# pathint/RankCompV3.jl

Measured on AMD Instinct MI355X. Metric: gene-pair·sample comparisons/sec at 20k genes × 1k samples, higher is better.
Workload: dtype u16

## Files before the change

rankcompv3.jl_amd/_ffi.py:

```python
from __future__ import annotations

import ctypes
import os
import subprocess
from typing import NamedTuple

import numpy as np

_HERE = os.path.dirname(os.path.abspath(__file__))
LIB_PATH = os.environ.get("REO_LIB_PATH") or os.path.join(_HERE, "libreo_hip.so")
CSRC = os.path.join(_HERE, "csrc")

REO_OK, REO_EINVAL, REO_EHIP, REO_ECOMM, REO_ENOMEM = 0, -1, -2, -3, -4
NTIMINGS = 12
CALL_BINS = 8192

SYMBOLS = [
    "reo_version", "reo_last_error", "reo_create", "reo_destroy", "reo_trim_memory", "reo_set_shard", "reo_set_allreduce", "reo_set_allgather",
    "reo_create_multi", "reo_comm_unique_id", "reo_comm_init_rank",
    "reo_set_matrix_f64", "reo_set_matrix_i64", "reo_set_matrix_dev_f64", "reo_set_matrix_dev_i64",
    "reo_set_matrix_f32", "reo_set_matrix_i32", "reo_set_matrix_dev_f32", "reo_set_matrix_dev_i32",
    "reo_set_matrix_rm_f64", "reo_set_matrix_rm_i64", "reo_set_matrix_rm_f32", "reo_set_matrix_rm_i32",
    "reo_set_matrix_csc_f64", "reo_set_matrix_csc_i64", "reo_set_matrix_csc_f32", "reo_set_matrix_csc_i32",
    "reo_set_groups", "reo_compute_thresholds", "reo_set_thresholds", "reo_get_thresholds", "reo_threshold",
# ... 1138 lines not shown
        counts, key = np.zeros((m, 4), dtype=np.int32), np.zeros((m, 2), dtype=np.int64)
        found, passes = ctypes.c_int64(0), ctypes.c_int32(0)
        check(self._L.reo_top_pairs(self._h, a, b, _opt(gm), n, _ptr(gi), _ptr(gj), _ptr(counts), _ptr(key), ctypes.addressof(found),
                                    ctypes.addressof(passes)))
        k = int(found.value)
        return TopPairs(gi[:k].copy(), gj[:k].copy(), counts[:k, 0::2].copy(), counts[:k, 1::2].copy(), key[:k, 0].copy(), key[:k, 1].copy(),
                        sizes, a, None if b < 0 else b, int(passes.value))

    def top_partners(self, genes=None, m: int = 1, a: int = 0, b=None, partner_mask=None) -> TopPartners:
        m = int(m)
        a, b, sizes = self._sides(a, b)
        g = np.arange(self.G, dtype=np.int32) if genes is None else np.ascontiguousarray(np.asarray(genes).reshape(-1), dtype=np.int32)
        pm = None
        if partner_mask is not None:
            pm = np.asarray(partner_mask)
            if pm.shape != (self.G,):
                raise DimensionMismatch(REO_EINVAL, f"top_partners: partner_mask has shape {tuple(pm.shape)}, the matrix has {self.G} genes")
            pm = np.ascontiguousarray(pm if pm.dtype == np.uint8 else pm != 0, dtype=np.uint8)
        Q = int(g.size)
        w = min(max(m, 1), 1024)
        rows = Q if 1 <= Q <= 1 << 20 and Q * w <= 1 << 26 else 1
        partner = np.full((rows, w), -1, dtype=np.int32)
        counts, key = np.zeros((rows, w, 4), dtype=np.int32), np.zeros((rows, w, 2), dtype=np.int64)
        found = np.zeros(rows, dtype=np.int32)
        check(self._L.reo_top_partners(self._h, a, b, _ptr(g) if Q else None, Q, _opt(pm), m, _ptr(partner), _ptr(counts), _ptr(key), _ptr(found)))
        return TopPartners(g, partner, counts[:, :, 0::2].copy(), counts[:, :, 1::2].copy(), key[:, :, 0].copy(), key[:, :, 1].copy(), found,
                           sizes, a, None if b < 0 else b)

    def top_pairs_null(self, sides, a: int = 0, b=None, gene_mask=None, cuts=None) -> TopPairsNull:
        a, b, sizes = self._sides(a, b)
        rows = np.asarray(sides)
        if rows.ndim == 1:
            rows = rows.reshape(1, -1)
        if rows.ndim != 2 or rows.shape[1] != self.S:
            raise DimensionMismatch(REO_EINVAL, f"top_pairs_null: sides has shape {tuple(np.shape(sides))}, label rows are B x S = B x {self.S}")
        if rows.size and (rows.min() < 0 or rows.max() > 255):
            raise DimensionMismatch(REO_EINVAL, "top_pairs_null: label rows hold 0 (side B), 1 (side A) and 2 (takes no part)")
        rows = np.ascontiguousarray(rows, dtype=np.uint8)
        gm = None
        if gene_mask is not None:
            gm = np.asarray(gene_mask)
            if gm.shape != (self.G,):
                raise DimensionMismatch(REO_EINVAL, f"top_pairs_null: gene_mask has shape {tuple(gm.shape)}, the matrix has {self.G} genes")
            gm = np.ascontiguousarray(gm if gm.dtype == np.uint8 else gm != 0, dtype=np.uint8)
        ct = np.zeros(0, dtype=np.int64) if cuts is None else np.ascontiguousarray(np.asarray(cuts, dtype=np.int64).reshape(-1))
        B = rows.shape[0]
        m = min(max(B, 1), 1 << 20)
        nc = min(ct.size, 8)
        max_n, gi, gj = np.zeros(m, dtype=np.int64), np.zeros(m, dtype=np.int32), np.zeros(m, dtype=np.int32)
        reach = np.zeros((m, nc), dtype=np.int64)
        check(self._L.reo_top_pairs_null(self._h, a, b, _ptr(rows) if rows.size else None, B, _opt(gm), _ptr(ct) if ct.size else None, ct.size,
                                         _ptr(max_n), _ptr(gi), _ptr(gj), _ptr(reach) if reach.size else None))
        return TopPairsNull(max_n[:B], gi[:B], gj[:B], reach[:B], ct, sizes, a, None if b < 0 else b)

    def top_pairs_loo(self, kmax: int, a: int = 0, b=None, gene_mask=None) -> TopPairsLoo:
        kmax = int(kmax)
        a, b, sizes = self._sides(a, b)
        gm = None
        if gene_mask is not None:
            gm = np.asarray(gene_mask)
            if gm.shape != (self.G,):
                raise DimensionMismatch(REO_EINVAL, f"top_pairs_loo: gene_mask has shape {tuple(gm.shape)}, the matrix has {self.G} genes")
            gm = np.ascontiguousarray(gm if gm.dtype == np.uint8 else gm != 0, dtype=np.uint8)
        m, S = min(max(kmax, 1), 64), max(self.S, 1)
        gi, gj = np.full((S, m), -1, dtype=np.int32), np.full((S, m), -1, dtype=np.int32)
        num, gam = np.zeros((S, m), dtype=np.int64), np.zeros((S, m), dtype=np.int64)
        out, side, stats = np.zeros((S, m), dtype=np.int8), np.full(S, 2, dtype=np.int8), np.zeros(4, dtype=np.int64)
        check(self._L.reo_top_pairs_loo(self._h, a, b, _opt(gm), kmax, _ptr(gi), _ptr(gj), _ptr(num), _ptr(gam), _ptr(out), _ptr(side), _ptr(stats)))
        n = self.S
        return TopPairsLoo(gi[:n], gj[:n], num[:n], gam[:n], out[:n], side[:n], sizes, a, None if b < 0 else b, int(stats[0]), int(stats[1]))

    def mccullagh(self, cont) -> np.ndarray:
        cont = np.ascontiguousarray(cont, dtype=np.int32).reshape(-1, 9)
        out = np.zeros((cont.shape[0], 5), dtype=np.float64)
        check(self._L.reo_mccullagh(self._h, _ptr(cont), cont.shape[0], _ptr(out)))
        return out

    @staticmethod
    def _pseudobulk_args(cells, order, chunk_ptr):
        order = np.ascontiguousarray(order, dtype=np.int32)
        chunk_ptr = np.ascontiguousarray(chunk_ptr, dtype=np.int32)
        n_out = chunk_ptr.size - 1
        if hasattr(cells, "tocsc"):
            m = cells.tocsc()
            m.sort_indices()
            G, C = m.shape
            isint = np.issubdtype(m.dtype, np.integer)
            val = np.ascontiguousarray(m.data, dtype=np.int64 if isint else np.float64)
            colptr = np.ascontiguousarray(m.indptr, dtype=np.int64)
            rowidx = np.ascontiguousarray(m.indices, dtype=np.int32)
            args = (G, C, _ptr(colptr), _ptr(rowidx), _ptr(val), _ptr(order), order.size, _ptr(chunk_ptr), n_out)
            return "csc", "i64" if isint else "f64", args, G, (m, val, colptr, rowidx, order, chunk_ptr)
        X = np.asarray(cells)
        isint = np.issubdtype(X.dtype, np.integer)
        Xf = np.asfortranarray(X, dtype=np.int64 if isint else np.float64)
        G, C = Xf.shape
        args = (_ptr(Xf), G, C, G, _ptr(order), order.size, _ptr(chunk_ptr), n_out)
        return "dense", "i64" if isint else "f64", args, G, (Xf, order, chunk_ptr)

    def pseudobulk(self, cells, order, chunk_ptr) -> np.ndarray:
        form, ty, args, G, keep = self._pseudobulk_args(cells, order, chunk_ptr)
        out = np.zeros((G, args[-1]), dtype=np.int64 if ty == "i64" else np.float64, order="F")
        check(getattr(self._L, f"reo_pseudobulk_{form}_{ty}")(self._h, *args, _ptr(out)))
        return out

    def set_matrix_pseudobulk(self, cells, order, chunk_ptr) -> None:
        if is_device_sparse(cells) or is_device_tensor(cells):
            order = np.ascontiguousarray(order, dtype=np.int32)
            chunk_ptr = np.ascontiguousarray(chunk_ptr, dtype=np.int32)
            n_out = chunk_ptr.size - 1
            tail = (_ptr(order) if order.size else None, order.size, _ptr(chunk_ptr), n_out)
            if is_device_sparse(cells):
                ty, G, C, nnz, colptr, rowidx, val, bits, keep = device_csc_entry(cells)
                check(getattr(self._L, "reo_set_matrix_pseudobulk_csc_dev_" + ty)(self._h, G, C, nnz, _dptr(colptr), _dptr(rowidx), bits, _dptr(val), *tail))
            else:
                ptr, G, C, ld, ty, keep = device_matrix(cells)
                check(getattr(self._L, "reo_set_matrix_pseudobulk_dense_dev_" + ty)(self._h, ctypes.c_void_p(ptr), G, C, ld, *tail))
            self.G, self.S = G, n_out
            return
        form, ty, args, G, keep = self._pseudobulk_args(cells, order, chunk_ptr)
        check(getattr(self._L, f"reo_set_matrix_pseudobulk_{form}_{ty}")(self._h, *args))
        self.G, self.S = G, args[-1]

    def filter_matrix(self, min_profiles: int = 0, min_features: int = 0):
        info = self.info()
        pk = np.zeros(info["S"], dtype=np.uint8)
        gk = np.zeros(info["G"], dtype=np.uint8)
        sk, gkn = ctypes.c_int64(0), ctypes.c_int64(0)
        check(self._L.reo_filter_matrix(self._h, int(min_profiles), int(min_features), _ptr(pk) if pk.size else None, _ptr(gk) if gk.size else None,
                                        ctypes.byref(sk), ctypes.byref(gkn)))
        self.G, self.S = int(gkn.value), int(sk.value)
        return pk.astype(bool), gk.astype(bool)

    def get_matrix(self) -> np.ndarray:
        info = self.info()
        dt = {1: np.float64, 2: np.int64, 3: np.float32}.get(info["resident_dtype"])
        if dt is None:
            raise DimensionMismatch(REO_EINVAL, "no expression matrix set")
        out = np.zeros((info["G"], info["S"]), dtype=dt, order="F")
        check(self._L.reo_get_matrix(self._h, _ptr(out), out.nbytes))
        return out

    def set_profiling(self, on: bool) -> None:
        check(self._L.reo_set_profiling(self._h, 1 if on else 0))

    def reset_timings(self) -> None:
        check(self._L.reo_reset_timings(self._h))

    def timings(self) -> dict:
        ms = np.zeros(NTIMINGS, dtype=np.float64)
        check(self._L.reo_get_timings(self._h, _ptr(ms), NTIMINGS))
        return {"transform_ms": ms[0], "k1_ms": ms[1], "k2_ms": ms[2], "iter_ms": ms[3], "k3_ms": max(ms[3] - ms[2], 0.0), "k2_launches": int(ms[4]),
                "k1_launches": int(ms[5]), "exchange_ms": ms[6], "pseudobulk_ms": ms[7], "k2_full_ms": ms[8],
                "k2_full_launches": int(ms[9]), "k2_delta_ms": ms[10], "set_matrix_host_wall_ms": ms[11]}

    def info(self) -> dict:
        w = np.zeros(44, dtype=np.int64)
        check(self._L.reo_get_info(self._h, _ptr(w), 44))
        v = np.zeros(28, dtype=np.int64)
        v[:] = w[:28]
        return {"G": int(v[0]), "S": int(v[1]), "Gp": int(v[2]), "table_bytes": int(v[3]), "has_ties": int(v[4]),
                "tiles_owned": int(v[5]), "tiles_total": int(v[6]), "tile_i": int(v[7]), "chunk_j": int(v[8]),
                "chunks_per_panel": int(v[9]), "unit_h": int(v[10]), "sample_slots": int(v[11]),
                "shared_group_counts": int(v[12]), "group_count_bytes": int(v[13]), "transform_in_lds": int(v[14]), "xcc_local_histograms": int(v[15]),
                "cycle_period": int(v[16]), "cycle_found_at_pass": int(v[17]), "cycle_passes_skipped": int(v[18]), "upload_link_bytes": int(v[19]),
                "eager_range_launches": int(v[20]), "rowmajor_upload": int(v[21]),
                "csc_upload": int(v[22]), "csc_nnz": int(v[23]), "resident_dtype": int(v[24]),
                "k1_slot_order": int(v[25]), "k1_half_tiles_separated": int(v[26]), "csc_device": int(v[27]),
                "k1_unslot_form": int(w[28]), "contrast_treat": int(w[29]), "k1_slot_sides": int(w[30]),
                "masked_build": int(w[31]), "k1_slot_slice": int(w[32]), "planes_on_demand": int(w[33]),
                "perm_batch": int(w[34]), "perm_kernel_us": int(w[35]),
                "top_pairs_hist_us": int(w[36]), "top_pairs_emit_us": int(w[37]),
                "top_pairs_null_batch": int(w[38]), "top_pairs_null_us": int(w[39]),
                "top_pairs_loo_words_us": int(w[40]), "top_pairs_loo_select_us": int(w[41]),
                "top_partners_count_us": int(w[42]), "top_partners_select_us": int(w[43])}
```

rankcompv3.jl_amd/csrc/api.hip:

```cpp
#include <execinfo.h>
#include <signal.h>
#include <unistd.h>

#include <ctime>
#include <algorithm>
#include <chrono>
#include <cmath>
#include <cstdarg>
#include <cstdio>
#include <cstdlib>
#include <cstring>

#include "reo_internal.h"
#include "contrast.h"
#include "masked_pairs.h"
#include "perm_null.h"
#include "sample_counts.h"
#include "upload_csc.h"

#include <mutex>
#include <unordered_map>

namespace reo {

// ... 34 lines not shown
        auto &v = H.streams[kind];
        for (size_t i = v.size(); i-- > 0;)
            if (v[i].first == dev) { *s = v[i].second; v.erase(v.begin() + static_cast<long>(i)); return hipSuccess; }
    }
    if (kind == 0) return hipStreamCreateWithFlags(s, hipStreamNonBlocking);
    int lo_pri = 0, hi_pri = 0;
    const hipError_t e = hipDeviceGetStreamPriorityRange(&lo_pri, &hi_pri);
    return e != hipSuccess ? e : hipStreamCreateWithPriority(s, hipStreamNonBlocking, hi_pri);
}

hipError_t handle_event(hipEvent_t *ev, int kind)
{
    int dev = 0;
    (void)hipGetDevice(&dev);
    {
        Handles &H = handles();
        std::lock_guard<std::mutex> lk(H.mu);
        auto &v = H.events[kind];
        for (size_t i = v.size(); i-- > 0;)
            if (v[i].first == dev) { *ev = v[i].second; v.erase(v.begin() + static_cast<long>(i)); return hipSuccess; }
    }
    return kind ? hipEventCreate(ev) : hipEventCreateWithFlags(ev, hipEventDisableTiming);
}

void release_stream(hipStream_t s, int kind)
{
    if (!s) return;
    int dev = 0;
    (void)hipGetDevice(&dev);
    Handles &H = handles();
    {
        std::lock_guard<std::mutex> lk(H.mu);
        if (H.streams[kind].size() < 64 && pool().cap > 0 && hipStreamQuery(s) == hipSuccess) { H.streams[kind].emplace_back(dev, s); return; }
    }
    (void)hipStreamDestroy(s);
}

void release_event(hipEvent_t ev, int kind)
{
    if (!ev) return;
    int dev = 0;
    (void)hipGetDevice(&dev);
    Handles &H = handles();
    {
        std::lock_guard<std::mutex> lk(H.mu);
        if (H.events[kind].size() < 1024 && pool().cap > 0) { H.events[kind].emplace_back(dev, ev); return; }
    }
    (void)hipEventDestroy(ev);
}

hipError_t pool_alloc(void **out, size_t bytes, bool pinned)
{
    Pool &P = pool();
    bytes = pool_round(bytes);
    int dev = 0;
    (void)hipGetDevice(&dev);
    {
        std::lock_guard<std::mutex> lk(P.mu);
        if (!P.read_env) {
            P.read_env = true;
            if (const char *e = getenv("REO_DEVICE_CACHE_MB")) P.cap = static_cast<size_t>(std::max(0L, atol(e))) << 20;
        }
        int best = -1;
        for (int i = 0; i < static_cast<int>(P.free_blocks.size()); ++i) {
            const Block &b = P.free_blocks[i];
            if (b.pinned != pinned || (!pinned && b.device != dev) || b.bytes < bytes || b.bytes > bytes + bytes / 4 + 4096) continue;
            if (best < 0 || b.bytes < P.free_blocks[best].bytes) best = i;
        }
        if (best >= 0) {
            *out = P.free_blocks[best].p;
            P.cached -= P.free_blocks[best].bytes;
            P.live[*out] = P.free_blocks[best].bytes;
            P.free_blocks.erase(P.free_blocks.begin() + best);
            return hipSuccess;
        }
    }
    hipError_t e = raw_alloc(out, bytes, pinned);
    if (e == hipErrorOutOfMemory) {
        (void)hipGetLastError();
        (void)reo_trim_memory();
        e = raw_alloc(out, bytes, pinned);
    }
    if (e == hipSuccess) { std::lock_guard<std::mutex> lk(P.mu); P.live[*out] = bytes; }
    return e;
}

void pool_free(void *p, size_t bytes, bool pinned)
{
    if (!p) return;
    Pool &P = pool();
    bytes = pool_round(bytes);
    int dev = 0;
    (void)hipGetDevice(&dev);
    std::vector<Block> evict;
    {
        std::lock_guard<std::mutex> lk(P.mu);
        const auto it = P.live.find(p);
        if (it != P.live.end()) { bytes = it->second; P.live.erase(it); }
        if (bytes > P.cap) { evict.push_back({p, bytes, dev, pinned}); }
        else {
            P.free_blocks.push_back({p, bytes, dev, pinned});
            P.cached += bytes;
            while (P.cached > P.cap && !P.free_blocks.empty()) {
                evict.push_back(P.free_blocks.front());
                P.cached -= P.free_blocks.front().bytes;
                P.free_blocks.erase(P.free_blocks.begin());
            }
        }
    }
    for (const Block &b : evict) {
        if (!b.pinned && b.device != dev) (void)hipSetDevice(b.device);
        raw_free(b.p, b.pinned);
        if (!b.pinned && b.device != dev) (void)hipSetDevice(dev);
    }
}

void set_error(const char *fmt, ...)
{
    char buf[1024];
    va_list ap;
    va_start(ap, fmt);
    vsnprintf(buf, sizeof buf, fmt, ap);
    va_end(ap);
    g_err = buf;
}

void tic(reo_ctx *c, int slot)
{
    if (!c->profiling) return;
    StageTimer t;
    if (!c->pool.empty()) { t = c->pool.back(); c->pool.pop_back(); }
    else { (void)handle_event(&t.a, 1); (void)handle_event(&t.b, 1); }
    (void)hipEventRecord(t.a, c->stream);
    c->pending.emplace_back(slot, t);
    c->open.push_back(c->pending.size() - 1);
}

void toc(reo_ctx *c)
{
    if (!c->profiling || c->open.empty()) return;
    (void)hipEventRecord(c->pending[c->open.back()].second.b, c->stream);
    c->open.pop_back();
}

void collect_timings(reo_ctx *c)
{
    for (auto &pr : c->pending) {
        float ms = 0.f;
        (void)hipEventSynchronize(pr.second.b);
        if (hipEventElapsedTime(&ms, pr.second.a, pr.second.b) == hipSuccess) {
            c->t_ms[pr.first] += ms;
            if (pr.first == 2 && !c->k2_modes.empty()) {
                if (c->k2_seen < c->k2_modes.size()) {
                    if (c->k2_modes[c->k2_seen]) { c->t_ms[8] += ms; c->t_ms[9] += 1.0; }
                    else c->t_ms[10] += ms;
                }
                ++c->k2_seen;
            }
        }
        c->pool.push_back(pr.second);
    }
    c->pending.clear();
    c->open.clear();
    c->k2_modes.clear();
    c->k2_seen = 0;
}

static int32_t major_reo_lower_count(int32_t n, double thr) { return reo_lower_count(n, thr); }

static hipError_t stream_wait(reo_ctx *c)
{
    if (!c->spin_wait) return hipStreamSynchronize(c->stream);
    for (unsigned spin = 0;; ++spin) {
        const hipError_t q = hipStreamQuery(c->stream);
        if (q != hipErrorNotReady) return q;
        if (spin > (1u << 22)) return hipStreamSynchronize(c->stream);
    }
}

static struct sigaction g_old_action[3];

static void segv_backtrace(int sig)
{
    static const char head[] = "libreo_hip: fatal signal, native backtrace of the faulting thread:\n";
    (void)!write(2, head, sizeof head - 1);
    void *frames[64];
    const int n = backtrace(frames, 64);
    backtrace_symbols_fd(frames, n, 2);
    sigaction(sig, &g_old_action[sig == SIGSEGV ? 0 : (sig == SIGBUS ? 1 : 2)], nullptr);
    raise(sig);
}

static void install_segv_backtrace()
{
    static bool done = false;
    if (done) return;
    done = true;
    void *warm[2];
    (void)backtrace(warm, 2);
    struct sigaction sa;
    memset(&sa, 0, sizeof sa);
    sa.sa_handler = segv_backtrace;
    sa.sa_flags = SA_NODEFER;
    sigaction(SIGSEGV, &sa, &g_old_action[0]);
    sigaction(SIGBUS, &sa, &g_old_action[1]);
    sigaction(SIGABRT, &sa, &g_old_action[2]);
}

static double wall_us()
{
    timespec ts;
    clock_gettime(CLOCK_MONOTONIC, &ts);
    return ts.tv_sec * 1e6 + ts.tv_nsec * 1e-3;
}

static void drop_ref_mask(reo_ctx *c, const char *why)
{
    c->ref_slot = -1;
    c->ref_gone = why;
}

int32_t wait_or_drop_table(reo_ctx *c)
{
    const hipError_t e = stream_wait(c);
    if (e == hipSuccess) return REO_OK;
    c->built_k = -1;
    c->table_complete = false;
    drop_ref_mask(c, "a kernel queued on this context failed and the class table was dropped");
    set_error("a kernel queued on this context failed: %s (the class table was dropped: call reo_build_pairs again)", hipGetErrorString(e));
    return REO_EHIP;
}

int32_t use(reo_ctx *c)
{
    if (!c) { set_error("null context"); return REO_EINVAL; }
    REO_HIP_CHECK(hipSetDevice(c->device));
    return REO_OK;
}

int32_t no_multi(reo_ctx *c, const char *what)
{
    if (!c) { set_error("null context"); return REO_EINVAL; }
    if (c->in_multi) {
        set_error("%s is not available on a reo_create_multi context (every device would need the matrix: use one process per GPU, each with its own context)", what);
        return REO_EINVAL;
    }
    return REO_OK;
}

bool mask_in_force(reo_ctx *c)
{
    if (c->vmask_set && (c->vmask_G != c->G || c->vmask_S != c->S)) { c->vmask_set = false; c->vwords_valid = false; }
    return c->vmask_set;
}

int32_t refuse_under_mask(reo_ctx *c, const char *what)
{
    if (!c || !mask_in_force(c)) return REO_OK;
    char msg[320];
    mp_query_refusal(what, msg, sizeof msg);
    set_error("%s", msg);
    return REO_EINVAL;
}

static void invalidate(reo_ctx *c)
{
    drop_ref_mask(c, "the matrix or the groups changed after the last reo_identify_degs (reo_set_matrix_*, reo_filter_matrix, reo_set_groups): "
                     "the class table it ran on is gone");
    c->transformed = false;
    c->planes_ready = false; c->planes_on_demand = 0; c->last_k1_slot_slice = 0;
    c->built_k = -1;
    c->built_treat = -1;
    c->built_masked = 0;
    c->gc_valid = false;
    c->eager_k1 = false;
    c->vwords_valid = false;
    (void)mask_in_force(c);
    c->last_k1_slots = 0; c->last_k1_slot_sides = 0; c->k1_slot_items = nullptr; c->k1_slot_items_n = 0; c->k1_slot_gp = 0;
}

static size_t elem_bytes(int dtype) { return dtype >= 3 ? 4 : 8; }

static int32_t check_shape(int64_t G, int64_t S)
{
    if (G < 2 || G > kMaxGenes || S < 2 || S > (1 << 20)) {
        set_error("matrix is %lld x %lld; G must be in [2, %d] and S in [2, 1048576]", (long long)G, (long long)S, kMaxGenes);
        return REO_EINVAL;
    }
    return REO_OK;
}

static int32_t set_matrix(reo_ctx *c, const void *X, int64_t G, int64_t S, int64_t ld, int dtype, bool on_device, int layout = kLayoutColMajor)
{
    const bool rowmajor = layout == kLayoutRowMajor;
    int32_t rc = use(c);
    if (rc) return rc;
    if (dtype >= 3 && getenv("REO_TRANSFORM") && getenv("REO_TRANSFORM")[0] == 's') {
        set_error("REO_TRANSFORM=segmented: the segmented sort of the A/B build takes Float64 and Int64 matrices only, not Float32 / Int32");
        return REO_EINVAL;
    }
    if (!X) { set_error("matrix pointer is null"); return REO_EINVAL; }
    if ((rc = check_shape(G, S))) return rc;
    if (rowmajor && ld < S) { set_error("row pitch %lld < S = %lld (row-major: ld counts the elements from one gene's row to the next)", (long long)ld, (long long)S); return REO_EINVAL; }
    if (layout == kLayoutColMajor && ld < G) { set_error("leading dimension %lld < G = %lld", (long long)ld, (long long)G); return REO_EINVAL; }
    invalidate(c);
    c->rowmajor_upload = 0;
    c->csc_upload = 0; c->csc_nnz = 0; c->csc_device = 0;
    const bool host_i32 = dtype == 4 && !on_device;
    const size_t resident = static_cast<size_t>(G) * S * (dtype == 3 ? 4 : 8);
    c->G = G; c->S = S; c->dtype = dtype == 4 ? 2 : dtype;
    if (on_device && dtype == 4) {
        if ((rc = c->dX_owned.ensure(resident))) return rc;
        c->dX = c->dX_owned.p; c->ld = G;
        if ((rc = widen_device_i32(c, X, ld, G, S, c->dX_owned.p))) { invalidate(c); c->dtype = 0; return rc; }
        if (hipStreamSynchronize(c->stream) != hipSuccess) { set_error("widening the Int32 matrix failed"); invalidate(c); c->dtype = 0; return REO_EHIP; }
    } else if (on_device) {
        c->dX = X; c->ld = ld;
        c->dX_owned.release();
    } else {
        if ((rc = c->dX_owned.ensure(resident))) return rc;
        c->dX = c->dX_owned.p; c->ld = G;
        const bool lds_ranking = G <= 65535 && !(getenv("REO_TRANSFORM") && getenv("REO_TRANSFORM")[0] == 's');
        if (c->eager_mode > 0 && lds_ranking && static_cast<int64_t>(c->group_id.size()) == S && !c->in_multi) {
            const bool k1 = c->eager_mode > 1 && c->ngroups == 2 && c->thr_set && c->world <= 1 && !c->comm && !c->ag && !c->ar && c->k1_wave &&
                            S <= 65535 && !c->k1_stamps;
            c->Gp = static_cast<int>((c->G + kGenePad - 1) / kGenePad) * kGenePad;
            c->Wp = c->Gp / 32;
            if ((rc = c->table.ensure(static_cast<size_t>(c->G) * kPlanes * c->Wp))) return rc;
            const double w0 = wall_us();
            struct DrainUp {
                reo_ctx *c;
                ~DrainUp() { if (c->up) (void)hipStreamSynchronize(c->up); if (c->rk) (void)hipStreamSynchronize(c->rk); }
            } drain_up{c};
            DrainOnExit drain(c);
            rc = eager_upload(c, X, ld, k1, host_i32, layout);
            if (rc) { invalidate(c); return rc; }
            c->rowmajor_upload = rowmajor ? 1 : 0;
            c->csc_upload = layout == kLayoutCsc ? 1 : 0;
            drain.dismiss();
            c->t_ms[11] += (wall_us() - w0) * 1e-3;
            if (c->eager_k1) { c->built_k = 0; c->table_complete = true; }
            return REO_OK;
        }
        struct DrainUp2 {
            reo_ctx *c;
            ~DrainUp2() { if (c->up) (void)hipStreamSynchronize(c->up); }
        } drain_up{c};
        DrainOnExit drain(c);
        const double w0 = wall_us();
        if ((rc = upload_columns(c, X, ld, G, S, c->dX_owned.p, dtype, layout))) { invalidate(c); return rc; }
        c->rowmajor_upload = rowmajor ? 1 : 0;
        c->csc_upload = layout == kLayoutCsc ? 1 : 0;
        drain.dismiss();
        c->t_ms[11] += (wall_us() - w0) * 1e-3;
    }
    return REO_OK;
}

int32_t ensure_transform(reo_ctx *c)
{
    if (c->dtype == 0) { set_error("no expression matrix set"); return REO_EINVAL; }
    if (c->group_id.empty()) { set_error("no groups set"); return REO_EINVAL; }
    if (static_cast<int64_t>(c->group_id.size()) != c->S) {
        set_error("'data' and 'group' do not have compatible sizes (%lld columns, %zu group labels)",
                  (long long)c->S, c->group_id.size());
        return REO_EINVAL;
    }
    if (c->transformed) return REO_OK;
    c->Gp = static_cast<int>((c->G + kGenePad - 1) / kGenePad) * kGenePad;
    c->Wp = c->Gp / 32;
    c->table_prezeroed = false;
    int32_t rc = c->table.ensure(static_cast<size_t>(c->G) * kPlanes * c->Wp);
    if (rc) return rc;
    return run_transform(c);
}

static int32_t ensure_iter_buffers(reo_ctx *c)
{
    int32_t rc;
    const size_t G = c->G;
    for (int t = 0; t < 2; ++t) {
        if ((rc = c->refbits[t].ensure(c->Wp))) return rc;
        if ((rc = c->refbytes[t].ensure(c->Gp))) return rc;
    }
    if ((rc = c->raw.ensure(G * kRaw)) ||
        (rc = c->delta_list.ensure(2 * static_cast<size_t>(c->Gp))) || (rc = c->cont.ensure(G * 9)) || (rc = c->result.ensure(G * 15)) ||
        (rc = c->sorted_d.ensure((G + 63) / 64 * 64 + (G + 63) / 64)) || (rc = c->sorted_p.ensure(G)) || (rc = c->rank_s.ensure(G)) ||
        (rc = c->rank_a.ensure(G)) || (rc = c->scal.ensure(8)) || (rc = c->blockmin.ensure(std::max<size_t>(64, (G + 1023) / 1024))) ||
        (rc = c->state.ensure(1)) ||
        (rc = c->chunk_v.ensure(((G + kSortChunk - 1) / kSortChunk) * (kSortChunk + kSortChunk / 32))) ||
        (rc = c->chunk_i.ensure(((G + kSortChunk - 1) / kSortChunk) * kSortChunk)) || (rc = c->part.ensure(3 * (std::max<size_t>(65536, (G + kSortChunk - 1) / kSortChunk * kSortChunk) / 16 + 8))) ||
        (rc = c->cand.ensure(2 * 1024)) || (rc = c->gridbar.ensure(4)) || (rc = c->hist.ensure(3 * kHistParts * ((G + 32767) / 32768 * 32768))) || (rc = c->olist.ensure(2 * kOneStride)) || (rc = c->mrank.ensure(c->Gp)) || (rc = c->lstate.ensure(1)) || (rc = c->clist.ensure(2 * kListStride)) || (rc = c->scal.ensure(64)))
        return rc;
    if (!c->host_state) REO_HIP_CHECK(pool_alloc(reinterpret_cast<void **>(&c->host_state), sizeof(IterState), true));
    return REO_OK;
}

static int32_t upload_ref(reo_ctx *c, const uint8_t *ref, int slot, int32_t *nref)
{
    int32_t n = 0;
    for (int64_t i = 0; i < c->G; ++i) n += ref[i] != 0;
    *nref = n;
    REO_HIP_CHECK(hipMemsetAsync(c->refbytes[slot].p, 0, c->Gp, c->stream));
    REO_HIP_CHECK(hipMemcpyAsync(c->refbytes[slot].p, ref, c->G, hipMemcpyHostToDevice, c->stream));
    return launch_pack_ref(c, c->refbytes[slot].p, c->refbits[slot].p);
}

static int32_t init_state(reo_ctx *c, int32_t nref)
{
    IterState st;
    memset(&st, 0, sizeof st);
    st.nref = nref;
    st.nref_prev = nref;
    st.delta_cnt[0] = st.delta_cnt[1] = 0x7FFFFFFF;
    st.need_full = 1;
    st.raw_pass = -1;
    st.kstar = -1;
    *c->host_state = st;
    REO_HIP_CHECK(hipMemcpyAsync(c->state.p, c->host_state, sizeof st, hipMemcpyHostToDevice, c->stream));
    return REO_OK;
}

static int32_t exchange_table(reo_ctx *c)
{
    if (c->x_pipelined) {
        c->table_complete = true;
        return REO_OK;
    }
    c->table_complete = c->world <= 1;
    if (c->world <= 1 && !c->comm) return REO_OK;
    int32_t rc;
    if (c->comm || c->ag) {
        const int64_t bytes = exchange_unit_words(c) * exchange_units_per_rank(c) * static_cast<int64_t>(sizeof(uint32_t));
        if ((rc = c->xsend.ensure(static_cast<size_t>(bytes / 4))) || (rc = c->xrecv.ensure(static_cast<size_t>(bytes / 4) * c->world))) return rc;
        tic(c, 6);
        if ((rc = launch_pack_units(c))) return rc;
        if (c->comm) {
            if ((rc = comm_allgather(c, c->xsend.p, c->xrecv.p, bytes)) < 0) return rc;
        } else {
            rc = c->ag(c->xsend.p, c->xrecv.p, bytes, c->stream, c->ag_user);
            if (rc) { set_error("all-gather hook failed with %d", rc); return REO_ECOMM; }
        }
        if ((rc = launch_expand_units(c))) return rc;
        toc(c);
    } else {
        if (!c->ar) return REO_OK;
        const int64_t count = static_cast<int64_t>(c->G) * kPlanes * c->Wp;
        tic(c, 6);
        rc = c->ar(c->table.p, count, c->stream, c->ar_user);
        toc(c);
        if (rc) { set_error("all-reduce hook failed with %d", rc); return REO_ECOMM; }
    }
    c->table_complete = true;
    return REO_OK;
}

static int32_t pass_fault(reo_ctx *c)
{
    const int32_t f = c->host_state ? c->host_state->fault : 0;
    if (!f) return REO_OK;
    if (f == kFaultTallies) {
        set_error("the iteration passes met tallies that no class table can produce (a gene pair in two states at once): the table in "
                  "this context is not what reo_build_pairs makes -- an exchange hook delivered wrong words and the scan of its "
                  "table was switched off (REO_CHECK_HOOK_TABLE=0)");
        c->built_k = -1;
        c->table_complete = false;
    } else {
        set_error("the persistent iteration kernel gave up at a grid barrier (a workgroup did not arrive within its bound); "
                  "REO_LIGHT=1 runs the same passes as separate launches");
    }
    return REO_EHIP;
}

int32_t upload_slot2col(reo_ctx *c, const std::vector<int32_t> &map)
{
    if (map == c->sc_slot2col_host && c->sc_slot2col.p == c->sc_slot2col_uploaded) return REO_OK;
    c->sc_slot2col_host = map;
    c->sc_slot2col_uploaded = nullptr;
    REO_HIP_CHECK(hipMemcpyAsync(c->sc_slot2col.p, c->sc_slot2col_host.data(), map.size() * sizeof(int32_t), hipMemcpyHostToDevice, c->stream));
    c->sc_slot2col_uploaded = c->sc_slot2col.p;
    return REO_OK;
}

int32_t need_complete_table(reo_ctx *c)
{
    if (c->built_k < 0) { set_error("no class table: call reo_build_pairs first"); return REO_EINVAL; }
    if (!c->table_complete) {
        set_error("shard %d of %d holds only its own part of the class table: attach a communicator (reo_comm_init_rank) or an "
                  "exchange hook (reo_set_allgather, reo_set_allreduce) before reo_build_pairs", c->rank, c->world);
        return REO_ECOMM;
    }
    return REO_OK;
}

}

using namespace reo;

extern "C" {

int32_t reo_version(void) { return 1600; }

int32_t reo_trim_memory(void)
{
    std::vector<Block> all;
    {
        Pool &P = pool();
        std::lock_guard<std::mutex> lk(P.mu);
        all.swap(P.free_blocks);
        P.cached = 0;
    }
    int dev = 0;
    const bool have_dev = hipGetDevice(&dev) == hipSuccess;
    for (const Block &b : all) {
        if (!b.pinned) (void)hipSetDevice(b.device);
        raw_free(b.p, b.pinned);
    }
    {
        Handles &H = handles();
        std::lock_guard<std::mutex> lk(H.mu);
        for (int k = 0; k < 2; ++k) {
            for (auto &st : H.streams[k]) { (void)hipSetDevice(st.first); (void)hipStreamDestroy(st.second); }
            for (auto &ev : H.events[k]) { (void)hipSetDevice(ev.first); (void)hipEventDestroy(ev.second); }
            H.streams[k].clear(); H.events[k].clear();
        }
    }
    if (have_dev) (void)hipSetDevice(dev);
    return REO_OK;
}

const char *reo_last_error(void) { return g_err.c_str(); }

int32_t reo_create(reo_ctx **out, int32_t device, uint64_t seed)
{
    if (!out) { set_error("out is null"); return REO_EINVAL; }
    *out = nullptr;
    if (getenv("REO_DEBUG_SEGV")) install_segv_backtrace();
    int ndev = 0;
    if (hipGetDeviceCount(&ndev) != hipSuccess || ndev == 0) {
        set_error("no HIP device visible: libreo_hip has no CPU fallback");
        return REO_EHIP;
    }
    if (device < 0) REO_HIP_CHECK(hipGetDevice(&device));
    if (device >= ndev) { set_error("device %d out of range (%d visible)", device, ndev); return REO_EINVAL; }
    hipDeviceProp_t prop;
    REO_HIP_CHECK(hipGetDeviceProperties(&prop, device));
    if (strncmp(prop.gcnArchName, "gfx950", 6) != 0) {
        set_error("device %d is %s; this library carries gfx950 (MI355X) code objects only", device, prop.gcnArchName);
        return REO_EHIP;
    }
    REO_HIP_CHECK(hipSetDevice(device));
    reo_ctx *c = new (std::nothrow) reo_ctx();
    if (!c) { set_error("out of host memory"); return REO_ENOMEM; }
    c->device = device;
    c->seed = seed;
    if (const char *e = getenv("REO_K1_WAVE")) c->k1_wave = (e[0] != '0');
    if (const char *e = getenv("REO_K1_HALF")) c->k1_half = (e[0] != '0');
    if (const char *e = getenv("REO_K1_SLOTS")) c->k1_slots = (e[0] != '0');
    if (const char *e = getenv("REO_K1_QUEUE")) c->k1_queue = (e[0] != '0');
    if (const char *e = getenv("REO_K1_UNSLOT")) { const int v = atoi(e); c->k1_unslot = (v == 8 || v == 4) ? v : (e[0] == '0' ? 0 : -1); }
    if (const char *e = getenv("REO_K1_SLOT_SIDES")) { const int v = atoi(e); c->k1_slot_sides = (v == 1 || v == 2) ? v : 0; }
    if (const char *e = getenv("REO_K1_SLOT_SLICE")) c->k1_slot_slice = atoi(e) != 0;
    if (const char *e = getenv("REO_K1_WORKERS")) c->k1_workers = std::max(1, atoi(e));
    if (const char *e = getenv("REO_K1_ORDER")) c->k1_order = std::max(0, std::min(2, atoi(e)));
    {
        int n = 0;
        if (hipDeviceGetAttribute(&n, hipDeviceAttributeMultiprocessorCount, c->device) == hipSuccess && n > 0) c->n_cus = n;
    }
    if (const char *e = getenv("REO_SPIN_WAIT")) c->spin_wait = (e[0] != '0');
    if (const char *e = getenv("REO_CHECK_HOOK_TABLE")) c->check_hook_table = (e[0] != '0');
    if (const char *e = getenv("REO_SHARE_GROUP_COUNTS")) c->share_counts = (e[0] != '0');
    if (const char *e = getenv("REO_LIGHT_BAND")) c->light_band = std::max(0, atoi(e));
    if (const char *e = getenv("REO_HIST_BELOW")) c->hist_below = std::max(0, atoi(e));
    if (const char *e = getenv("REO_CYCLE")) c->cycle_watch = atoi(e) != 0;
    if (const char *e = getenv("REO_LIGHT")) c->light_mode = e[0] == '0' ? 0 : (e[0] == '2' ? 2 : (e[0] == '3' ? 3 : 1));
    c->light_window = light_window(); c->light_min_g = light_min_genes();
    if (const char *e = getenv("REO_LIGHT_WINDOW")) c->light_window = std::max(1, std::min(31, atoi(e)));
    if (const char *e = getenv("REO_LIGHT_MIN_G")) c->light_min_g = std::max(64, atoi(e));
    if (const char *e = getenv("REO_STATE_MIRROR")) c->state_mirror_wanted = (e[0] != '0');
    if (const char *e = getenv("REO_EXCHANGE_WAVES")) c->x_waves = std::max(1, std::min(8, atoi(e)));
    if (const char *e = getenv("REO_EAGER_UPLOAD")) c->eager_mode = std::max(0, std::min(2, atoi(e)));
    if (const char *e = getenv("REO_EAGER_CHUNK")) c->eager_chunk = std::max(1, atoi(e));
    if (const char *e = getenv("REO_EAGER_GATE")) c->eager_gate = atoi(e) != 0;
    if (const char *e = getenv("REO_EAGER_RANGES")) c->eager_ranges = std::max(1, std::min(6, atoi(e)));
    if (const char *e = getenv("REO_UPLOAD_THREADS")) c->upload_threads = std::max(0, std::min(64, atoi(e)));
    c->debug_passes = getenv("REO_DEBUG_PASSES") != nullptr;
    c->debug_stamps = getenv("REO_DEBUG_STAMPS") != nullptr;
    c->k1_stamps = getenv("REO_K1_STAMPS") != nullptr;
    hipError_t e = handle_stream(&c->stream, 0);
    if (e != hipSuccess) { delete c; set_error("hipStreamCreate failed: %s", hipGetErrorString(e)); return REO_EHIP; }
    int ok = 0;
    const char *xe = getenv("REO_XCC_LOCAL");
    if (!(xe && xe[0] == '0')) {
        const int32_t rc = xcc_selftest(c, &ok);
        if (rc) { reo_destroy(c); return rc; }
    }
    c->xcc_local = ok;
    *out = c;
    return REO_OK;
}

void reo_destroy(reo_ctx *c)
{
    if (!c) return;
    for (reo_ctx *p : c->peers) reo_destroy(p);
    c->peers.clear();
    (void)hipSetDevice(c->device);
    for (int q = 0; q < 2; ++q) if (c->k1s[q]) (void)hipStreamSynchronize(c->k1s[q]);
    if (c->xs) (void)hipStreamSynchronize(c->xs);
    if (c->up) (void)hipStreamSynchronize(c->up);
    if (c->rk) (void)hipStreamSynchronize(c->rk);
    (void)hipStreamSynchronize(c->stream);
    comm_release(c);
    collect_timings(c);
    tl_release_synced = true;
    for (auto &t : c->pool) { release_event(t.a, 1); release_event(t.b, 1); }
    c->dX_owned.release(); c->pos.release(); c->lo.release(); c->hi.release(); c->goff_dev.release();
    c->table.release();
    c->t_kin.release(); c->t_kout.release(); c->t_vin.release(); c->t_vout.release(); c->t_temp.release();
    c->t_order.release(); c->t_flags.release(); c->t_slots.release(); c->unit_map.release();
    for (auto &il : c->k1_wave_items) il.buf.release();
    for (int q = 0; q < 2; ++q) { release_stream(c->k1s[q], 0); release_event(c->ev_k1_join[q], 0); }
    release_stream(c->xs, 0);
    release_stream(c->up, 0);
    release_stream(c->rk, 1);
    for (auto &e : c->ev_rk) release_event(e, 0);
    for (auto &e : c->ev_up) release_event(e, 0);
    c->e_lists.release();
    for (int q = 0; q < 3; ++q) {
        if (c->stage_h[q]) pool_free(c->stage_h[q], c->stage_cap, true);
        c->stage_d[q].release();
        release_event(c->ev_stage[q], 0);
        release_event(c->ev_widen[q], 0);
    }
    release_event(c->ev_fork, 0);
    release_event(c->ev_x, 0);
    for (auto &e : c->ev_k1) release_event(e, 0);
    c->t_pos16.release(); c->t_lo16.release(); c->t_hi16.release(); c->gcounts.release();
    c->k1_slot_part.release(); c->k1_slot_maps.release(); c->pos_s.release(); c->lo_s.release(); c->k1_queue_ctr.release();
    c->t_pos32.release(); c->t_lo32.release(); c->t_hi32.release(); c->t_vin32.release(); c->t_vout32.release();
    for (int t = 0; t < 2; ++t) { c->refbits[t].release(); c->refbytes[t].release(); }
    c->raw.release(); c->delta_list.release(); c->cont.release(); c->result.release(); c->sorted_d.release(); c->sorted_p.release();
    c->rank_s.release(); c->rank_a.release(); c->scal.release(); c->blockmin.release();
    c->state.release(); c->trace.release(); c->modes.release(); c->cand.release(); c->hist.release(); c->mrank.release(); c->lstate.release(); c->clist.release(); c->olist.release(); c->units_all.release(); c->xsend.release(); c->xrecv.release(); c->check_flag.release(); c->gridbar.release(); c->chunk_v.release(); c->chunk_i.release(); c->part.release();
    if (c->host_state) pool_free(c->host_state, sizeof(IterState), true);
    if (c->host_flags) pool_free(c->host_flags, 8 * sizeof(int32_t), true);
    release_event(c->ev_flags, 0);
    if (c->host_ref) pool_free(c->host_ref, c->host_ref_cap, true);
    release_stream(c->stream, 0);
    delete c;
    tl_release_synced = false;
}

int32_t reo_set_shard(reo_ctx *c, int32_t rank, int32_t world)
{
    if (!c) { set_error("null context"); return REO_EINVAL; }
    if (world < 1 || rank < 0 || rank >= world) { set_error("bad shard %d of %d", rank, world); return REO_EINVAL; }
    if (!c->peers.empty()) { set_error("a multi-GPU context (reo_create_multi) shards by itself"); return REO_EINVAL; }
    c->rank = rank; c->world = world;
    c->built_k = -1;
    drop_ref_mask(c, "reo_set_shard dropped the class table that the last reo_identify_degs ran on");
    c->eager_k1 = false;
    c->gc_valid = false;
    c->table_complete = false;
    return REO_OK;
}

int32_t reo_set_allreduce(reo_ctx *c, reo_allreduce_fn fn, void *user)
{
    if (!c) { set_error("null context"); return REO_EINVAL; }
    c->ar = fn; c->ar_user = user;
    return REO_OK;
}

int32_t reo_set_allgather(reo_ctx *c, reo_allgather_fn fn, void *user)
{
    if (!c) { set_error("null context"); return REO_EINVAL; }
    c->ag = fn; c->ag_user = user;
    return REO_OK;
}

static int32_t set_matrix_all(reo_ctx *c, const void *X, int64_t G, int64_t S, int64_t ld, int dtype, bool on_device, int layout = kLayoutColMajor)
{
    int32_t rc = set_matrix(c, X, G, S, ld, dtype, on_device, layout);
    for (size_t d = 0; d < (c ? c->peers.size() : 0) && !rc; ++d) {
        reo_ctx *p = c->peers[d];
        if (!on_device) { rc = set_matrix(p, X, G, S, ld, dtype, false, layout); continue; }
        const void *src = dtype == 4 ? c->dX : X;
        const int64_t sld = dtype == 4 ? G : ld;
        const size_t eb = dtype == 4 ? 8 : elem_bytes(dtype);
        if ((rc = use(p)) || (rc = p->dX_owned.ensure(static_cast<size_t>(G) * S * eb))) break;
        if (hipMemcpy2DAsync(p->dX_owned.p, static_cast<size_t>(G) * eb, src, static_cast<size_t>(sld) * eb, static_cast<size_t>(G) * eb, static_cast<size_t>(S),
                             hipMemcpyDefault, p->stream) != hipSuccess) {
            set_error("peer copy of the matrix to device %d failed", p->device); rc = REO_EHIP;
        }
        if (!rc && hipStreamSynchronize(p->stream) != hipSuccess) { set_error("peer copy failed"); rc = REO_EHIP; }
        if (!rc) { invalidate(p); p->G = G; p->S = S; p->dtype = dtype == 4 ? 2 : dtype; p->dX = p->dX_owned.p; p->ld = G; }
    }
    if (c && !c->peers.empty()) (void)hipSetDevice(c->device);
    return rc;
}

int32_t reo_set_matrix_f64(reo_ctx *c, const double *X, int64_t G, int64_t S, int64_t ld) { return set_matrix_all(c, X, G, S, ld, 1, false); }
int32_t reo_set_matrix_i64(reo_ctx *c, const int64_t *X, int64_t G, int64_t S, int64_t ld) { return set_matrix_all(c, X, G, S, ld, 2, false); }
int32_t reo_set_matrix_dev_f64(reo_ctx *c, const void *dX, int64_t G, int64_t S, int64_t ld) { return set_matrix_all(c, dX, G, S, ld, 1, true); }
int32_t reo_set_matrix_dev_i64(reo_ctx *c, const void *dX, int64_t G, int64_t S, int64_t ld) { return set_matrix_all(c, dX, G, S, ld, 2, true); }
int32_t reo_set_matrix_f32(reo_ctx *c, const float *X, int64_t G, int64_t S, int64_t ld) { return set_matrix_all(c, X, G, S, ld, 3, false); }
int32_t reo_set_matrix_i32(reo_ctx *c, const int32_t *X, int64_t G, int64_t S, int64_t ld) { return set_matrix_all(c, X, G, S, ld, 4, false); }
int32_t reo_set_matrix_dev_f32(reo_ctx *c, const void *dX, int64_t G, int64_t S, int64_t ld) { return set_matrix_all(c, dX, G, S, ld, 3, true); }
int32_t reo_set_matrix_dev_i32(reo_ctx *c, const void *dX, int64_t G, int64_t S, int64_t ld) { return set_matrix_all(c, dX, G, S, ld, 4, true); }
int32_t reo_set_matrix_rm_f64(reo_ctx *c, const double *X, int64_t G, int64_t S, int64_t ld) { return set_matrix_all(c, X, G, S, ld, 1, false, kLayoutRowMajor); }
int32_t reo_set_matrix_rm_i64(reo_ctx *c, const int64_t *X, int64_t G, int64_t S, int64_t ld) { return set_matrix_all(c, X, G, S, ld, 2, false, kLayoutRowMajor); }
int32_t reo_set_matrix_rm_f32(reo_ctx *c, const float *X, int64_t G, int64_t S, int64_t ld) { return set_matrix_all(c, X, G, S, ld, 3, false, kLayoutRowMajor); }
int32_t reo_set_matrix_rm_i32(reo_ctx *c, const int32_t *X, int64_t G, int64_t S, int64_t ld) { return set_matrix_all(c, X, G, S, ld, 4, false, kLayoutRowMajor); }

extern "C++" template <class V>
static int32_t set_matrix_csc(reo_ctx *c, int64_t G, int64_t S, const int64_t *colptr, const int32_t *rowidx, const V *val, int dtype)
{
    if (!c) { set_error("null context"); return REO_EINVAL; }
    int32_t rc = check_shape(G, S);
    if (rc) return rc;
    if (!colptr) { set_error("colptr is null"); return REO_EINVAL; }
    if (colptr[0] != 0) { set_error("colptr must start at 0 (colptr[0] = %lld)", (long long)colptr[0]); return REO_EINVAL; }
    const int64_t nnz = colptr[S];
    if (nnz < 0 || nnz > G * S) { set_error("colptr[S] = %lld is not a number of entries of a %lld x %lld matrix", (long long)nnz, (long long)G, (long long)S); return REO_EINVAL; }
    if (nnz > 0 && (!rowidx || !val)) { set_error("%s is null with nnz = %lld entries", !rowidx ? "rowidx" : "val", (long long)nnz); return REO_EINVAL; }
    const CscSrc<V> src{colptr, rowidx, val, nnz};
    rc = set_matrix_all(c, &src, G, S, 0, dtype, false, kLayoutCsc);
    if (!rc) {
        c->csc_nnz = nnz;
        for (reo_ctx *p : c->peers) p->csc_nnz = nnz;
    }
    return rc;
}
int32_t reo_set_matrix_csc_f64(reo_ctx *c, int64_t G, int64_t S, const int64_t *colptr, const int32_t *rowidx, const double *val) { return set_matrix_csc(c, G, S, colptr, rowidx, val, 1); }
int32_t reo_set_matrix_csc_i64(reo_ctx *c, int64_t G, int64_t S, const int64_t *colptr, const int32_t *rowidx, const int64_t *val) { return set_matrix_csc(c, G, S, colptr, rowidx, val, 2); }
int32_t reo_set_matrix_csc_f32(reo_ctx *c, int64_t G, int64_t S, const int64_t *colptr, const int32_t *rowidx, const float *val) { return set_matrix_csc(c, G, S, colptr, rowidx, val, 3); }
int32_t reo_set_matrix_csc_i32(reo_ctx *c, int64_t G, int64_t S, const int64_t *colptr, const int32_t *rowidx, const int32_t *val) { return set_matrix_csc(c, G, S, colptr, rowidx, val, 4); }

static int32_t set_matrix_pseudobulk(reo_ctx *c, bool csc, bool is_int, const void *X, int64_t G, int64_t C, int64_t ld, const int64_t *colptr,
                                     const int32_t *rowidx, const void *val, const int32_t *order, int64_t n_order, const int32_t *chunk_ptr,
                                     int32_t n_out)
{
    int32_t rc = no_multi(c, "reo_set_matrix_pseudobulk");
    if (rc) return rc;
    invalidate(c);
    c->dtype = 0; c->dX = nullptr;
    c->narrowed_bytes = 0; c->rowmajor_upload = 0; c->csc_upload = 0; c->csc_nnz = 0; c->csc_device = 0;
    if ((rc = use(c)) || (rc = check_shape(G, n_out))) return rc;
    rc = csc ? pseudobulk_resident_csc(c, is_int, G, C, colptr, rowidx, val, order, n_order, chunk_ptr, n_out)
             : pseudobulk_resident_dense(c, X, is_int, G, C, ld, order, n_order, chunk_ptr, n_out);
    if (rc) return rc;
    c->narrowed_bytes = 0;
    c->G = G; c->S = n_out; c->ld = G; c->dX = c->dX_owned.p; c->dtype = is_int ? 2 : 1;
    return REO_OK;
}

int32_t reo_set_matrix_pseudobulk_dense_f64(reo_ctx *c, const double *X, int64_t G, int64_t C, int64_t ld, const int32_t *order, int64_t n_order,
                                            const int32_t *chunk_ptr, int32_t n_out)
{ return set_matrix_pseudobulk(c, false, false, X, G, C, ld, nullptr, nullptr, nullptr, order, n_order, chunk_ptr, n_out); }
int32_t reo_set_matrix_pseudobulk_dense_i64(reo_ctx *c, const int64_t *X, int64_t G, int64_t C, int64_t ld, const int32_t *order, int64_t n_order,
                                            const int32_t *chunk_ptr, int32_t n_out)
{ return set_matrix_pseudobulk(c, false, true, X, G, C, ld, nullptr, nullptr, nullptr, order, n_order, chunk_ptr, n_out); }
int32_t reo_set_matrix_pseudobulk_csc_f64(reo_ctx *c, int64_t G, int64_t C, const int64_t *colptr, const int32_t *rowidx, const double *val,
                                          const int32_t *order, int64_t n_order, const int32_t *chunk_ptr, int32_t n_out)
{ return set_matrix_pseudobulk(c, true, false, nullptr, G, C, 0, colptr, rowidx, val, order, n_order, chunk_ptr, n_out); }
int32_t reo_set_matrix_pseudobulk_csc_i64(reo_ctx *c, int64_t G, int64_t C, const int64_t *colptr, const int32_t *rowidx, const int64_t *val,
                                          const int32_t *order, int64_t n_order, const int32_t *chunk_ptr, int32_t n_out)
{ return set_matrix_pseudobulk(c, true, true, nullptr, G, C, 0, colptr, rowidx, val, order, n_order, chunk_ptr, n_out); }

static int32_t begin_device_entry(reo_ctx *c, const char *what, int64_t G, int64_t S)
{
    int32_t rc = no_multi(c, what);
    if (rc) return rc;
    invalidate(c);
    c->dtype = 0; c->dX = nullptr;
    c->narrowed_bytes = 0; c->rowmajor_upload = 0; c->csc_upload = 0; c->csc_nnz = 0; c->csc_device = 0;
    if ((rc = use(c)) || (rc = check_shape(G, S))) return rc;
    return REO_OK;
}

static int32_t set_matrix_csc_dev(reo_ctx *c, int64_t G, int64_t S, int64_t nnz, const void *d_colptr, const void *d_rowidx, int32_t index_bits,
                                  const void *d_val, int dtype)
{
    int32_t rc = begin_device_entry(c, "reo_set_matrix_csc_dev", G, S);
    if (rc) return rc;
    if (dtype >= 3 && getenv("REO_TRANSFORM") && getenv("REO_TRANSFORM")[0] == 's') {
        set_error("REO_TRANSFORM=segmented: the segmented sort of the A/B build takes Float64 and Int64 matrices only, not Float32 / Int32");
        return REO_EINVAL;
    }
    DrainOnExit drain(c);
    const int64_t *colptr = nullptr;
    if ((rc = csc_device_check(c, G, S, nnz, d_colptr, d_rowidx, index_bits, d_val, &colptr))) return rc;
    if ((rc = c->dX_owned.ensure(static_cast<size_t>(G) * S * (dtype == 3 ? 4 : 8)))) return rc;
    if ((rc = densify_device_csc(c, G, S, colptr, d_rowidx, index_bits, d_val, dtype, c->dX_owned.p))) return rc;
// ... 282 lines not shown
    int32_t rc;
    if ((rc = c->sc_slot2col.ensure(map.size())) || (rc = c->vwords.ensure(map.size() / 32 * static_cast<size_t>(c->Gp)))) return rc;
    if ((rc = upload_slot2col(c, map)) || (rc = launch_valid_words(c, c->sc_slot2col.p))) return rc;
    c->vwords_valid = true;
    return REO_OK;
}

int32_t reo_set_valid_mask(reo_ctx *c, const uint8_t *valid, int64_t G, int64_t S, int64_t ld)
{
    int32_t rc = use(c);
    if (rc) return rc;
    if (!valid) { c->vmask_set = false; c->vwords_valid = false; return REO_OK; }
    char msg[320];
    if (mp_check_mask_args(mp_state(c), G, S, ld, msg, sizeof msg)) { set_error("%s", msg); return REO_EINVAL; }
    REO_HIP_CHECK(stream_wait(c));
    if ((rc = c->vmask.ensure(static_cast<size_t>(G) * S))) { c->vmask_set = false; c->vwords_valid = false; return rc; }
    c->vmask_set = false; c->vwords_valid = false;
    DrainOnExit drain(c);
    REO_HIP_CHECK(hipMemcpy2DAsync(c->vmask.p, static_cast<size_t>(G), valid, static_cast<size_t>(ld), static_cast<size_t>(G), static_cast<size_t>(S),
                                   hipMemcpyHostToDevice, c->stream));
    REO_HIP_CHECK(hipStreamSynchronize(c->stream));
    drain.dismiss();
    c->vmask_set = true; c->vmask_G = G; c->vmask_S = S;
    return REO_OK;
}

int32_t reo_build_pairs_masked(reo_ctx *c, int32_t k, double pval_reo, const int32_t *min_complete)
{
    int32_t rc = use(c);
    if (rc) return rc;
    const MpState st = mp_state(c);
    if (!st.multi && st.world <= 1 && (c->dtype == 0 || c->group_id.empty() || static_cast<int64_t>(c->group_id.size()) != c->S))
        return ensure_transform(c);
    char msg[320];
    if (mp_check_build_args(st, k, pval_reo, min_complete, msg, sizeof msg)) { set_error("%s", msg); return REO_EINVAL; }
    int32_t n1 = 0;
    for (int32_t g : c->group_id) n1 += g == k;
    const int32_t n2 = static_cast<int32_t>(c->S) - n1;
    if (c->mp_thr_n[0] != n1 || c->mp_thr_n[1] != n2 || c->mp_thr_pval != pval_reo || c->mp_thr_host.size() != static_cast<size_t>(n1) + n2 + 2) {
        std::vector<int32_t> m1, m2;
        if (!mp_threshold_table(n1, pval_reo, m1) || !mp_threshold_table(n2, pval_reo, m2)) {
            set_error("reo_build_pairs_masked: no count in 0..n/2 has a two-sided binomial p above %g (the reference's findfirst returns nothing)", pval_reo);
            return REO_EINVAL;
        }
        c->mp_thr_host = m1;
        c->mp_thr_host.insert(c->mp_thr_host.end(), m2.begin(), m2.end());
        c->mp_thr_n[0] = n1; c->mp_thr_n[1] = n2; c->mp_thr_pval = pval_reo;
        c->mp_thr_uploaded = nullptr;
    }
    if ((rc = ensure_transform(c))) return rc;
    if ((rc = c->table.ensure(static_cast<size_t>(c->G) * kPlanes * c->Wp)) || (rc = c->mp_thr.ensure(c->mp_thr_host.size()))) return rc;
    if (c->mp_thr_uploaded != c->mp_thr.p) {
        REO_HIP_CHECK(hipMemcpyAsync(c->mp_thr.p, c->mp_thr_host.data(), c->mp_thr_host.size() * sizeof(int32_t), hipMemcpyHostToDevice, c->stream));
        REO_HIP_CHECK(hipStreamSynchronize(c->stream));
        c->mp_thr_uploaded = c->mp_thr.p;
    }
    if ((rc = ensure_valid_words(c, "reo_build_pairs_masked"))) return rc;
    drop_ref_mask(c, "reo_build_pairs_masked has replaced the class table that the last reo_identify_degs ran on: no reo_identify_degs has run on the current one");
    c->built_k = -1; c->built_treat = -1; c->built_masked = 0; c->eager_k1 = false; c->table_complete = false;
    c->last_k1_slots = 0; c->last_k1_slot_sides = 0; c->k1_slot_items = nullptr; c->k1_slot_items_n = 0; c->k1_slot_gp = 0; c->last_k1_shared = 0;
    REO_HIP_CHECK(hipMemsetAsync(c->table.p, 0, static_cast<size_t>(c->G) * kPlanes * c->Wp * sizeof(uint32_t), c->stream));
    c->table_prezeroed = false;
    if ((rc = launch_pairs_masked(c, k, c->mp_thr.p, n1, c->mp_thr.p + n1 + 1, n2, min_complete[0], min_complete[1]))) return rc;
    c->built_k = k; c->built_masked = 1; c->table_complete = true;
    return REO_OK;
}

int32_t reo_pair_counts_masked(reo_ctx *c, int64_t i0, int64_t i1, int64_t j0, int64_t j1, int32_t *n_gt, int32_t *n_eq, int32_t *n_avail)
{
    int32_t rc = use(c);
    if (rc) return rc;
    const MpState st = mp_state(c);
    if (!st.multi && st.world <= 1 && (c->dtype == 0 || c->group_id.empty() || static_cast<int64_t>(c->group_id.size()) != c->S))
        return ensure_transform(c);
    char msg[320];
    if (mp_check_counts_args(st, i0, i1, j0, j1, n_gt, n_eq, n_avail, msg, sizeof msg)) { set_error("%s", msg); return REO_EINVAL; }
    if ((rc = ensure_transform(c)) || (rc = ensure_valid_words(c, "reo_pair_counts_masked"))) return rc;
    const size_t n = static_cast<size_t>(i1 - i0) * (j1 - j0) * c->ngroups;
    DevBuf<int32_t> dg, de, da;
    if ((rc = dg.ensure(n)) || (rc = de.ensure(n)) || (rc = da.ensure(n))) return rc;
    DrainOnExit drain(c);
    if ((rc = launch_counts_masked(c, i0, i1, j0, j1, dg.p, de.p, da.p))) return rc;
    REO_HIP_CHECK(hipMemcpyAsync(n_gt, dg.p, n * sizeof(int32_t), hipMemcpyDeviceToHost, c->stream));
    REO_HIP_CHECK(hipMemcpyAsync(n_eq, de.p, n * sizeof(int32_t), hipMemcpyDeviceToHost, c->stream));
    REO_HIP_CHECK(hipMemcpyAsync(n_avail, da.p, n * sizeof(int32_t), hipMemcpyDeviceToHost, c->stream));
    if ((rc = wait_or_drop_table(c))) return rc;
    drain.dismiss();
    return REO_OK;
}

int32_t reo_get_codes(reo_ctx *c, int64_t i0, int64_t i1, int64_t j0, int64_t j1, uint8_t *code)
{
    int32_t rc = use(c);
    if (rc) return rc;
    if (c->built_k < 0) { set_error("no class table: call reo_build_pairs first"); return REO_EINVAL; }
    if (!code || i0 < 0 || j0 < 0 || i1 > c->G || j1 > c->G || i0 >= i1 || j0 >= j1) {
        set_error("bad pair block"); return REO_EINVAL;
    }
    const size_t n = static_cast<size_t>(i1 - i0) * (j1 - j0);
    DevBuf<uint8_t> d;
    if ((rc = d.ensure(n))) return rc;
    DrainOnExit drain(c);
    rc = launch_decode(c, i0, i1, j0, j1, d.p);
    if (!rc) {
        hipError_t e = hipMemcpyAsync(code, d.p, n, hipMemcpyDeviceToHost, c->stream);
        if (e == hipSuccess) e = hipStreamSynchronize(c->stream);
        if (e != hipSuccess) { set_error("copy-back failed: %s", hipGetErrorString(e)); rc = REO_EHIP; }
    }
    d.release();
    return rc;
}

int32_t reo_tally(reo_ctx *c, const uint8_t *ref_mask, int32_t *cont)
{
    int32_t rc = use(c);
    if (rc) return rc;
    if ((rc = need_complete_table(c))) return rc;
    if (!ref_mask || !cont) { set_error("null argument"); return REO_EINVAL; }
    if ((rc = ensure_iter_buffers(c))) return rc;
    drop_ref_mask(c, "reo_tally has run since the last reo_identify_degs: it uploads its own mask into the iteration's buffers");
    DrainOnExit drain(c);
    int32_t nref = 0;
    if ((rc = upload_ref(c, ref_mask, 0, &nref))) return rc;
    if ((rc = init_state(c, nref))) return rc;
    if ((rc = launch_tally(c, nref))) return rc;
    REO_HIP_CHECK(hipMemcpyAsync(cont, c->cont.p, sizeof(int32_t) * 9 * c->G, hipMemcpyDeviceToHost, c->stream));
    REO_HIP_CHECK(hipStreamSynchronize(c->stream));
    drain.dismiss();
    collect_timings(c);
    return REO_OK;
}

int32_t reo_identify_degs(reo_ctx *c, const uint8_t *ref0, double pval_deg, double padj_deg, int32_t n_iter,
                          int32_t n_conv, double *result, int32_t *iters_run, int32_t *trace)
{
    int32_t rc = use(c);
    if (rc) return rc;
    drop_ref_mask(c, "the last reo_identify_degs on this context failed");
    if ((rc = need_complete_table(c))) return rc;
    if (!ref0 || !result) { set_error("null argument"); return REO_EINVAL; }
    if ((rc = ensure_iter_buffers(c))) return rc;
    const int64_t G = c->G;
    const int64_t a = static_cast<int64_t>(std::nearbyint(static_cast<double>(G) * 0.05));
    const int64_t b = static_cast<int64_t>(std::nearbyint(static_cast<double>(G) * 0.95));
    if (n_iter > 0 && (a < 1 || b > G || b - a + 1 < 2)) {
        set_error("G = %lld: the slice %lld:%lld of the sorted delta1 vector is out of bounds or too short "
                  "(the reference throws at src/RankCompV3.jl:411-413)", (long long)G, (long long)a, (long long)b);
        return REO_EINVAL;
    }
    if ((rc = c->trace.ensure(2 * static_cast<size_t>(n_iter > 0 ? n_iter : 1)))) return rc;
    if ((rc = c->modes.ensure(static_cast<size_t>(n_iter > 0 ? n_iter : 1) + 64))) return rc;
    for (const auto &pr : c->pending)
        if (pr.first == 2) { collect_timings(c); break; }
    if (c->host_ref_cap < static_cast<size_t>(G)) {
        if (c->host_ref) pool_free(c->host_ref, c->host_ref_cap, true);
        c->host_ref = nullptr; c->host_ref_cap = 0;
        REO_HIP_CHECK(pool_alloc(reinterpret_cast<void **>(&c->host_ref), static_cast<size_t>(c->Gp), true));
        c->host_ref_cap = static_cast<size_t>(c->Gp);
    }
    int32_t nref = 0;
    for (int64_t i = 0; i < G; ++i) { c->host_ref[i] = ref0[i]; nref += ref0[i] != 0; }
    {
        IterState st;
        memset(&st, 0, sizeof st);
        st.nref = nref;
        st.nref_prev = nref;
        st.delta_cnt[0] = st.delta_cnt[1] = 0x7FFFFFFF;
        st.need_full = 1;
        st.raw_pass = -1;
        st.kstar = -1;
        st.cyc_period = -1;
        *c->host_state = st;
    }
    const bool watch = c->cycle_watch && c->light_mode != 0 && (c->light_mode == 1 || G > 65535) && G >= c->light_min_g && n_iter > 0;
    if (watch) {
        if ((rc = c->snap.ensure(2 * static_cast<size_t>(c->Gp)))) return rc;
        c->host_state->cyc_period = 0;
    }
    c->it_cycle_period = 0; c->it_cycle_at = 0; c->it_cycle_skipped = 0;
    DrainOnExit drain(c);
    if ((rc = launch_iter_init(c, c->host_ref, c->host_state))) return rc;
    c->it_pval_deg = pval_deg; c->it_padj_deg = padj_deg; c->it_n_iter = n_iter; c->it_n_conv = n_conv;
    c->it_a0 = static_cast<int>(a - 1); c->it_b0 = static_cast<int>(b - 1);
    c->k2_idx = 0;
    const int light_form = (G > 65535 && c->light_mode != 0) ? 1 : c->light_mode;
    c->it_light_form = light_form;
    c->state_mirror = light_form != 2 && c->state_mirror_wanted;
    bool small = G < c->light_min_g || c->light_mode == 0;
    c->it_no_light = false;
    int passes = 0, seen_need_full = 1, light_batches = 0, idle_light = 0, idle_any = 0;
    while (n_iter > 0) {
        const int remaining = n_iter - passes;
        const double w_loop = c->debug_passes ? wall_us() : 0.0;
        const int nfull = small ? std::min(8, remaining) : (seen_need_full ? std::min(passes == 0 ? 4 : 2, remaining) : 0);
        const int nlight = (small || seen_need_full) ? 0 : std::min(light_batches == 0 ? 32 : kLightBatch, remaining);
        if (nlight > 0) ++light_batches;
        tic(c, 3);
        for (int t = 0; t < nfull; ++t)
            if ((rc = launch_full_pass(c, false))) return rc;
        if (nlight > 0 && light_form == 2) {
            if ((rc = launch_light_persistent(c))) return rc;
        } else if (nlight > 0) {
            if ((rc = launch_light_batch(c, nlight))) return rc;
        }
        toc(c);
        if (!c->state_mirror) REO_HIP_CHECK(hipMemcpyAsync(c->host_state, c->state.p, sizeof(IterState), hipMemcpyDeviceToHost, c->stream));
        const double w0 = c->debug_passes ? wall_us() : 0.0;
        if ((rc = wait_or_drop_table(c))) return rc;
        if (c->debug_passes) fprintf(stderr, "  waited %.0f us for the batch (enqueueing it took %.0f us)\n", wall_us() - w0, w0 - w_loop);
        if (c->debug_passes && nlight > 0 && light_form == 3) {
            static LightState hs;
            if (hipMemcpy(&hs, c->lstate.p, sizeof hs, hipMemcpyDeviceToHost) == hipSuccess)
                for (int q = 1; q <= nlight; ++q)
                    if (hs.slot[q].pad0[0] || q <= 3)
                        fprintf(stderr, "  launch %d: why %d (1 window, 2 se left the bracket, 4 the histogram's cut left the band, 8 a list overflowed, 16 too many listed, 32 cut below the band), "
                                "cut of the m_lo histogram %d, listed %d, surely inside %d, cut %d (band around %d), eta %.3g, se %.10g\n", q, hs.slot[q].pad0[0], hs.slot[q].pad0[1],
                                hs.slot[q].pad0[2], hs.slot[q].pad0[3], hs.slot[q].pad0[4], hs.slot[q - 1].rec.kstar, hs.slot[q - 1].eta, hs.slot[q].se_base);
        }
        if (c->debug_passes)
            fprintf(stderr, "batch: %d sorting + %d light launches, passes %d -> %d, need_full %d, done %d, last_full %d, changed genes in front of the next pass %d\n", nfull, nlight,
                    passes, c->host_state->passes, c->host_state->need_full, c->host_state->done, c->host_state->last_full,
                    c->host_state->delta_cnt[c->host_state->passes & 1]);
        if ((rc = pass_fault(c))) return rc;
        idle_any = c->host_state->passes == passes ? idle_any + 1 : 0;
        if (idle_any >= 4) {
            set_error("the iteration made no progress in four batches of launches (passes %d, need_full %d): loop control fault", passes, c->host_state->need_full);
            return REO_EHIP;
        }
        if (nlight > 0) idle_light = c->host_state->passes == passes ? idle_light + 1 : 0;
        if (idle_light >= 2 && !small) {
            small = true;
            c->it_no_light = true;
        }
        if (c->host_state->passes < passes || c->host_state->passes > n_iter) {
            set_error("the iteration's pass counter reads %d after %d of %d passes: loop control fault", c->host_state->passes, passes, n_iter);
            return REO_EHIP;
        }
        passes = c->host_state->passes;
        seen_need_full = c->host_state->need_full;
        if (c->host_state->done || passes >= n_iter) break;
        if (c->host_state->cyc_period > 0) {
            const int p = c->host_state->cyc_period, P = (p & 1) ? 2 * p : p;
            const int skip = (n_iter - passes - 1) / P * P;
            if ((rc = launch_cycle_skip(c, skip, p))) return rc;
            c->it_cycle_period = p; c->it_cycle_at = passes; c->it_cycle_skipped = skip;
            if (c->debug_passes) fprintf(stderr, "cycle: the reference set in front of pass %d equals that of pass %d; %d passes skipped\n", passes, passes - p, skip);
            passes += skip;
        }
    }
    if (passes > 0 && !c->host_state->last_full) {
        tic(c, 3);
        if ((rc = launch_full_pass(c, true))) return rc;
        toc(c);
    }
    if (trace && passes > 0)
        REO_HIP_CHECK(hipMemcpyAsync(trace, c->trace.p, sizeof(int32_t) * 2 * passes, hipMemcpyDeviceToHost, c->stream));
    const int nk2 = std::min<int>(c->k2_idx, static_cast<int>(c->modes.n));
    if (c->profiling && nk2 > 0) {
        c->k2_modes.assign(c->k2_idx, 0);
        REO_HIP_CHECK(hipMemcpyAsync(c->k2_modes.data(), c->modes.p, sizeof(int32_t) * nk2, hipMemcpyDeviceToHost, c->stream));
    }
    if (c->debug_stamps) {
        unsigned long long st[24];
        REO_HIP_CHECK(hipMemcpy(st, c->scal.p + 32, sizeof st, hipMemcpyDeviceToHost));
        if (light_form == 3) {
            fprintf(stderr, "stamps kl_one (inputs back, se, cut, lists + mask step, changed rows, delta1, sums + windows, end):");
            for (int k = 0; k <= 7; ++k) fprintf(stderr, " %lld", (long long)(st[k] - st[8]));
        } else if (light_form == 2) {
            fprintf(stderr, "stamps kl_persist, one pass (phase 1, barrier, phase 2, barrier, loads asked, cut, mask step):");
            for (int k = 1; k <= 7; ++k) fprintf(stderr, " %lld", (long long)(st[k] - st[0]));
        } else {
            fprintf(stderr, "stamps kl_head (inputs back, cut, mask step, changed rows, delta1, window flags, block sums, end):");
            for (int k = 0; k <= 7; ++k) fprintf(stderr, " %lld", (long long)(st[k] - st[8]));
            fprintf(stderr, "\nstamps kl_rank (inputs back, selection + se, p + BH rank, end):");
            for (int k = 20; k <= 23; ++k) fprintf(stderr, " %lld", (long long)(st[k] - st[19]));
        }
        fprintf(stderr, "  (x 10 ns)\n");
    }
    if (iters_run) *iters_run = passes;
    const double w_copy = c->debug_passes ? wall_us() : 0.0;
    REO_HIP_CHECK(hipMemcpyAsync(result, c->result.p, sizeof(double) * 15 * G, hipMemcpyDeviceToHost, c->stream));
    const double w_copied = c->debug_passes ? wall_us() : 0.0;
    if ((rc = wait_or_drop_table(c))) return rc;
    drain.dismiss();
    if (c->debug_passes) fprintf(stderr, "  result copy: enqueued in %.0f us, waited %.0f us\n", w_copied - w_copy, wall_us() - w_copied);
    collect_timings(c);
    if ((rc = pass_fault(c))) return rc;
    if (passes > 0) c->ref_slot = (passes - 1) & 1;
    else drop_ref_mask(c, "the last reo_identify_degs was called with n_iter <= 0: no pass ran, no tallies were counted");
    return REO_OK;
}

int32_t reo_get_ref_mask(reo_ctx *c, uint8_t *ref_mask, int32_t *nref)
{
    int32_t rc = use(c);
    if (rc) return rc;
    if (!ref_mask) { set_error("reo_get_ref_mask: ref_mask must not be null"); return REO_EINVAL; }
    if (c->ref_slot < 0 || c->built_k < 0) {
        set_error("reo_get_ref_mask: no reference set to deliver: %s", c->ref_slot < 0 ? c->ref_gone : "the class table was dropped");
        return REO_EINVAL;
    }
    DrainOnExit drain(c);
    REO_HIP_CHECK(hipMemcpyAsync(ref_mask, c->refbytes[c->ref_slot].p, static_cast<size_t>(c->G), hipMemcpyDeviceToHost, c->stream));
    REO_HIP_CHECK(hipStreamSynchronize(c->stream));
    drain.dismiss();
    int32_t n = 0;
    for (int64_t i = 0; i < c->G; ++i) { ref_mask[i] = ref_mask[i] != 0; n += ref_mask[i]; }
    if (nref) *nref = n;
    return REO_OK;
}


namespace {

PnState pn_state(reo_ctx *c)
{
    PnState st{};
    st.multi = c->in_multi || !c->peers.empty();
    st.world = c->world;
    st.G = c->dtype ? c->G : 0; st.S = c->dtype ? c->S : 0;
    st.ngroups = c->ngroups;
    st.n_labels = static_cast<int64_t>(c->group_id.size());
    st.has_mask = mask_in_force(c);
    st.thr_set = c->thr_set && c->thr.size() == 2 * static_cast<size_t>(c->ngroups);
    st.built_k = c->built_k;
    st.plain_table = c->built_k >= 0 && c->built_treat < 0 && !c->built_masked && c->table_complete;
    return st;
}

struct TableLoan {
    reo_ctx *c;
    uint32_t *resident;
    explicit TableLoan(reo_ctx *ctx) : c(ctx), resident(ctx->table.p) {}
    TableLoan(const TableLoan &) = delete;
    TableLoan &operator=(const TableLoan &) = delete;
    void lend(uint32_t *t) { c->table.p = t; }
    void back() { c->table.p = resident; }
    ~TableLoan() { back(); }
};

int32_t pn_slot_map(reo_ctx *c, const char *what)
{
    std::vector<int32_t> map;
    if (!sc_slot_map(c->group_id.data(), c->S, c->ngroups, map) || c->goff32.empty() || static_cast<int64_t>(map.size()) != c->goff32.back()) {
        set_error("%s: the sample slots of the bit planes do not match the group labels", what);
        return REO_EHIP;
    }
    int32_t rc = c->sc_slot2col.ensure(map.size());
    return rc ? rc : upload_slot2col(c, map);
}

int32_t pn_side_size(const reo_ctx *c, int32_t k)
{
    int32_t n1 = 0;
    for (int32_t g : c->group_id) n1 += g == k;
    return n1;
}

}

int32_t reo_perm_codes(reo_ctx *c, int32_t k, const uint8_t *side_a, int64_t i0, int64_t i1, int64_t j0, int64_t j1, uint8_t *code)
{
    int32_t rc = use(c);
    if (rc) return rc;
    const PnState st = pn_state(c);
    char msg[320];
    const int32_t n1 = (k >= 0 && k < c->ngroups) ? pn_side_size(c, k) : 0;
    if (pn_check_codes_args(st, k, side_a, n1, i0, i1, j0, j1, code, msg, sizeof msg)) { set_error("%s", msg); return REO_EINVAL; }
    if ((rc = ensure_transform(c)) || (rc = pn_slot_map(c, "reo_perm_codes"))) return rc;
    const int nblk = c->goff32.back() / 32;
    const size_t table_words = static_cast<size_t>(c->G) * kPlanes * c->Wp, n = static_cast<size_t>(i1 - i0) * (j1 - j0);
    const char *env = getenv("REO_PERM_CODES_SLOT");
    int slot = env ? atoi(env) : 0;
    if (slot < 0 || slot >= kPermBatchCap) slot = 0;
    const int np = slot + 1;
    const size_t S = static_cast<size_t>(c->S);
    std::vector<uint8_t> rep(static_cast<size_t>(np) * S);
    for (int t = 0; t < np; ++t)
        for (size_t s = 0; s < S; ++s) rep[static_cast<size_t>(t) * S + s] = side_a[t == slot ? s : (s + static_cast<size_t>(t) + 1) % S];
    DevBuf<uint32_t> d_table, d_aw, d_live;
    DevBuf<uint8_t> d_side, d_code;
    if ((rc = d_table.ensure(static_cast<size_t>(np) * table_words)) || (rc = d_aw.ensure(pn_word_count(np, nblk))) || (rc = d_live.ensure(nblk)) ||
        (rc = d_side.ensure(rep.size())) || (rc = d_code.ensure(n)))
        return rc;
    TableLoan loan(c);
    DrainOnExit drain(c);
    REO_HIP_CHECK(hipMemcpyAsync(d_side.p, rep.data(), rep.size(), hipMemcpyHostToDevice, c->stream));
    REO_HIP_CHECK(hipMemsetAsync(d_table.p, 0, static_cast<size_t>(np) * table_words * sizeof(uint32_t), c->stream));
    if ((rc = launch_perm_words(c, d_side.p, np, c->sc_slot2col.p, d_aw.p, d_live.p)) ||
        (rc = launch_pairs_permuted(c, d_aw.p, d_live.p, np, n1, static_cast<int>(c->S) - n1, c->thr[2 * k], c->thr[2 * k + 1], d_table.p)))
        return rc;
    loan.lend(d_table.p + static_cast<size_t>(slot) * table_words);
    rc = launch_decode(c, i0, i1, j0, j1, d_code.p);
    loan.back();
    if (rc) return rc;
    REO_HIP_CHECK(hipMemcpyAsync(code, d_code.p, n, hipMemcpyDeviceToHost, c->stream));
    REO_HIP_CHECK(hipStreamSynchronize(c->stream));
    drain.dismiss();
    return REO_OK;
}

int32_t reo_perm_null(reo_ctx *c, int32_t k, const uint8_t *side_a, int64_t n_perm, const uint8_t *ref_mask, double pval_deg, double padj_deg,
                      double *delta1_obs, int32_t *n_ge, int32_t *n_up, int32_t *n_down, double *se_null, double *delta1_null)
{
    int32_t rc = use(c);
    if (rc) return rc;
    const PnState st = pn_state(c);
    char msg[320];
    const int32_t n1 = (k >= 0 && k < c->ngroups) ? pn_side_size(c, k) : 0;
    if (pn_check_null_args(st, k, side_a, n_perm, n1, ref_mask, pval_deg, padj_deg, delta1_obs, n_ge, n_up, n_down, se_null, msg, sizeof msg)) {
        set_error("%s", msg);
        return REO_EINVAL;
    }
    if ((rc = need_complete_table(c)) || (rc = ensure_transform(c))) return rc;
    if ((rc = wait_or_drop_table(c))) return rc;
    const int64_t G = c->G, S = c->S;
    const int nblk = c->goff32.back() / 32;
    const size_t table_words = static_cast<size_t>(G) * kPlanes * c->Wp;
    size_t free_b = 0, total_b = 0;
    REO_HIP_CHECK(hipMemGetInfo(&free_b, &total_b));
    const char *env = getenv("REO_PERM_BATCH");
    const int64_t P = pn_batch_tables(free_b, table_words * sizeof(uint32_t), n_perm, env ? atoll(env) : 0);
    if (P < 1) {
        set_error("reo_perm_null: one permuted class table needs %zu bytes of device memory beside the resident one, %zu are free", table_words * sizeof(uint32_t),
                  free_b);
        return REO_ENOMEM;
    }
    c->perm_batch = P; c->perm_kernel_us = 0;
    DevBuf<uint32_t> d_tables, d_aw, d_live;
    DevBuf<uint8_t> d_side;
    DevBuf<double> d_obs, d_se;
    DevBuf<int32_t> d_nge, d_cnt;
    if ((rc = d_tables.ensure(static_cast<size_t>(P) * table_words)) || (rc = d_aw.ensure(pn_word_count(P, nblk))) || (rc = d_live.ensure(nblk)) ||
        (rc = d_side.ensure(static_cast<size_t>(P) * S)) || (rc = d_obs.ensure(G)) || (rc = d_se.ensure(n_perm)) || (rc = d_nge.ensure(G)) ||
        (rc = d_cnt.ensure(2 * static_cast<size_t>(n_perm))) || (rc = pn_slot_map(c, "reo_perm_null")))
        return rc;
    std::vector<double> host_res(static_cast<size_t>(15) * G);
    hipEvent_t ev[2] = {nullptr, nullptr};
    REO_HIP_CHECK(hipEventCreate(&ev[0]));
    if (hipEventCreate(&ev[1]) != hipSuccess) { (void)hipEventDestroy(ev[0]); set_error("reo_perm_null: no event"); return REO_EHIP; }
    struct EventPair { hipEvent_t *e; ~EventPair() { (void)hipEventDestroy(e[0]); (void)hipEventDestroy(e[1]); } } ev_guard{ev};
    TableLoan loan(c);
    DrainOnExit drain(c);
    int32_t iters = 0;
    if ((rc = reo_identify_degs(c, ref_mask, pval_deg, padj_deg, 1, 0, host_res.data(), &iters, nullptr))) return rc;
    memcpy(delta1_obs, host_res.data() + 11 * G, sizeof(double) * G);
    REO_HIP_CHECK(hipMemcpyAsync(d_obs.p, c->result.p + 11 * G, sizeof(double) * G, hipMemcpyDeviceToDevice, c->stream));
    REO_HIP_CHECK(hipMemsetAsync(d_nge.p, 0, sizeof(int32_t) * G, c->stream));
    REO_HIP_CHECK(hipMemsetAsync(d_cnt.p, 0, sizeof(int32_t) * 2 * n_perm, c->stream));
    REO_HIP_CHECK(hipMemsetAsync(d_tables.p, 0, static_cast<size_t>(P) * table_words * sizeof(uint32_t), c->stream));
    for (int64_t p0 = 0; p0 < n_perm; p0 += P) {
        const int np = static_cast<int>(std::min<int64_t>(P, n_perm - p0));
        REO_HIP_CHECK(hipMemcpyAsync(d_side.p, side_a + p0 * S, static_cast<size_t>(np) * S, hipMemcpyHostToDevice, c->stream));
        if ((rc = launch_perm_words(c, d_side.p, np, c->sc_slot2col.p, d_aw.p, d_live.p))) return rc;
        REO_HIP_CHECK(hipEventRecord(ev[0], c->stream));
        if ((rc = launch_pairs_permuted(c, d_aw.p, d_live.p, np, n1, static_cast<int>(S) - n1, c->thr[2 * k], c->thr[2 * k + 1], d_tables.p))) return rc;
        REO_HIP_CHECK(hipEventRecord(ev[1], c->stream));
        for (int q = 0; q < np; ++q) {
            const int64_t p = p0 + q;
            loan.lend(d_tables.p + static_cast<size_t>(q) * table_words);
            rc = reo_identify_degs(c, ref_mask, pval_deg, padj_deg, 1, 0, host_res.data(), &iters, nullptr);
            loan.back();
            if (rc) return rc;
            if (q == 0) {
                float ms = 0.f;
                REO_HIP_CHECK(hipEventElapsedTime(&ms, ev[0], ev[1]));
                c->perm_kernel_us += static_cast<int64_t>(ms * 1000.0f + 0.5f);
            }
            if ((rc = launch_perm_accumulate(c, d_obs.p, pval_deg, padj_deg, d_nge.p, d_cnt.p + p, d_cnt.p + n_perm + p, d_se.p + p))) return rc;
            if (delta1_null) memcpy(delta1_null + p * G, host_res.data() + 11 * G, sizeof(double) * G);
        }
    }
    REO_HIP_CHECK(hipMemcpyAsync(n_ge, d_nge.p, sizeof(int32_t) * G, hipMemcpyDeviceToHost, c->stream));
    REO_HIP_CHECK(hipMemcpyAsync(n_up, d_cnt.p, sizeof(int32_t) * n_perm, hipMemcpyDeviceToHost, c->stream));
    REO_HIP_CHECK(hipMemcpyAsync(n_down, d_cnt.p + n_perm, sizeof(int32_t) * n_perm, hipMemcpyDeviceToHost, c->stream));
    REO_HIP_CHECK(hipMemcpyAsync(se_null, d_se.p, sizeof(double) * n_perm, hipMemcpyDeviceToHost, c->stream));
    if ((rc = wait_or_drop_table(c))) return rc;
    drain.dismiss();
    drop_ref_mask(c, "reo_perm_null has run since the last reo_identify_degs: its passes use the iteration's buffers");
    return REO_OK;
}

int32_t reo_mccullagh(reo_ctx *c, const int32_t *cont, int64_t n, double *out)
{
    int32_t rc = use(c);
    if (rc) return rc;
    if (!cont || !out || n < 1) { set_error("bad argument"); return REO_EINVAL; }
    DevBuf<int32_t> dc;
    DevBuf<double> dout;
    if ((rc = dc.ensure(n * 9)) || (rc = dout.ensure(n * 5))) return rc;
    DrainOnExit drain(c);
    hipError_t e = hipMemcpyAsync(dc.p, cont, sizeof(int32_t) * 9 * n, hipMemcpyHostToDevice, c->stream);
    if (e == hipSuccess) {
        rc = launch_mccullagh(c, dc.p, n, dout.p);
        if (!rc) {
            e = hipMemcpyAsync(out, dout.p, sizeof(double) * 5 * n, hipMemcpyDeviceToHost, c->stream);
            if (e == hipSuccess) e = hipStreamSynchronize(c->stream);
        }
    }
    if (e != hipSuccess) { set_error("HIP failure: %s", hipGetErrorString(e)); rc = REO_EHIP; }
    dc.release(); dout.release();
    return rc;
}

int32_t reo_set_profiling(reo_ctx *c, int32_t on)
{
    if (!c) { set_error("null context"); return REO_EINVAL; }
    c->profiling = on != 0;
    for (reo_ctx *p : c->peers) p->profiling = c->profiling;
    return REO_OK;
}

int32_t reo_reset_timings(reo_ctx *c)
{
    if (!c) { set_error("null context"); return REO_EINVAL; }
    collect_timings(c);
    for (double &v : c->t_ms) v = 0.0;
    return REO_OK;
}

int32_t reo_get_timings(reo_ctx *c, double *ms, int32_t n)
{
    if (!c || !ms) { set_error("null argument"); return REO_EINVAL; }
    collect_timings(c);
    for (int i = 0; i < n && i < REO_NTIMINGS; ++i) ms[i] = c->t_ms[i];
    return REO_OK;
}

int32_t reo_get_info(reo_ctx *c, int64_t *info, int32_t n)
{
    if (!c || !info) { set_error("null argument"); return REO_EINVAL; }
    int64_t separated = 0;
    if (n > 26 && c->last_k1_slots) {
        int32_t rc = use(c);
        if (rc || (rc = launch_slot_separated(c, &separated))) return rc;
    }
    const int64_t v[44] = {c->G, c->S, c->Gp, static_cast<int64_t>(c->table.n * sizeof(uint32_t)), c->has_ties,
                           c->tiles_owned, c->tiles_total, kTileI, c->k1_cj, c->k1_q, kUnitH,
                           c->goff32.empty() ? 0 : c->goff32.back(), c->last_k1_shared,
                           static_cast<int64_t>(c->gcounts.n * sizeof(uint16_t)), c->transform_in_lds, c->xcc_local,
                           c->it_cycle_period, c->it_cycle_at, c->it_cycle_skipped, c->narrowed_bytes, c->eager_range_launches, c->rowmajor_upload,
                           c->csc_upload, c->csc_nnz, c->dtype, c->last_k1_slots, separated, c->csc_device,
                           c->last_k1_slots ? c->last_k1_unslot : 0, c->built_k >= 0 ? c->built_treat : -1,
                           c->last_k1_slots ? c->last_k1_slot_sides : 0, (c->built_k >= 0 && c->built_masked) ? 1 : 0,
                           c->last_k1_slots ? c->last_k1_slot_slice : 0, c->transformed ? c->planes_on_demand : 0, c->perm_batch, c->perm_kernel_us,
                           c->top_hist_us, c->top_emit_us, c->top_null_batch, c->top_null_us, c->top_loo_words_us, c->top_loo_select_us,
                           c->top_partners_count_us, c->top_partners_select_us};
    for (int i = 0; i < n && i < 44; ++i) info[i] = v[i];
    return REO_OK;
}

}
```

rankcompv3.jl_amd/csrc/kernels.hip:

```cpp
#include <algorithm>
#include <chrono>
#include <cstddef>
#include <cstdio>
#include <cstdlib>
#include <cstring>
#include <mutex>
#include <type_traits>

#include "reo_internal.h"
#include "k1_items.h"
#include "k1_slots.h"
#include "k1_queue.h"
#include "contrast.h"
#include "tie_coin.h"
#include "band_chain.h"

namespace reo {

namespace {

template <bool COH, class T>
__device__ __forceinline__ T ldc(const T *p)
{
    if (COH) return __hip_atomic_load(p, __ATOMIC_RELAXED, __HIP_MEMORY_SCOPE_AGENT);
// ... 1197 lines not shown
__global__ __launch_bounds__(64, NB > 16 ? 2 : 3) void k1w_pairs_multi(K1Args a)
{
    constexpr int RI = kTileI, RJ = kRJ, NE = TIES ? 2 : 1;
    constexpr bool BIG = NB > 16;
    constexpr int LQ = BIG ? 5 : 4, ROWB = BIG ? 128 : 64;
    __shared__ uint4 ring[2 * RI * ROWB / 16];
    const uint32_t item = a.items[blockIdx.x];
    const int i0 = __builtin_amdgcn_readfirstlane(static_cast<int>(item & 0xFFFFu) * RI);
    const int jw = __builtin_amdgcn_readfirstlane(static_cast<int>((item >> 16) & 0x7FFFu) * (64 * RJ));
    const int lane = threadIdx.x, jl = jw + lane, bi = i0 >> 6;
    const uint32_t lds = static_cast<uint32_t>(reinterpret_cast<uintptr_t>(&ring[0]));
    uint32_t nk[RJ * (RI / 2)], tot[RJ * (RI / 2)];
    uint32_t park[TIES ? RJ * (RI / 2) : 1];
#pragma unroll
    for (int h = 0; h < RJ * (RI / 2); ++h) { nk[h] = 0; tot[h] = 0; }
#pragma clang loop unroll(disable)
    for (int g = 0; g < a.ngroups; ++g) {
        const int bb = __builtin_amdgcn_readfirstlane(a.goff[g]), be = __builtin_amdgcn_readfirstlane(a.goff[g + 1]);
        if (be <= bb) continue;
        u32x16 gt0, gt1, gt2, gt3;
        const char *pb = reinterpret_cast<const char *>(a.P) + static_cast<size_t>(bb) * LQ * a.Gp * 16;
        const size_t aoff = (static_cast<size_t>(bb) * a.Gp + i0) * ROWB;
#pragma clang loop unroll(disable)
        for (int e = 0; e < NE; ++e) {
            const char *ab = reinterpret_cast<const char *>(e ? a.AL : (TIES ? a.AH : a.AL)) + aoff;
            k1_loop<NB>(gt0, gt1, gt2, gt3, pb, static_cast<uint32_t>(a.Gp) * 16u, ab, static_cast<uint32_t>(a.Gp) * static_cast<uint32_t>(ROWB),
                        static_cast<uint32_t>(be - bb), static_cast<uint32_t>(jl) * 16u, static_cast<uint32_t>(lane) * 16u, lds);
            if (TIES && e == 0) {
#pragma unroll
                for (int h = 0; h < RI / 2; ++h) {
                    park[h] = gt0[h]; park[(TIES ? 1 : 0) * (RI / 2) + h] = gt1[h];
                    park[(TIES ? 2 : 0) * (RI / 2) + h] = gt2[h]; park[(TIES ? 3 : 0) * (RI / 2) + h] = gt3[h];
                }
            }
        }
#pragma clang loop unroll(disable)
        for (int r = 0; r < RJ; ++r) {
            const int j = jl + 64 * r;
#pragma unroll
            for (int h = 0; h < RI / 2; ++h) {
                uint32_t w = gt0[h];
                if (TIES) {
                    const uint32_t w2 = park[r * (RI / 2) + h];
                    uint32_t n0 = w & 0xFFFFu, n1 = w >> 16;
                    const uint32_t e0 = (w2 & 0xFFFFu) - n0, e1 = (w2 >> 16) - n1;
                    if (e0) n0 += tie_wins(a.seed, i0 + 2 * h, j, g, e0);
                    if (e1) n1 += tie_wins(a.seed, i0 + 2 * h + 1, j, g, e1);
                    w = n0 | (n1 << 16);
                }
                if (g == a.gc) nk[r * (RI / 2) + h] = w; else tot[r * (RI / 2) + h] += w;
            }
            gt0 = gt1; gt1 = gt2; gt2 = gt3;
        }
    }
#pragma clang loop unroll(disable)
    for (int r = 0; r < RJ; ++r) {
        uint32_t ck[RI / 2], ct[RI / 2];
#pragma unroll
        for (int h = 0; h < RI / 2; ++h) { ck[h] = nk[r * (RI / 2) + h]; ct[h] = tot[r * (RI / 2) + h]; }
        emit_gene<RI, true>(a, i0, jl + 64 * r, bi, lane, 0, a.m1, a.nc - a.m1, [&](int ii) { return static_cast<int>((ii & 1) ? (ck[ii >> 1] >> 16) : (ck[ii >> 1] & 0xFFFFu)); });
        emit_gene<RI, true>(a, i0, jl + 64 * r, bi, lane, 2, a.m2, a.nt - a.m2, [&](int ii) { return static_cast<int>((ii & 1) ? (ct[ii >> 1] >> 16) : (ct[ii >> 1] & 0xFFFFu)); });
    }
}

template <bool BIG>
__global__ __launch_bounds__(256) void k1_counts(const uint4 *__restrict__ P, const uint4 *__restrict__ AL,
                                                 const uint4 *__restrict__ AH, int Gp, int nbits,
                                                 const int32_t *__restrict__ goff, int ngroups, int ci0, int ci1, int cj0, int cj1,
                                                 uint16_t *__restrict__ out_gt, uint16_t *__restrict__ out_eq)
{
    constexpr int NW = BandLayout<BIG>::NW;
    const int j = cj0 + blockIdx.x * 256 + threadIdx.x, i = ci0 + blockIdx.y;
    if (j >= cj1 || i >= ci1) return;
    const int nj = cj1 - cj0;
    for (int g = 0; g < ngroups; ++g) {
        uint32_t n_gt = 0, n_ge = 0;
        for (int b = goff[g]; b < goff[g + 1]; ++b) {
            uint32_t p[NW], lo[NW], hi[NW];
#pragma unroll
            for (int q = 0; q < BandLayout<BIG>::NQ; ++q) {
                band_unpack(P[(static_cast<size_t>(b) * BandLayout<BIG>::NQ + q) * Gp + j], p, q);
                band_unpack(AL[band_edge_row<BIG>(Gp, b, i) + q], lo, q);
                band_unpack(AH[band_edge_row<BIG>(Gp, b, i) + q], hi, q);
            }
            uint32_t lt = 0, le = 0;
#pragma unroll
            for (int k = 0; k < NW; ++k) {
                if (k >= nbits) break;
                const int ew = BandLayout<BIG>::edge_word(k);
                lt = band_borrow(p[k], lo[ew], lt);
                le = band_borrow(p[k], hi[ew], le);
            }
            n_gt += __builtin_popcount(lt);
            n_ge += __builtin_popcount(le);
        }
        const size_t o = (static_cast<size_t>(i - ci0) * nj + (j - cj0)) * ngroups + g;
        out_gt[o] = static_cast<uint16_t>(n_gt);
        out_eq[o] = static_cast<uint16_t>(n_ge - n_gt);
    }
}

__global__ void k_decode(const uint32_t *__restrict__ table, int Wp, int i0, int i1, int j0, int j1,
                         uint8_t *__restrict__ code)
{
    const int j = j0 + blockIdx.x * blockDim.x + threadIdx.x;
    const int i = i0 + blockIdx.y;
    if (j >= j1 || i >= i1) return;
    const uint32_t *row = table + static_cast<size_t>(i) * kPlanes * Wp + (j >> 5);
    const uint32_t sh = j & 31;
    const int l = (row[0] >> sh) & 1, h = (row[Wp] >> sh) & 1;
    const int tl = (row[2 * Wp] >> sh) & 1, th = (row[3 * Wp] >> sh) & 1;
    const int ic = l ? 0 : (h ? 2 : 1), it = tl ? 0 : (th ? 2 : 1);
    code[static_cast<size_t>(i - i0) * (j1 - j0) + (j - j0)] = (i == j) ? 255 : static_cast<uint8_t>(3 * ic + it);
}

__global__ void k_time_mark(unsigned long long *out) { if (threadIdx.x == 0) *out = __builtin_amdgcn_s_memrealtime(); }

__global__ __launch_bounds__(256) void k_check_table(const uint32_t *__restrict__ table, int G, int Wp, int32_t *__restrict__ flag)
{
    const int row = blockIdx.x * 4 + (threadIdx.x >> 6), lane = threadIdx.x & 63;
    if (row >= G) return;
    const uint32_t *r = table + static_cast<size_t>(row) * kPlanes * Wp;
    uint32_t bad = 0;
    for (int w = lane; w < Wp; w += 64) {
        const uint32_t cl = r[w], ch = r[Wp + w], tl = r[2 * Wp + w], th = r[3 * Wp + w];
        uint32_t valid = 0xFFFFFFFFu;
        const int c0 = w * 32;
        if (c0 + 32 > G) valid = c0 >= G ? 0u : (0xFFFFFFFFu >> (c0 + 32 - G));
        if ((row >> 5) == w) valid &= ~(1u << (row & 31));
        bad |= (cl & ch) | (tl & th) | ((cl | ch | tl | th) & ~valid);
    }
    if (__ballot(bad != 0) && lane == 0) atomicOr(flag, 1);
}

__global__ __launch_bounds__(256) void k_pack_ref(const uint8_t *__restrict__ bytes, int Gp,
                                                  uint32_t *__restrict__ bits)
{
    const int g = blockIdx.x * 256 + threadIdx.x;
    const unsigned long long m = __ballot(g < Gp && bytes[g] != 0);
    if ((threadIdx.x & 63) == 0) {
        bits[g >> 5] = static_cast<uint32_t>(m);
        bits[(g >> 5) + 1] = static_cast<uint32_t>(m >> 32);
    }
}

struct IterInitArgs {
    const uint8_t *host_ref;
    const uint32_t *host_state;
    uint8_t *refbytes;
    uint32_t *refbits, *state;
    uint32_t *zero[3];
    size_t zero_n[3];
    int G, Gp, state_words;
};
__global__ __launch_bounds__(256) void k_iter_init(IterInitArgs a)
{
    const int g = blockIdx.x * 256 + threadIdx.x;
    const uint8_t b = g < a.G ? a.host_ref[g] : 0;
    a.refbytes[g] = b;
    const unsigned long long m = __ballot(b != 0);
    if ((threadIdx.x & 63) == 0) {
        a.refbits[g >> 5] = static_cast<uint32_t>(m);
        a.refbits[(g >> 5) + 1] = static_cast<uint32_t>(m >> 32);
    }
    if (blockIdx.x == 0 && static_cast<int>(threadIdx.x) < a.state_words) a.state[threadIdx.x] = a.host_state[threadIdx.x];
    const size_t nthreads = static_cast<size_t>(gridDim.x) * 256;
#pragma unroll
    for (int k = 0; k < 3; ++k)
        for (size_t i = static_cast<size_t>(g); i < a.zero_n[k]; i += nthreads) a.zero[k][i] = 0;
}

__device__ __forceinline__ void tally_word(uint32_t cl, uint32_t ch, uint32_t tl, uint32_t th, uint32_t m,
                                           uint32_t (&c)[kRaw])
{
    cl &= m; ch &= m; tl &= m; th &= m;
    c[0] += __popc(cl); c[1] += __popc(ch); c[2] += __popc(tl); c[3] += __popc(th);
    c[4] += __popc(cl & tl); c[5] += __popc(cl & th); c[6] += __popc(ch & tl); c[7] += __popc(ch & th);
}

__device__ __forceinline__ void tally_rows(const uint4 *__restrict__ table, const uint4 *__restrict__ refbits, int G, int Wq,
                                           int32_t *__restrict__ raw)
{
    const int lane = threadIdx.x & 63;
    const int row = blockIdx.x * 4 + (threadIdx.x >> 6);
    if (row >= G) return;
    const uint4 *r = table + static_cast<size_t>(row) * kPlanes * Wq;
    uint32_t c[kRaw] = {0, 0, 0, 0, 0, 0, 0, 0};
    for (int q = lane; q < Wq; q += 64) {
        const uint4 m = refbits[q];
        const uint4 cl = r[q], ch = r[Wq + q], tl = r[2 * Wq + q], th = r[3 * Wq + q];
        tally_word(cl.x, ch.x, tl.x, th.x, m.x, c);
        tally_word(cl.y, ch.y, tl.y, th.y, m.y, c);
        tally_word(cl.z, ch.z, tl.z, th.z, m.z, c);
        tally_word(cl.w, ch.w, tl.w, th.w, m.w, c);
    }
#pragma unroll
    for (int t = 0; t < kRaw; ++t) {
        uint32_t v = c[t];
#pragma unroll
        for (int o = 32; o > 0; o >>= 1) v += __shfl_xor(v, o, 64);
        c[t] = v;
    }
    if (lane == 0) {
        int4 *o = reinterpret_cast<int4 *>(raw + static_cast<size_t>(row) * kRaw);
        o[0] = make_int4(c[0], c[1], c[2], c[3]);
        o[1] = make_int4(c[4], c[5], c[6], c[7]);
    }
}

template <bool COH, int U = 4>
__device__ __forceinline__ void delta_counts(const uint32_t *__restrict__ table, int Wp, const uint32_t *list, int n, int i, int (&d)[kRaw])
{
    const int w = i >> 5, sh = i & 31;
#pragma unroll
    for (int q = 0; q < kRaw; ++q) d[q] = 0;
    for (int e0 = 0; e0 < n; e0 += U) {
        uint32_t ent[U], w0[U], w1[U], w2[U], w3[U];
#pragma unroll
        for (int u = 0; u < U; ++u) ent[u] = ldc<COH>(list + min(e0 + u, n - 1));
#pragma unroll
        for (int u = 0; u < U; ++u) {
            if (U > 4 && e0 + u >= n) { w0[u] = w1[u] = w2[u] = w3[u] = 0; continue; }
            const uint32_t *row = table + static_cast<size_t>(ent[u] >> 1) * kPlanes * Wp + w;
            w0[u] = row[0]; w1[u] = row[Wp]; w2[u] = row[2 * Wp]; w3[u] = row[3 * Wp];
        }
#pragma unroll
        for (int u = 0; u < U; ++u) {
            if (e0 + u >= n) continue;
            const int sgn = (ent[u] & 1u) ? 1 : -1;
            const int cl = (w1[u] >> sh) & 1, ch = (w0[u] >> sh) & 1;
            const int tl = (w3[u] >> sh) & 1, th = (w2[u] >> sh) & 1;
            d[0] += sgn * cl; d[1] += sgn * ch; d[2] += sgn * tl; d[3] += sgn * th;
            d[4] += sgn * (cl & tl); d[5] += sgn * (cl & th); d[6] += sgn * (ch & tl); d[7] += sgn * (ch & th);
        }
    }
}

__device__ __forceinline__ void delta_counts_block(const uint32_t *__restrict__ table, int Wp, const uint32_t *list, int n, int (&d)[kRaw], uint4 *buf)
{
    static_assert(kDeltaMax <= 255 && kDeltaMax * 32 <= 256 * 16, "8-bit fields; at most 16 fetches per thread");
    const int items = n * 32;
    uint32_t v[16];
#pragma unroll
    for (int k = 0; k < 16; ++k) {
        const int id = threadIdx.x + 256 * k;
        v[k] = 0;
        if (id < items) {
            const uint32_t ent = list[id >> 5];
            v[k] = table[(static_cast<size_t>(ent >> 1) * kPlanes + ((id >> 3) & 3)) * Wp + blockIdx.x * 8 + (id & 7)];
        }
    }
#pragma unroll
    for (int k = 0; k < 16; ++k) {
        const int id = threadIdx.x + 256 * k;
        if (id < items) reinterpret_cast<uint32_t *>(buf)[((id >> 5) * 8 + (id & 7)) * 4 + ((id >> 3) & 3)] = v[k];
    }
    lds_barrier();
    const int wi = threadIdx.x >> 5, sh = threadIdx.x & 31;
    uint32_t accA[2] = {0, 0}, accB[2] = {0, 0}, accX[2] = {0, 0};
#pragma unroll 4
    for (int e = 0; e < n; ++e) {
        const uint4 w = buf[e * 8 + wi];
        const uint32_t A = ((w.y >> sh) & 1u) | (((w.x >> sh) & 1u) << 16);
        const uint32_t B = ((w.w >> sh) & 1u) | (((w.z >> sh) & 1u) << 8);
        const int s = list[e] & 1u;
        accA[s] += A; accB[s] += B; accX[s] += A * B;
    }
    auto f = [](uint32_t x, int at) { return static_cast<int>((x >> at) & 0xFFu); };
    d[0] = f(accA[1], 0) - f(accA[0], 0);  d[1] = f(accA[1], 16) - f(accA[0], 16);
    d[2] = f(accB[1], 0) - f(accB[0], 0);  d[3] = f(accB[1], 8) - f(accB[0], 8);
    d[4] = f(accX[1], 0) - f(accX[0], 0);  d[5] = f(accX[1], 8) - f(accX[0], 8);
    d[6] = f(accX[1], 16) - f(accX[0], 16); d[7] = f(accX[1], 24) - f(accX[0], 24);
}

__device__ __forceinline__ void delta_gene(const uint32_t *__restrict__ table, int Wp, const uint32_t *__restrict__ list,
                                           int n, int32_t *__restrict__ raw, int i)
{
    int d[kRaw];
    delta_counts<false>(table, Wp, list, n, i, d);
    int4 *o = reinterpret_cast<int4 *>(raw + static_cast<size_t>(i) * kRaw);
    int4 a = o[0], b = o[1];
    a.x += d[0]; a.y += d[1]; a.z += d[2]; a.w += d[3];
    b.x += d[4]; b.y += d[5]; b.z += d[6]; b.w += d[7];
    o[0] = a; o[1] = b;
}

__device__ __forceinline__ void delta_genes(const uint32_t *__restrict__ table, int G, int Wp, const uint32_t *__restrict__ list,
                                            int n, int32_t *__restrict__ raw)
{
    const int i = blockIdx.x * 256 + threadIdx.x;
    if (i < G) delta_gene(table, Wp, list, n, raw, i);
}

struct IterArgs {
    IterState *st;
    const uint32_t *table;
    int G, Gp, Wp;
    int n_iter, n_conv;
    int a0, b0;
    double pval_deg, padj_deg;
    uint32_t *refbits[2];
    uint8_t *refbytes[2];
    int32_t *raw;
    uint32_t *delta_list;
    double *result;
    double *chunk_v; uint16_t *chunk_i; double *chunk_spl;
    double *sorted_d; double *sorted_spl; double *sorted_p;
    uint32_t *rank_s; uint32_t *rank_a;
    double *part; double *blockmin; double *scal;
    int32_t *trace; int32_t *modes;
    double *cand;
    int32_t *hist;
    int hist_stride;
    int32_t *mrank;
    int replay;
    int k2_idx;
    int xcc_local;
    int32_t *olist;
    int hist_below;
    uint8_t *snap;
    int32_t *clist; int band;
    int window, light_min_g;
    unsigned long long *stamps;
    IterState *host_st;
};

#ifdef REO_STAMPS
#define STAMP(a, k) do { if (blockIdx.x == 0 && threadIdx.x == 0) (a).stamps[k] = __builtin_amdgcn_s_memrealtime(); } while (0)
#else
#define STAMP(a, k) do { } while (0)
#endif

__device__ __forceinline__ void raise_fault(const IterArgs &a, int code)
{
    a.st->fault = code;
    if (a.host_st) a.host_st->fault = code;
}

constexpr int kCandMax = 64;
constexpr int kWindow = 24;
constexpr int kLightMinG = 4096;

__device__ __forceinline__ bool full_pass_active(const IterArgs &a, int &t, int &nref)
{
    const IterState *st = a.st;
    if (a.replay) { t = st->passes - 1; nref = st->nref_prev; return t >= 0; }
    t = st->passes; nref = st->nref;
    return !st->done && st->passes < a.n_iter && st->need_full;
}

__global__ __launch_bounds__(256) void k2_tally(IterArgs a)
{
    int t, nref;
    if (!full_pass_active(a, t, nref) || a.st->raw_pass == t) return;
    const int cur = t & 1;
    const int n = a.st->delta_cnt[cur];
    const bool full = n > kDeltaMax;
    if (a.modes && blockIdx.x == 0 && threadIdx.x == 0) a.modes[a.k2_idx] = full ? 1 : 0;
    if (full) tally_rows(reinterpret_cast<const uint4 *>(a.table), reinterpret_cast<const uint4 *>(a.refbits[cur]), a.G, a.Wp / 4, a.raw);
    else if (static_cast<int>(blockIdx.x) * 256 < a.G) delta_genes(a.table, a.G, a.Wp, a.delta_list + static_cast<size_t>(cur) * a.Gp, n, a.raw);
}

__global__ __launch_bounds__(256) void k2_scan(const uint32_t *__restrict__ table, const uint4 *__restrict__ refbits, int G, int Wp,
                                               int32_t *__restrict__ raw)
{
    tally_rows(reinterpret_cast<const uint4 *>(table), refbits, G, Wp / 4, raw);
}

template <bool FULL>
__device__ __forceinline__ void mccullagh3(const int32_t *n, double *out)
{
    const long long n12 = n[1], n13 = n[2], n21 = n[3], n23 = n[5], n31 = n[6], n32 = n[7];
    const long long a = n12 + n13 + n21 + n31;
    const long long b = n13 + n31;
    const long long d = n13 + n23 + n31 + n32;
    const long long R1 = n12 + n13, R2 = n13 + n23;
    const long long det = a * d - b * b;
    const double fa = static_cast<double>(a), fd = static_cast<double>(d);
    double w1 = 0.0, w2 = 0.0;
    if (det != 0) {
        const double fdet = static_cast<double>(det);
        w1 = static_cast<double>(d * (a - b)) / fdet;
        w2 = static_cast<double>(a * (d - b)) / fdet;
    } else {
        bool singular = b == 0;
        if (!singular) {
            const double B = fa, inv = 1.0 / B, l = B * inv;
            const double u = B - B * l;
            singular = u == 0.0 || fabs(B * u) <= 2.220446049250313e-16;
            if (!singular) {
                const double inv2 = 1.0 / u;
                const double i10 = (0.0 - l) * inv2, i11 = inv2;
                const double i00 = inv - l * i10, i01 = 0.0 - l * i11;
                w1 = i00 * B + i01 * B;
                w2 = i10 * B + i11 * B;
            }
        }
        if (singular) { out[0] = 1.0; out[1] = out[2] = out[3] = out[4] = 0.0; return; }
    }
    const double nu = 1.0 / (fa * w1 + fd * w2);
    const double r1 = static_cast<double>(R1), r2 = static_cast<double>(R2);
    const double d1 = (fa * w1 * nu) * log((r1 + 0.5) / (fa - r1 + 0.5)) +
                      (fd * w2 * nu) * log((r2 + 0.5) / (fd - r2 + 0.5));
    out[1] = d1;
    if (!FULL) return;
    const double A = w1 * r1 + w2 * r2, B = w1 * (fa - r1) + w2 * (fd - r2);
    const double d2 = log((0.5 + A) / (0.5 + B));
    const double v1 = 4.0 * (1.0 + 0.25 * d1 * d1) * nu;
    const double v2 = 4.0 * (1.0 + 0.25 * d2 * d2) * nu;
    const double se = sqrt((v1 + v2) * 0.5);
    const double z1 = d1 / se;
    double p = erfc(fabs(z1) * 0.70710678118654752440);
    out[0] = p > 1.0 ? 1.0 : p;
    out[2] = d2; out[3] = se; out[4] = z1;
}

__global__ void k_mccullagh(const int32_t *__restrict__ cont, int64_t n, double *__restrict__ out)
{
    const int64_t i = static_cast<int64_t>(blockIdx.x) * blockDim.x + threadIdx.x;
    if (i >= n) return;
    int32_t c[9];
    for (int t = 0; t < 9; ++t) c[t] = cont[i * 9 + t];
    double o[5];
    mccullagh3<true>(c, o);
    for (int t = 0; t < 5; ++t) out[i * 5 + t] = o[t];
}

__device__ __forceinline__ bool tallies_from(const int4 &r0, const int4 &r1, int total, int32_t (&c)[9])
{
    const int cLt = r0.x, cHt = r0.y, tLt = r0.z, tHt = r0.w, LL = r1.x, LH = r1.y, HL = r1.z, HH = r1.w;
    c[0] = LL; c[2] = LH; c[6] = HL; c[8] = HH;
    c[1] = cLt - LL - LH;
    c[7] = cHt - HL - HH;
    c[3] = tLt - LL - HL;
    c[5] = tHt - LH - HH;
    c[4] = total - (cLt + cHt + c[3] + c[5]);
    return (c[0] | c[1] | c[2] | c[3] | c[4] | c[5] | c[6] | c[7] | c[8]) >= 0;
}

__device__ __forceinline__ bool tallies_of(const int32_t *__restrict__ raw, bool in_ref, int nref, int i, int32_t (&c)[9])
{
    const int4 r0 = reinterpret_cast<const int4 *>(raw)[2 * i], r1 = reinterpret_cast<const int4 *>(raw)[2 * i + 1];
    return tallies_from(r0, r1, nref - (in_ref ? 1 : 0), c);
}


__global__ __launch_bounds__(256) void k3_tallies(const int32_t *__restrict__ raw, const uint8_t *__restrict__ refbytes, int nref, int G,
                                                  int32_t *__restrict__ cont)
{
    const int i = blockIdx.x * 256 + threadIdx.x;
    if (i >= G) return;
    int32_t c[9];
    tallies_of(raw, refbytes[i] != 0, nref, i, c);
#pragma unroll
    for (int t = 0; t < 9; ++t) cont[static_cast<size_t>(i) * 9 + t] = c[t];
}

__global__ __launch_bounds__(256) void k3_derive(IterArgs a)
{
    int t, nref;
    if (!full_pass_active(a, t, nref)) return;
    const int cur = t & 1;
    const int i = blockIdx.x * 256 + threadIdx.x;
    if (i == 0 && !a.replay) {
        a.st->delta_cnt[1 - cur] = 0;
        a.st->raw_pass = t;
    }
    if (i >= a.G) return;
    int32_t c[9];
    const bool ok = tallies_of(a.raw, a.refbytes[cur][i] != 0, nref, i, c);
    double o[5] = {1.0, 0.0, 0.0, 0.0, 0.0};
    if (ok) mccullagh3<true>(c, o);
    if (!ok || !(fabs(o[1]) < INFINITY)) {
        o[0] = 1.0; o[1] = o[2] = o[3] = o[4] = 0.0;
        raise_fault(a, kFaultTallies);
    }
    const size_t Gs = a.G;
    double *result = a.result;
    result[i] = o[0];
    result[Gs + i] = 1.0;
#pragma unroll
    for (int q = 0; q < 9; ++q) result[(2 + q) * Gs + i] = static_cast<double>(c[q]);
    result[11 * Gs + i] = o[1]; result[12 * Gs + i] = o[2];
    result[13 * Gs + i] = o[3]; result[14 * Gs + i] = o[4];
}

__device__ __forceinline__ double block_sum_256(double v, double *red)
{
#pragma unroll
    for (int o = 32; o > 0; o >>= 1) v += __shfl_xor(v, o, 64);
    if ((threadIdx.x & 63) == 0) red[threadIdx.x >> 6] = v;
    lds_barrier();
    const double r = (red[0] + red[1]) + (red[2] + red[3]);
    lds_barrier();
    return r;
}

__device__ __forceinline__ void block_sum2_256(double v, double w, double *red, double &rv, double &rw)
{
#pragma unroll
    for (int o = 32; o > 0; o >>= 1) { const double pv = __shfl_xor(v, o, 64), pw = __shfl_xor(w, o, 64); v += pv; w += pw; }
    if ((threadIdx.x & 63) == 0) { red[threadIdx.x >> 6] = v; red[4 + (threadIdx.x >> 6)] = w; }
    lds_barrier();
    rv = (red[0] + red[1]) + (red[2] + red[3]);
    rw = (red[4] + red[5]) + (red[6] + red[7]);
    lds_barrier();
}


template <int J>
__device__ __forceinline__ int lane_xor_b32(int v)
{
    if constexpr (J == 1) return __builtin_amdgcn_update_dpp(0, v, 0xB1, 0xF, 0xF, true);
    else if constexpr (J == 2) return __builtin_amdgcn_update_dpp(0, v, 0x4E, 0xF, 0xF, true);
    else if constexpr (J < 32) return __builtin_amdgcn_ds_swizzle(v, (J << 10) | 0x1F);
    else return __shfl_xor(v, J, 64);
}
template <int J>
__device__ __forceinline__ double lane_xor(double x)
{
    const long long b = __double_as_longlong(x);
    const int lo = lane_xor_b32<J>(static_cast<int>(b)), hi = lane_xor_b32<J>(static_cast<int>(b >> 32));
    return __longlong_as_double((static_cast<long long>(hi) << 32) | static_cast<unsigned int>(lo));
}

__device__ __forceinline__ void cmpx(double &v, uint32_t &i, double pv, uint32_t pi, bool keep_min)
{
    const bool take = ((pv < v) & keep_min) | ((pv > v) & !keep_min);
    v = take ? pv : v;
    i = take ? pi : i;
}

__global__ __launch_bounds__(kSortChunk) void k3_sort_chunks(IterArgs a)
{
    int tp, nref;
    if (!full_pass_active(a, tp, nref)) return;
    __shared__ double sv[kSortChunk];
    __shared__ uint16_t si[kSortChunk];
    const double *d1 = a.result + 11 * static_cast<size_t>(a.G);
    const int t = threadIdx.x, base = blockIdx.x * kSortChunk;
    double v = base + t < a.G ? d1[base + t] : INFINITY;
    uint32_t id = t;
    for (int k = 2; k <= kSortChunk; k <<= 1) {
        const bool up = (t & k) == 0;
        for (int j = k >> 1; j >= 64; j >>= 1) {
            lds_barrier();
            sv[t] = v; si[t] = static_cast<uint16_t>(id);
            lds_barrier();
            cmpx(v, id, sv[t ^ j], si[t ^ j], ((t & j) == 0) == up);
        }
        const int j0 = (k >> 1) < 32 ? (k >> 1) : 32;
        auto stage = [&](auto J) {
            constexpr int jj = decltype(J)::value;
            const double pv = lane_xor<jj>(v);
            const uint32_t pi = static_cast<uint32_t>(lane_xor_b32<jj>(static_cast<int>(id)));
            cmpx(v, id, pv, pi, ((t & jj) == 0) == up);
        };
        if (j0 >= 32) stage(std::integral_constant<int, 32>{});
        if (j0 >= 16) stage(std::integral_constant<int, 16>{});
        if (j0 >= 8) stage(std::integral_constant<int, 8>{});
        if (j0 >= 4) stage(std::integral_constant<int, 4>{});
        if (j0 >= 2) stage(std::integral_constant<int, 2>{});
        stage(std::integral_constant<int, 1>{});
    }
    a.chunk_v[base + t] = v; a.chunk_i[base + t] = static_cast<uint16_t>(id);
    if ((t & 31) == 0) a.chunk_spl[blockIdx.x * (kSortChunk / 32) + (t >> 5)] = v;
}

struct Range { int l, h; };

template <int LOG>
__device__ __forceinline__ Range coarse_range(const double *spl, int nspl, int n, double v, bool strict)
{
    int lo = 0, hi = nspl;
    while (lo < hi) { const int m = (lo + hi) >> 1; const double w = spl[m]; if (strict ? (w < v) : (w <= v)) lo = m + 1; else hi = m; }
    if (lo == 0) return Range{0, 0};
    return Range{((lo - 1) << LOG) + 1, min(n, lo << LOG)};
}

__device__ __forceinline__ void halve(Range &r, double w, double v, bool strict)
{
    if (r.l < r.h) { const int m = (r.l + r.h) >> 1; if (strict ? (w < v) : (w <= v)) r.l = m + 1; else r.h = m; }
}

constexpr int kMergeLanes = 16;
constexpr int kMergeThreads = 256;
constexpr int kSplit = kSortChunk / 32;

__global__ __launch_bounds__(kMergeThreads) void k3_merge_rank(IterArgs a, int nchunk)
{
    int tp, nref;
    if (!full_pass_active(a, tp, nref)) return;
    const int G = a.G;
    const double *cv = a.chunk_v;
    __shared__ double slice[kMergeThreads / kMergeLanes];
    extern __shared__ double spl[];
    for (int t = threadIdx.x; t < nchunk * kSplit; t += kMergeThreads) spl[t] = a.chunk_spl[t];
    __syncthreads();
    const int e = blockIdx.x * (kMergeThreads / kMergeLanes) + threadIdx.x / kMergeLanes;
    const int sub = threadIdx.x % kMergeLanes;
    const int c = e / kSortChunk, p = e % kSortChunk;
    const bool live = e < nchunk * kSortChunk;
    const int gene = live ? c * kSortChunk + a.chunk_i[e] : G;
    const double v = live ? cv[e] : 0.0;
    int count = 0;
    if (gene < G) {
        for (int cc = sub; cc < nchunk; cc += 2 * kMergeLanes) {
            const int c2 = cc + kMergeLanes;
            const bool on1 = cc != c, on2 = c2 < nchunk && c2 != c;
            const int n1 = min(kSortChunk, G - cc * kSortChunk), n2 = on2 ? min(kSortChunk, G - c2 * kSortChunk) : 0;
            const bool s1 = cc > c, s2 = c2 > c;
            Range r1 = on1 ? coarse_range<5>(spl + cc * kSplit, (n1 + 31) >> 5, n1, v, s1) : Range{0, 0};
            Range r2 = on2 ? coarse_range<5>(spl + c2 * kSplit, (n2 + 31) >> 5, n2, v, s2) : Range{0, 0};
            const double *ch1 = cv + cc * kSortChunk, *ch2 = cv + (on2 ? c2 : cc) * kSortChunk;
#pragma unroll
            for (int step = 0; step < 5; ++step) {
                const double w1 = ch1[min((r1.l + r1.h) >> 1, kSortChunk - 1)], w2 = ch2[min((r2.l + r2.h) >> 1, kSortChunk - 1)];
                halve(r1, w1, v, s1); halve(r2, w2, v, s2);
            }
            count += r1.l + r2.l;
        }
    }
#pragma unroll
    for (int o = kMergeLanes >> 1; o > 0; o >>= 1) count += __shfl_xor(count, o, 64);
    bool in = false;
    if (sub == 0 && gene < G) {
        const int rank = min(p + count, G - 1);
        a.rank_s[gene] = rank;
        a.sorted_d[rank] = v;
        if ((rank & 63) == 0) a.sorted_spl[rank >> 6] = v;
        in = rank >= a.a0 && rank <= a.b0;
    }
    if (sub == 0) slice[threadIdx.x / kMergeLanes] = in ? v : NAN;
    __syncthreads();
    if (threadIdx.x < 64) {
        constexpr int kElems = kMergeThreads / kMergeLanes;
        static_assert(kElems <= 64, "one wave reduces the workgroup's slice values");
        const double x = static_cast<int>(threadIdx.x) < kElems ? slice[threadIdx.x] : NAN;
        const bool has = x == x;
        double n = has ? 1.0 : 0.0, sum = has ? x : 0.0;
#pragma unroll
        for (int o = 32; o > 0; o >>= 1) { n += __shfl_xor(n, o, 64); sum += __shfl_xor(sum, o, 64); }
        const double mean = n > 0.0 ? sum / n : 0.0;
        double m2 = has ? (x - mean) * (x - mean) : 0.0;
#pragma unroll
        for (int o = 32; o > 0; o >>= 1) m2 += __shfl_xor(m2, o, 64);
        if (threadIdx.x == 0) { a.part[3 * blockIdx.x] = n; a.part[3 * blockIdx.x + 1] = mean; a.part[3 * blockIdx.x + 2] = m2; }
    }
}

__device__ __forceinline__ void combine_moments(const double *__restrict__ part, int npart, double *red, double &n, double &mean, double &m2)
{
    double nb = 0.0, sb = 0.0;
    for (int t = threadIdx.x; t < npart; t += 256) { const double n_ = part[3 * t]; nb += n_; sb += n_ * part[3 * t + 1]; }
    n = block_sum_256(nb, red);
    mean = block_sum_256(sb, red) / n;
    double qb = 0.0;
    for (int t = threadIdx.x; t < npart; t += 256) {
        const double n_ = part[3 * t], d_ = part[3 * t + 1] - mean;
        qb += part[3 * t + 2] + n_ * d_ * d_;
    }
    m2 = block_sum_256(qb, red);
}

__device__ __forceinline__ double normal_p(double v, double se)
{
    if (se == 0.0) return 0.0;
    const double p = erfc(fabs(v) / se * 0.70710678118654752440);
    return p > 1.0 ? 1.0 : p;
}

__global__ __launch_bounds__(256) void k3_abs_rank(IterArgs a, int npart)
{
    int tp, nref;
    if (!full_pass_active(a, tp, nref)) return;
    const int G = a.G;
    const double *sorted_d = a.sorted_d;
    __shared__ double red[256];
    extern __shared__ double spl[];
    const int nspl = (G + 63) >> 6;
    for (int t = threadIdx.x; t < nspl; t += 256) spl[t] = a.sorted_spl[t];
    double n, mean, m2;
    combine_moments(a.part, npart, red, n, mean, m2);
    const double se = sqrt(m2 / (n - 1.0));
    if (blockIdx.x == 0 && threadIdx.x == 0) a.scal[0] = se;
    const int i = blockIdx.x * 256 + threadIdx.x;
    if (i >= G) return;
    const double v = a.result[11 * static_cast<size_t>(G) + i];
    const int r = a.rank_s[i];
    Range r1 = coarse_range<6>(spl, nspl, G, v, true), r2 = coarse_range<6>(spl, nspl, G, -v, false),
          r3 = coarse_range<6>(spl, nspl, G, v, false);
#pragma unroll
    for (int step = 0; step < 6; ++step) {
        const double w1 = sorted_d[min((r1.l + r1.h) >> 1, G - 1)], w2 = sorted_d[min((r2.l + r2.h) >> 1, G - 1)],
                     w3 = sorted_d[min((r3.l + r3.h) >> 1, G - 1)];
        halve(r1, w1, v, true); halve(r2, w2, -v, false); halve(r3, w3, v, false);
    }
    const int lbv = r1.l, ubn = r2.l, ubv = r3.l;
    int rank;
    if (v > 0.0) {
        rank = (G - ubv) + ubn + (r - lbv);
    } else {
        rank = lbv + (G - ubn) + (r - lbv);
    }
    rank = min(max(rank, 0), G - 1);
    a.rank_a[i] = rank;
    const double p = normal_p(v, se);
    a.result[i] = p;
    a.sorted_p[rank] = p;
}

__global__ __launch_bounds__(1024) void k3_bh_local(IterArgs a)
{
    int tp, nref;
    if (!full_pass_active(a, tp, nref)) return;
    const int G = a.G;
    __shared__ double wmin[16];
    const int r = blockIdx.x * 1024 + threadIdx.x;
    const int lane = threadIdx.x & 63, wave = threadIdx.x >> 6;
    double v = r < G ? a.sorted_p[r] * (static_cast<double>(G) / static_cast<double>(r + 1)) : INFINITY;
#pragma unroll
    for (int o = 1; o < 64; o <<= 1) {
        const double w = __shfl_down(v, o, 64);
        if (lane + o < 64) v = w < v ? w : v;
    }
    if (lane == 0) wmin[wave] = v;
    __syncthreads();
    double t = INFINITY;
    for (int k = wave + 1; k < 16; ++k) { const double w = wmin[k]; t = w < t ? w : t; }
    v = t < v ? t : v;
    if (r < G) a.sorted_p[r] = v;
    if (threadIdx.x == 0) a.blockmin[blockIdx.x] = v;
}

__device__ __forceinline__ int publish_mask(const IterArgs &a, int t, int i, bool ind, bool in_cut)
{
    IterState *st = a.st;
    const int cur = t & 1, nxt = 1 - cur;
    if (i < a.Gp) a.refbytes[nxt][i] = ind ? 1 : 0;
    const bool changed = i < a.G && ind != (a.refbytes[cur][i] != 0);
    const unsigned long long cm = __ballot(changed);
    if (cm) {
        int basepos = 0;
        if ((threadIdx.x & 63) == 0) basepos = atomicAdd(&st->delta_cnt[nxt], __popcll(cm));
        basepos = __shfl(basepos, 0, 64);
        const int at = basepos + __popcll(cm & ((1ULL << (threadIdx.x & 63)) - 1ULL));
        if (changed && at < kDeltaMax) a.delta_list[static_cast<size_t>(nxt) * a.Gp + at] = (static_cast<uint32_t>(i) << 1) | (ind ? 1u : 0u);
    }
    const unsigned long long m = __ballot(ind), mc = __ballot(in_cut);
    __shared__ int wave_nn[4], wave_kc[4];
    if ((threadIdx.x & 63) == 0) {
        if (i < a.Gp) {
            a.refbits[nxt][i >> 5] = static_cast<uint32_t>(m);
            a.refbits[nxt][(i >> 5) + 1] = static_cast<uint32_t>(m >> 32);
        }
        wave_nn[threadIdx.x >> 6] = __popcll(m);
        wave_kc[threadIdx.x >> 6] = __popcll(mc);
    }
    __syncthreads();
    if (threadIdx.x != 0) return -1;
    const int nn_blk = wave_nn[0] + wave_nn[1] + wave_nn[2] + wave_nn[3];
    if (nn_blk) atomicAdd(&st->nn_acc, nn_blk);
    const int kc_blk = wave_kc[0] + wave_kc[1] + wave_kc[2] + wave_kc[3];
    if (kc_blk) atomicAdd(&st->kcut_acc, kc_blk);
    __threadfence();
    const int tk = atomicAdd(&st->ticket, 1);
    if (tk != static_cast<int>(gridDim.x) - 1) return -1;
    __threadfence();
    const int nn = atomicAdd(&st->nn_acc, 0);
    a.trace[2 * t] = a.G - nn;
    a.trace[2 * t + 1] = nn;
    st->passes = t + 1;
    st->cyc_pow = 0;
    st->nref_prev = st->nref;
    const int diff = st->nref - nn;
    if ((diff < 0 ? -diff : diff) < a.n_conv) {
        st->done = 1;
    } else {
        st->i_iter += 1;
        st->nref = nn;
    }
    st->last_full = 1;
    st->kstar = atomicAdd(&st->kcut_acc, 0);
    st->kcut_acc = 0;
    st->nn_acc = 0;
    st->ticket = 0;
    return atomicAdd(&st->delta_cnt[nxt], 0) > kDeltaMax ? 1 : 0;
}

__global__ __launch_bounds__(256) void k3_finalize(IterArgs a)
{
    int t, nref;
    if (!full_pass_active(a, t, nref)) return;
    const int G = a.G;
    constexpr int kMaxBlocks = (kMaxGenes + 1023) / 1024;
    __shared__ double tail[kMaxBlocks + 1];
    const int nb = (G + 1023) / 1024;
    __shared__ double bm[kMaxBlocks];
    for (int b = threadIdx.x; b < nb; b += 256) bm[b] = a.blockmin[b];
    __syncthreads();
    for (int b = threadIdx.x; b <= nb; b += 256) {
        double run = INFINITY;
        for (int k = b + 1; k < nb; ++k) { const double m = bm[k]; run = m < run ? m : run; }
        tail[b] = run;
    }
    __syncthreads();
    const int i = blockIdx.x * 256 + threadIdx.x;
    bool ind = false, in_cut = false;
    if (i < G) {
        const uint32_t r = a.rank_a[i];
        double q = a.sorted_p[r];
        const double tl = tail[r >> 10];
        q = tl < q ? tl : q;
        q = q < 1.0 ? q : 1.0;
        a.result[static_cast<size_t>(G) + i] = q;
        in_cut = q <= a.padj_deg;
        ind = !(a.result[i] <= a.pval_deg && in_cut);
    }
    if (a.replay) return;
    const int over = publish_mask(a, t, i, ind, in_cut);
    if (over < 0) return;
    const int W = a.window;
    bool ok = G >= a.light_min_g && a.a0 - W >= 0 && a.b0 + W < G && a.a0 + W < a.b0 - W;
    if (ok) {
        const double va = a.sorted_d[a.a0], vb = a.sorted_d[a.b0];
        const double wa_lo = a.sorted_d[a.a0 - W], wa_hi = a.sorted_d[a.a0 + W];
        const double wb_lo = a.sorted_d[a.b0 - W], wb_hi = a.sorted_d[a.b0 + W];
        ok = wa_hi < wb_lo;
        a.scal[1] = wa_lo; a.scal[2] = wa_hi; a.scal[3] = wb_lo; a.scal[4] = wb_hi;
        a.scal[5] = va - wa_lo; a.scal[6] = wa_hi - va; a.scal[7] = vb - wb_lo; a.scal[8] = wb_hi - vb;
    }
    a.st->need_full = (over || !ok) ? 1 : 0;
    if (a.host_st) {
        IterState *h = a.host_st;
        h->passes = t + 1; h->done = a.st->done; h->need_full = (over || !ok) ? 1 : 0; h->last_full = 1;
        h->delta_cnt[(t + 1) & 1] = a.st->delta_cnt[(t + 1) & 1];
    }
}


template <int K, int J>
__device__ __forceinline__ void sort_stage(double &x, int t)
{
    const bool up = (t & K) == 0 || K == 64;
    const bool keep_min = ((t & J) == 0) == up;
    const double px = lane_xor<J>(x);
    const bool take = ((px < x) & keep_min) | ((px > x) & !keep_min);
    x = take ? px : x;
}
__device__ __forceinline__ double sort64(double x)
{
    const int t = threadIdx.x & 63;
    sort_stage<2, 1>(x, t);
    sort_stage<4, 2>(x, t); sort_stage<4, 1>(x, t);
    sort_stage<8, 4>(x, t); sort_stage<8, 2>(x, t); sort_stage<8, 1>(x, t);
    sort_stage<16, 8>(x, t); sort_stage<16, 4>(x, t); sort_stage<16, 2>(x, t); sort_stage<16, 1>(x, t);
    sort_stage<32, 16>(x, t); sort_stage<32, 8>(x, t); sort_stage<32, 4>(x, t); sort_stage<32, 2>(x, t); sort_stage<32, 1>(x, t);
    sort_stage<64, 32>(x, t); sort_stage<64, 16>(x, t); sort_stage<64, 8>(x, t); sort_stage<64, 4>(x, t); sort_stage<64, 2>(x, t); sort_stage<64, 1>(x, t);
    return x;
}

__device__ __forceinline__ double wave_sum(double v)
{
    v += lane_xor<32>(v); v += lane_xor<16>(v); v += lane_xor<8>(v); v += lane_xor<4>(v); v += lane_xor<2>(v); v += lane_xor<1>(v);
    return v;
}

template <bool COH>
__device__ __forceinline__ int bh_cut(const int32_t *hist, int G, int rmax)
{
    __shared__ __attribute__((aligned(16))) int wsum[16][4];
    __shared__ int wbest[4];
    const int lane = threadIdx.x & 63, wave = threadIdx.x >> 6;
    const int ntile = (min(G, max(rmax, 1)) + 2047) / 2048;
    int best = 0, carry = 0;
    for (int q0 = 0; q0 < ntile; q0 += 16) {
        int hv[16][8];
        int s[16], inc[16];
#pragma unroll
        for (int e = 0; e < 16; ++e) {
            const size_t o = (static_cast<size_t>(q0 + e) * 256 + threadIdx.x) * 8;
            if (q0 + e >= ntile) {
#pragma unroll
                for (int u = 0; u < 8; ++u) hv[e][u] = 0;
            } else if (COH) {
#pragma unroll
                for (int u = 0; u < 4; ++u) {
                    const unsigned long long w = __hip_atomic_load(reinterpret_cast<const unsigned long long *>(hist + o) + u, __ATOMIC_RELAXED, __HIP_MEMORY_SCOPE_AGENT);
                    hv[e][2 * u] = static_cast<int>(w & 0xFFFFFFFFull); hv[e][2 * u + 1] = static_cast<int>(w >> 32);
                }
            } else {
                const int4 h0 = reinterpret_cast<const int4 *>(hist + o)[0], h1 = reinterpret_cast<const int4 *>(hist + o)[1];
                hv[e][0] = h0.x; hv[e][1] = h0.y; hv[e][2] = h0.z; hv[e][3] = h0.w; hv[e][4] = h1.x; hv[e][5] = h1.y; hv[e][6] = h1.z; hv[e][7] = h1.w;
            }
        }
#pragma unroll
        for (int e = 0; e < 16; ++e) {
            s[e] = ((hv[e][0] + hv[e][1]) + (hv[e][2] + hv[e][3])) + ((hv[e][4] + hv[e][5]) + (hv[e][6] + hv[e][7]));
            inc[e] = s[e];
        }
        const int nt = min(16, ntile - q0);
#pragma unroll
        for (int o = 1; o < 64; o <<= 1)
#pragma unroll
            for (int e = 0; e < 16; ++e)
                if (e < nt) { const int u = __shfl_up(inc[e], o, 64); if (lane >= o) inc[e] += u; }
        if (lane == 63)
#pragma unroll
            for (int e = 0; e < 16; ++e) wsum[e][wave] = inc[e];
        __syncthreads();
        int4 ws[16];
#pragma unroll
        for (int e = 0; e < 16; ++e) ws[e] = *reinterpret_cast<const int4 *>(wsum[e]);
#pragma unroll
        for (int e = 0; e < 16; ++e) {
            int run = carry + inc[e] - s[e] + (wave > 0 ? ws[e].x : 0) + (wave > 1 ? ws[e].y : 0) + (wave > 2 ? ws[e].z : 0);
            const int r0 = ((q0 + e) * 256 + threadIdx.x) * 8 + 1;
#pragma unroll
            for (int u = 0; u < 8; ++u) { run += hv[e][u]; if (r0 + u <= G && run >= r0 + u) best = max(best, r0 + u); }
            carry += ws[e].x + ws[e].y + ws[e].z + ws[e].w;
        }
        __syncthreads();
    }
#pragma unroll
    for (int o = 32; o > 0; o >>= 1) { const int u = __shfl_xor(best, o, 64); best = u > best ? u : best; }
    if (lane == 0) wbest[wave] = best;
    __syncthreads();
    const int k = max(max(wbest[0], wbest[1]), max(wbest[2], wbest[3]));
    __syncthreads();
    return k;
}

__device__ __forceinline__ int bh_rank(double p, int G, double al)
{
    const double Gd = static_cast<double>(G);
    auto within = [&](int r) { return p * (Gd / static_cast<double>(r)) <= al; };
    if (!within(G)) return G + 1;
    const double est = ceil(p * Gd / al);
    int m = est < 1.0 ? 1 : (est > Gd ? G : static_cast<int>(est));
    while (m > 1 && within(m - 1)) --m;
    while (!within(m)) ++m;
    return m;
}

__device__ __forceinline__ bool slice_std_vals(const IterArgs &a, double x, const double (&pn)[kPartPer], const double (&pm)[kPartPer], const double (&pq)[kPartPer],
                                               int below_a, int below_b, int cnt_a, int cnt_b, double (*sel)[4], double *red, double &se, double &va, double &vb)
{
    const int ia = a.a0 - below_a, ib = a.b0 - below_b;
    if (!(cnt_a <= kCandMax && cnt_b <= kCandMax && ia >= 0 && ia < cnt_a && ib >= 0 && ib < cnt_b)) return false;
    const int lane = threadIdx.x & 63, wave = threadIdx.x >> 6;
    if (wave < 2) {
        const int cnt = wave ? cnt_b : cnt_a, pos = wave ? ib : ia;
        x = sort64(lane < cnt ? x : INFINITY);
        const bool in = wave ? lane <= pos : (lane >= pos && lane < cnt);
        const double n = static_cast<double>(wave ? pos + 1 : cnt - pos);
        const double mean = wave_sum(in ? x : 0.0) / n;
        const double q = wave_sum(in ? (x - mean) * (x - mean) : 0.0);
        const double stat = __shfl(x, pos, 64);
        if (lane == 0) { sel[wave][0] = stat; sel[wave][1] = n; sel[wave][2] = mean; sel[wave][3] = q; }
    }
    double n0, mean0, sn = 0.0, sm = 0.0;
#pragma unroll
    for (int u = 0; u < kPartPer; ++u) { sn += pn[u]; sm += pn[u] * pm[u]; }
    block_sum2_256(sn, sm, red, n0, mean0);
    mean0 /= n0;
    double sq = 0.0;
#pragma unroll
    for (int u = 0; u < kPartPer; ++u) sq += pq[u] + pn[u] * (pm[u] - mean0) * (pm[u] - mean0);
    double q0 = block_sum_256(sq, red);
    va = sel[0][0]; vb = sel[1][0];
    const double n1 = sel[0][1], mean1 = sel[0][2], q1 = sel[0][3], n2 = sel[1][1], mean2 = sel[1][2], q2 = sel[1][3];
    lds_barrier();
    if (!(n0 > 0.0)) { mean0 = 0.0; q0 = 0.0; }
    const double n = n0 + n1 + n2;
    const double mean = (n0 * mean0 + n1 * mean1 + n2 * mean2) / n;
    const double m2 = (q0 + n0 * (mean0 - mean) * (mean0 - mean)) + (q1 + n1 * (mean1 - mean) * (mean1 - mean)) +
                      (q2 + n2 * (mean2 - mean) * (mean2 - mean));
    se = sqrt(m2 / (n - 1.0));
    return static_cast<int>(n) == a.b0 - a.a0 + 1;
}

constexpr int kPartLane = kListWgs / 64;
__device__ __forceinline__ bool slice_std_split(const IterArgs &a, double x, const double (&pn)[kPartLane], const double (&pm)[kPartLane], const double (&pq)[kPartLane],
                                                int below_a, int below_b, int cnt_a, int cnt_b, double (*sel)[4], double &se, double &va, double &vb)
{
    const int ia = a.a0 - below_a, ib = a.b0 - below_b;
    if (!(cnt_a <= kCandMax && cnt_b <= kCandMax && ia >= 0 && ia < cnt_a && ib >= 0 && ib < cnt_b)) return false;
    const int lane = threadIdx.x & 63, wave = threadIdx.x >> 6;
    if (wave < 2) {
// ... 1787 lines not shown
        if (!c->table_prezeroed) REO_HIP_CHECK(hipMemsetAsync(c->table.p, 0, static_cast<size_t>(c->G) * kPlanes * c->Wp * sizeof(uint32_t), c->stream));
        c->table_prezeroed = false;
    }
    if (units.empty()) return REO_OK;
    c->last_k1_shared = pl.shared ? 1 : 0;
    if (k1_slots_wanted(c, pl, sides, keep_table, gate, range, prepare) && c->k1_items_n) {
        if (k1_slots_alloc(c) == REO_OK) pl.slots = true;
        else (void)hipGetLastError();
    }
    if (!(pl.slots && c->k1_slot_slice) && (rc = ensure_planes(c))) return rc;
    if (a.stamps) k_time_mark<<<1, 64, 0, c->stream>>>(a.stamps + c->k1_items_n * 4);
    tic(c, 1);
    const int slot_sides = !pl.slots ? 0 : (c->k1_unslot == 0 ? 1 : slot_sides_wanted(a.ce - a.cb, a.te - a.tb, c->k1_slot_sides));
    if (pl.slots && (rc = k1_slots_front(c, a, slot_sides))) { toc(c); return rc; }
    dispatch_pairs(c, a, pl);
    if (pl.slots && (rc = k1_slots_back(c, a, slot_sides))) { toc(c); return rc; }
    toc(c);
    if (pl.slots) {
        c->last_k1_slots = 1; c->last_k1_slot_sides = slot_sides;
        c->k1_slot_items = a.items; c->k1_slot_items_n = c->k1_items_n; c->k1_slot_gp = a.Gp;
    }
    if (a.stamps) k_time_mark<<<1, 64, 0, c->stream>>>(a.stamps + c->k1_items_n * 4 + 1);
    REO_HIP_CHECK(hipGetLastError());
    if (a.stamps) return report_k1_stamps(c, a.stamps);
    return REO_OK;
}


int64_t exchange_unit_words(const reo_ctx *c) { return static_cast<int64_t>(kUnitRows) * kPlanes * (c->k1_q * c->k1_cj / 32); }
int32_t exchange_units_per_rank(const reo_ctx *c)
{
    const int total = static_cast<int>(c->units_all_host.size()), world = std::max(c->world, 1);
    return std::max(1, (total + world - 1) / world);
}

static int32_t upload_units_all(reo_ctx *c)
{
    int32_t rc;
    const size_t total = c->units_all_host.size();
    if ((rc = c->units_all.ensure(std::max<size_t>(total, 1)))) return rc;
    if (total && (c->units_all.p != c->units_all_uploaded || c->units_all_host != c->units_all_dev)) {
        REO_HIP_CHECK(hipMemcpyAsync(c->units_all.p, c->units_all_host.data(), total * sizeof(uint32_t), hipMemcpyHostToDevice, c->stream));
        REO_HIP_CHECK(hipStreamSynchronize(c->stream));
        c->units_all_dev = c->units_all_host;
        c->units_all_uploaded = c->units_all.p;
    }
    return REO_OK;
}

static int32_t exchange_args(reo_ctx *c, XArgs &a, int m0, int mcnt)
{
    const int32_t rc = upload_units_all(c);
    if (rc) return rc;
    a.table = c->table.p; a.units = c->units_all.p;
    a.G = static_cast<int>(c->G); a.Wp = c->Wp; a.Wc = c->k1_q * c->k1_cj / 32;
    a.total = static_cast<int>(c->units_all_host.size()); a.world = std::max(c->world, 1); a.rank = c->rank; a.maxu = exchange_units_per_rank(c);
    a.m0 = m0; a.mcnt = mcnt < 0 ? a.maxu : mcnt;
    return REO_OK;
}

int32_t launch_pack_units(reo_ctx *c, int m0, int mcnt, uint32_t *send, hipStream_t st)
{
    XArgs a;
    int32_t rc = exchange_args(c, a, m0, mcnt);
    if (rc) return rc;
    const size_t uw = static_cast<size_t>(exchange_unit_words(c));
    x_pack<<<dim3(static_cast<unsigned>((uw + 255) / 256), a.mcnt), 256, 0, st ? st : c->stream>>>(a, send ? send : c->xsend.p);
    REO_HIP_CHECK(hipGetLastError());
    return REO_OK;
}

int32_t launch_expand_units(reo_ctx *c, int m0, int mcnt, const uint32_t *recv, hipStream_t st)
{
    XArgs a;
    int32_t rc = exchange_args(c, a, m0, mcnt);
    if (rc) return rc;
    if (a.world < 2) return REO_OK;
    const size_t uw = static_cast<size_t>(exchange_unit_words(c));
    if (!st) st = c->stream;
    if (!recv) recv = c->xrecv.p;
    x_expand_fwd<<<dim3(static_cast<unsigned>((uw + 255) / 256), a.mcnt * a.world), 256, 0, st>>>(a, recv);
    x_expand_mirror<<<dim3(a.Wc, kPlanes, a.mcnt * a.world), 256, 0, st>>>(a, recv);
    REO_HIP_CHECK(hipGetLastError());
    return REO_OK;
}

int32_t launch_counts(reo_ctx *c, int64_t i0, int64_t i1, int64_t j0, int64_t j1, uint16_t *d_gt, uint16_t *d_eq)
{
    const int32_t rc = ensure_planes(c);
    if (rc) return rc;
    dim3 grid(static_cast<unsigned>((j1 - j0 + 255) / 256), static_cast<unsigned>(i1 - i0));
    const auto kernel = c->G > 65535 ? k1_counts<true> : k1_counts<false>;
    kernel<<<grid, 256, 0, c->stream>>>(c->pos.p, c->lo.p, c->hi.p, c->Gp, plane_bits(c->G), c->goff_dev.p, c->ngroups, static_cast<int>(i0),
                                        static_cast<int>(i1), static_cast<int>(j0), static_cast<int>(j1), d_gt, d_eq);
    REO_HIP_CHECK(hipGetLastError());
    return REO_OK;
}

int32_t launch_check_table(reo_ctx *c, int *bad)
{
    *bad = 0;
    int32_t rc = c->check_flag.ensure(1);
    if (rc) return rc;
    REO_HIP_CHECK(hipMemsetAsync(c->check_flag.p, 0, sizeof(int32_t), c->stream));
    const int G = static_cast<int>(c->G);
    k_check_table<<<(G + 3) / 4, 256, 0, c->stream>>>(c->table.p, G, c->Wp, c->check_flag.p);
    int32_t h = 0;
    REO_HIP_CHECK(hipMemcpyAsync(&h, c->check_flag.p, sizeof h, hipMemcpyDeviceToHost, c->stream));
    REO_HIP_CHECK(hipStreamSynchronize(c->stream));
    *bad = h;
    return REO_OK;
}

int32_t launch_decode(reo_ctx *c, int64_t i0, int64_t i1, int64_t j0, int64_t j1, uint8_t *d_code)
{
    dim3 grid(static_cast<unsigned>((j1 - j0 + 255) / 256), static_cast<unsigned>(i1 - i0));
    k_decode<<<grid, 256, 0, c->stream>>>(c->table.p, c->Wp, static_cast<int>(i0), static_cast<int>(i1),
                                          static_cast<int>(j0), static_cast<int>(j1), d_code);
    REO_HIP_CHECK(hipGetLastError());
    return REO_OK;
}

int32_t launch_pack_ref(reo_ctx *c, const uint8_t *d_bytes, uint32_t *d_bits)
{
    k_pack_ref<<<c->Gp / 256, 256, 0, c->stream>>>(d_bytes, c->Gp, d_bits);
    REO_HIP_CHECK(hipGetLastError());
    return REO_OK;
}

__global__ void k_cycle_skip(IterState *st, IterState *host_st, int32_t *trace, int skip, int period)
{
    const int T = st->passes;
    for (int u = T + static_cast<int>(threadIdx.x); u < T + skip; u += static_cast<int>(blockDim.x)) {
        const int src = T - period + (u - T) % period;
        trace[2 * u] = trace[2 * src]; trace[2 * u + 1] = trace[2 * src + 1];
    }
    __syncthreads();
    if (threadIdx.x != 0) return;
    st->passes = T + skip;
    if (st->raw_pass >= 0) st->raw_pass += skip;
    st->i_iter += skip;
    st->cyc_period = -1;
    if (host_st) { host_st->passes = T + skip; host_st->cyc_period = -1; }
}

int32_t launch_cycle_skip(reo_ctx *c, int skip, int period)
{
    if (skip < 0 || period < 1 || skip % period != 0 || (skip & 1)) { set_error("launch_cycle_skip: skip %d, period %d", skip, period); return REO_EINVAL; }
    k_cycle_skip<<<1, 256, 0, c->stream>>>(c->state.p, c->state_mirror ? c->host_state : nullptr, c->trace.p, skip, period);
    REO_HIP_CHECK(hipGetLastError());
    return REO_OK;
}

int32_t launch_iter_init(reo_ctx *c, const uint8_t *host_ref, const IterState *host_state)
{
    IterInitArgs a;
    a.host_ref = host_ref; a.host_state = reinterpret_cast<const uint32_t *>(host_state);
    a.refbytes = c->refbytes[0].p; a.refbits = c->refbits[0].p; a.state = reinterpret_cast<uint32_t *>(c->state.p);
    a.zero[0] = reinterpret_cast<uint32_t *>(c->result.p); a.zero_n[0] = static_cast<size_t>(c->G) * 15 * 2;
    a.zero[1] = reinterpret_cast<uint32_t *>(c->modes.p); a.zero_n[1] = c->modes.n;
    a.zero[2] = reinterpret_cast<uint32_t *>(c->hist.p); a.zero_n[2] = c->hist.n;
    a.G = static_cast<int>(c->G); a.Gp = c->Gp; a.state_words = static_cast<int>(sizeof(IterState) / 4);
    k_iter_init<<<c->Gp / 256, 256, 0, c->stream>>>(a);
    REO_HIP_CHECK(hipGetLastError());
    return REO_OK;
}

int32_t launch_tally(reo_ctx *c, int nref)
{
    const int G = static_cast<int>(c->G);
    tic(c, 2);
    k2_scan<<<(G + 3) / 4, 256, 0, c->stream>>>(c->table.p, reinterpret_cast<const uint4 *>(c->refbits[0].p), G, c->Wp, c->raw.p);
    toc(c);
    c->t_ms[4] += 1.0;
    k3_tallies<<<(G + 255) / 256, 256, 0, c->stream>>>(c->raw.p, c->refbytes[0].p, nref, G, c->cont.p);
    REO_HIP_CHECK(hipGetLastError());
    return REO_OK;
}

static IterArgs iter_args(reo_ctx *c, int replay)
{
    IterArgs a;
    a.st = c->state.p; a.table = c->table.p;
    a.G = static_cast<int>(c->G); a.Gp = c->Gp; a.Wp = c->Wp;
    a.n_iter = c->it_n_iter; a.n_conv = c->it_n_conv; a.a0 = c->it_a0; a.b0 = c->it_b0;
    a.pval_deg = c->it_pval_deg; a.padj_deg = c->it_padj_deg;
    for (int t = 0; t < 2; ++t) { a.refbits[t] = c->refbits[t].p; a.refbytes[t] = c->refbytes[t].p; }
    a.raw = c->raw.p; a.delta_list = c->delta_list.p; a.result = c->result.p;
    const int nchunk = (a.G + kSortChunk - 1) / kSortChunk;
    a.chunk_v = c->chunk_v.p; a.chunk_i = c->chunk_i.p;
    a.chunk_spl = c->chunk_v.p + static_cast<size_t>(nchunk) * kSortChunk;
    a.sorted_d = c->sorted_d.p; a.sorted_spl = c->sorted_d.p + ((c->G + 63) / 64) * 64;
    a.sorted_p = c->sorted_p.p; a.rank_s = c->rank_s.p; a.rank_a = c->rank_a.p;
    a.part = c->part.p; a.blockmin = c->blockmin.p; a.scal = c->scal.p;
    a.trace = c->trace.p; a.modes = nullptr;
    a.cand = c->cand.p; a.hist = c->hist.p; a.hist_stride = static_cast<int>(c->hist.n / (3 * kHistParts)); a.mrank = c->mrank.p;
    a.replay = replay; a.k2_idx = 0;
    a.clist = c->clist.p; a.olist = c->olist.p; a.band = c->light_band; a.hist_below = c->hist_below; a.snap = c->snap.p; a.xcc_local = c->xcc_local;
    a.window = c->light_window; a.light_min_g = (c->it_no_light || c->light_mode == 0) ? 0x7FFFFFFF : c->light_min_g;
    a.stamps = reinterpret_cast<unsigned long long *>(c->scal.p + 32);
    a.host_st = c->state_mirror ? c->host_state : nullptr;
    return a;
}

int32_t launch_full_pass(reo_ctx *c, bool replay)
{
    IterArgs a = iter_args(c, replay ? 1 : 0);
    const int G = a.G, nb = (G + 255) / 256;
    const int nchunk = (G + kSortChunk - 1) / kSortChunk;
    const int nmerge = (nchunk * kSortChunk + kMergeThreads / kMergeLanes - 1) / (kMergeThreads / kMergeLanes);
    if (!replay) {
        if (c->k2_idx < static_cast<int>(c->modes.n)) { a.modes = c->modes.p; a.k2_idx = c->k2_idx; }
        ++c->k2_idx;
        tic(c, 2);
        k2_tally<<<(G + 3) / 4, 256, 0, c->stream>>>(a);
        toc(c);
        c->t_ms[4] += 1.0;
    }
    k3_derive<<<nb, 256, 0, c->stream>>>(a);
    k3_sort_chunks<<<nchunk, kSortChunk, 0, c->stream>>>(a);
    const size_t spl_bytes = static_cast<size_t>(nchunk) * kSplit * sizeof(double);
    if (spl_bytes > (size_t(48) << 10))
        REO_HIP_CHECK(hipFuncSetAttribute(reinterpret_cast<const void *>(k3_merge_rank), hipFuncAttributeMaxDynamicSharedMemorySize, static_cast<int>(spl_bytes)));
    k3_merge_rank<<<nmerge, kMergeThreads, spl_bytes, c->stream>>>(a, nchunk);
    k3_abs_rank<<<nb, 256, static_cast<size_t>((G + 63) / 64) * sizeof(double), c->stream>>>(a, nmerge);
    k3_bh_local<<<(G + 1023) / 1024, 1024, 0, c->stream>>>(a);
    k3_finalize<<<c->Gp / 256, 256, 0, c->stream>>>(a);
    REO_HIP_CHECK(hipGetLastError());
    return REO_OK;
}

int32_t launch_light_persistent(reo_ctx *c)
{
    const IterArgs a = iter_args(c, 0);
    const unsigned nwg = static_cast<unsigned>(a.Gp / 256);
    REO_HIP_CHECK(hipMemsetAsync(c->gridbar.p, 0, sizeof(unsigned), c->stream));
    REO_HIP_CHECK(hipMemsetAsync(c->lstate.p, 0, 2 * sizeof(LightSlot), c->stream));
    kl_persist<<<nwg, 256, 0, c->stream>>>(a, c->lstate.p, c->gridbar.p);
    REO_HIP_CHECK(hipGetLastError());
    return REO_OK;
}

int32_t launch_light_batch(reo_ctx *c, int nlight)
{
    const IterArgs a = iter_args(c, 0);
    const int nb = (a.G + 255) / 256, nbp = a.Gp / 256;
    if (nlight < 1 || nlight > kLightBatch) { set_error("light batch of %d passes", nlight); return REO_EINVAL; }
    REO_HIP_CHECK(hipMemsetAsync(c->lstate.p, 0, static_cast<size_t>(nlight + 1) * sizeof(LightSlot), c->stream));
    if (c->it_light_form == 3) {
        REO_HIP_CHECK(hipMemsetAsync(c->hist.p, 0, static_cast<size_t>(kHistParts) * a.hist_stride * sizeof(int32_t), c->stream));
        for (int b = 0; b < nlight; ++b) kl_one<false><<<nbp, 256, 0, c->stream>>>(a, c->lstate.p, b);
        kl_one<true><<<nbp, 256, 0, c->stream>>>(a, c->lstate.p, nlight);
        REO_HIP_CHECK(hipGetLastError());
        return REO_OK;
    }
    for (int b = 0; b < nlight; ++b) {
        if (b < 2) kl_head<false, false><<<nbp, 256, 0, c->stream>>>(a, c->lstate.p, b);
        else kl_head<false, true><<<nbp, 256, 0, c->stream>>>(a, c->lstate.p, b);
        kl_rank<<<nb, 256, 0, c->stream>>>(a, c->lstate.p, b);
    }
    if (nlight < 2) kl_head<true, false><<<nbp, 256, 0, c->stream>>>(a, c->lstate.p, nlight);
    else kl_head<true, true><<<nbp, 256, 0, c->stream>>>(a, c->lstate.p, nlight);
    REO_HIP_CHECK(hipGetLastError());
    return REO_OK;
}

int32_t xcc_selftest(reo_ctx *c, int *ok)
{
    *ok = 0;
    DevBuf<int32_t> buf;
    static std::mutex mu;
    static int verdict[64];
    {
        std::lock_guard<std::mutex> lk(mu);
        if (c->device >= 0 && c->device < 64 && verdict[c->device]) { *ok = verdict[c->device] == 2; return REO_OK; }
    }
    int32_t rc = buf.ensure(kHistParts * 64 + kHistParts);
    if (rc) return rc;
    REO_HIP_CHECK(hipMemsetAsync(buf.p, 0xFF, buf.n * sizeof(int32_t), c->stream));
    k_xcc_selftest<<<1024, 256, 0, c->stream>>>(buf.p, buf.p + kHistParts * 64);
    k_xcc_selftest_zero<<<1024, 256, 0, c->stream>>>(buf.p, buf.p + kHistParts * 64);
    k_xcc_selftest<<<1024, 256, 0, c->stream>>>(buf.p, buf.p + kHistParts * 64);
    std::vector<int32_t> h(buf.n);
    REO_HIP_CHECK(hipMemcpyAsync(h.data(), buf.p, buf.n * sizeof(int32_t), hipMemcpyDeviceToHost, c->stream));
    REO_HIP_CHECK(hipStreamSynchronize(c->stream));
    int64_t waves = 0;
    bool good = true;
    for (int x = 0; x < kHistParts; ++x) {
        const int32_t w = h[kHistParts * 64 + x];
        waves += w;
        for (int l = 0; l < 64; ++l) good = good && h[x * 64 + l] == 16 * w;
    }
    *ok = good && waves == 1024 * 4 ? 1 : 0;
    {
        std::lock_guard<std::mutex> lk(mu);
        if (c->device >= 0 && c->device < 64) verdict[c->device] = *ok ? 2 : 1;
    }
    return REO_OK;
}

int32_t light_min_genes() { return kLightMinG; }
int32_t light_window() { return kWindow; }

int32_t launch_mccullagh(reo_ctx *c, const int32_t *d_cont, int64_t n, double *d_out)
{
    k_mccullagh<<<static_cast<unsigned>((n + 255) / 256), 256, 0, c->stream>>>(d_cont, n, d_out);
    REO_HIP_CHECK(hipGetLastError());
    return REO_OK;
}

}
```

rankcompv3.jl_amd/csrc/reo_internal.h:

```cpp
#pragma once

#include <hip/hip_runtime.h>

#include <cstdint>
#include <functional>
#include <string>
#include <type_traits>
#include <vector>

#include "reo_hip.h"

namespace reo {

constexpr int kTileJ = 256;
constexpr int kTileI = 32;
constexpr int kPlanes = 4;
constexpr int kUnitH = 32;
constexpr int kRJ = 4;
constexpr int kRJTies = 2;
constexpr int kMaxGenes = 262143;
constexpr int kGenePad = 1024;
constexpr int kRaw = 8;
constexpr int kDeltaMax = 128;
constexpr int kSortChunk = 1024;

struct IterState {
    int32_t done;
    int32_t passes;
    int32_t nref;
    int32_t i_iter;
    int32_t ticket;
    int32_t nn_acc;
    int32_t delta_cnt[2];
    int32_t need_full;
    int32_t raw_pass;
    int32_t nref_prev;
    int32_t last_full;
    int32_t fault;
    int32_t kstar;
    int32_t kcut_acc;
    int32_t cyc_period;
    int32_t cyc_pow;
    int32_t cyc_lam;
    int32_t cyc_sel;
    int32_t cyc_ndiff;
    int32_t pad[4];
};
constexpr int kFaultBarrier = 1;
constexpr int kFaultTallies = 2;

constexpr int kLightBatch = 128;
struct LightRec {
    int32_t active;
    int32_t t;
    int32_t nref, nref_prev, done, need_full, raw_pass;
    int32_t ran;
    int32_t dcnt;
    int32_t kstar;
    int32_t cper, cpow, clam, csel;
};
constexpr int kHistParts = 8;
constexpr int kSpread = 8;
constexpr int kListCap = 16;
constexpr int kListWgs = 1024;
static_assert(kMaxGenes <= kListWgs * 256, "the light passes' lists and block moments (clist, part) hold kListWgs workgroups of 256 genes");
constexpr int kPartPer = kListWgs / 256;
constexpr int kListStride = kListWgs + kListWgs * kListCap * 2;
constexpr int kOneListCap = 16;
constexpr int kOneListMax = 512;
constexpr int kOneStride = 256 + 256 * kOneListCap * 4;
struct LightCnt {
    int32_t cnt_a, cnt_b;
    int32_t pad[30];
    int32_t below_a[kSpread][32];
    int32_t below_b[kSpread][32];
    int32_t sig[kSpread][32];
    int32_t nsure[kSpread][32];
    int32_t nlow[kSpread][32];
};
struct LightSlot {
    LightRec rec;
    int32_t bfail;
    int32_t cdiff;
    int32_t cfound;
    int32_t pad0[5];
    double wnext[4];
    double se_base;
    double eta;
    double pad1[15];
    LightCnt lc;
};
struct LightState { LightSlot slot[kLightBatch + 2]; };
static_assert(sizeof(LightSlot) % 128 == 0, "LightSlot layout");

void set_error(const char *fmt, ...);

#define REO_HIP_CHECK(expr)                                                              \
    do {                                                                                 \
        hipError_t e_ = (expr);                                                          \
        if (e_ != hipSuccess) {                                                          \
            ::reo::set_error("%s failed: %s (%s:%d)", #expr, hipGetErrorString(e_),      \
                             __FILE__, __LINE__);                                        \
            return e_ == hipErrorOutOfMemory ? REO_ENOMEM : REO_EHIP;                    \
        }                                                                                \
    } while (0)

hipError_t pool_alloc(void **p, size_t bytes, bool pinned);
void pool_free(void *p, size_t bytes, bool pinned);
extern thread_local bool tl_release_synced;
hipError_t handle_stream(hipStream_t *s, int kind);
hipError_t handle_event(hipEvent_t *e, int kind);
void release_stream(hipStream_t s, int kind);
void release_event(hipEvent_t e, int kind);

template <class T>
struct DevBuf {
    T *p = nullptr;
    size_t n = 0;
    DevBuf() = default;
    DevBuf(const DevBuf &) = delete;
    DevBuf &operator=(const DevBuf &) = delete;
    ~DevBuf() { release(); }
    int32_t ensure(size_t count)
    {
        if (count <= n && p) return REO_OK;
        release();
        REO_HIP_CHECK(pool_alloc(reinterpret_cast<void **>(&p), count * sizeof(T), false));
        n = count;
        return REO_OK;
    }
    void release()
    {
        if (p) {
            if (!tl_release_synced) (void)hipDeviceSynchronize();
            pool_free(p, n * sizeof(T), false);
        }
        p = nullptr;
        n = 0;
    }
};

struct StageTimer {
    hipEvent_t a = nullptr, b = nullptr;
};

}

struct reo_ctx {
    int device = 0;
    hipStream_t stream = nullptr;
    uint64_t seed = 0;
    int rank = 0, world = 1;
    reo_allreduce_fn ar = nullptr;
    void *ar_user = nullptr;
    reo_allgather_fn ag = nullptr;
    void *ag_user = nullptr;

    int64_t G = 0, S = 0, ld = 0;
    int dtype = 0;
    const void *dX = nullptr;
    reo::DevBuf<unsigned char> dX_owned;
    std::vector<int32_t> group_id;
    int ngroups = 0;
    std::vector<int32_t> thr;
    bool thr_set = false;

    int Gp = 0, Wp = 0;
    std::vector<int32_t> goff;
    std::vector<int32_t> goff32;
    reo::DevBuf<uint4> pos;
    reo::DevBuf<uint4> lo;
    reo::DevBuf<uint4> hi;
    reo::DevBuf<uint16_t> t_pos16, t_lo16, t_hi16;
    reo::DevBuf<uint32_t> t_pos32, t_lo32, t_hi32;
    reo::DevBuf<uint32_t> t_vin32, t_vout32;
    reo::DevBuf<int32_t> goff_dev;
    reo::DevBuf<uint64_t> t_kin, t_kout;
    reo::DevBuf<uint16_t> t_vin, t_vout;
    reo::DevBuf<unsigned char> t_temp;
    reo::DevBuf<int32_t> t_order, t_flags, t_slots;
    reo::DevBuf<uint32_t> unit_map;
    std::vector<uint32_t> unit_map_host;
    std::vector<int32_t> t_order_host, t_slots_host, goff_blocks_host;
    const int32_t *t_meta_ptr[3] = {nullptr, nullptr, nullptr};
    int32_t *host_flags = nullptr;
    hipEvent_t ev_flags = nullptr;
    bool table_prezeroed = false;
    const uint32_t *unit_map_uploaded = nullptr;
    size_t k1_items_n = 0;
    bool transformed = false;
    int eager_mode = 2;
    int eager_chunk = 0;
    int eager_gate = 1;
    hipStream_t up = nullptr, rk = nullptr;
    hipEvent_t ev_up[8] = {nullptr};
    hipEvent_t ev_rk[4] = {nullptr, nullptr, nullptr, nullptr};
    reo::DevBuf<int32_t> e_lists;
    int upload_threads = 12;
    unsigned char *stage_h[3] = {nullptr, nullptr, nullptr};
    size_t stage_cap = 0;
    reo::DevBuf<unsigned char> stage_d[3];
    hipEvent_t ev_stage[3] = {nullptr, nullptr, nullptr}, ev_widen[3] = {nullptr, nullptr, nullptr};
    int64_t narrowed_bytes = 0;
    int rowmajor_upload = 0;
    int csc_upload = 0;
    int64_t csc_nnz = 0;
    reo::DevBuf<int64_t> csc_colptr;
    int csc_device = 0;
    bool eager_k1 = false;
    int has_ties = 0;
    int transform_in_lds = 0;

    reo::DevBuf<uint32_t> table;
    int built_k = -1;
    int built_treat = -1;
    bool table_complete = false;
    void *comm = nullptr;
    int spin_wait = 0;
    int check_hook_table = 1;
    bool comm_dead = false;
    bool in_multi = false;
    bool multi_one_device = false;
    std::vector<reo_ctx *> peers;
    reo::DevBuf<uint16_t> gcounts;
    bool gc_valid = false;
    int k1_wave = 1;
    int k1_order = 0;
    int k1_half = 1;
    int k1_slots = 1;
    int last_k1_slots = 0;
    int k1_unslot = -1;
    int k1_slot_sides = 0;
    int last_k1_slot_sides = 0;
    int last_k1_unslot = 0;
    int k1_unslot_attr = 0;
    const uint32_t *k1_slot_items = nullptr;
    size_t k1_slot_items_n = 0;
    int k1_slot_gp = 0;
    reo::DevBuf<uint32_t> k1_slot_part;
    reo::DevBuf<uint32_t> k1_slot_maps;
    reo::DevBuf<uint4> pos_s, lo_s;
    int k1_slot_slice = 1;
    int last_k1_slot_slice = 0;
    bool planes_ready = false;
    int planes_on_demand = 0;
    int k1_queue = 1;
    int k1_workers = 0;
    reo::DevBuf<uint32_t> k1_queue_ctr;
    int n_cus = 256;
    int share_counts = 1;
    int last_k1_shared = 0;
    int64_t tiles_owned = 0, tiles_total = 0;
    int k1_cj = 0, k1_q = 0;
    std::vector<uint32_t> units_all_host, units_all_dev;
    const uint32_t *units_all_uploaded = nullptr;
    reo::DevBuf<uint32_t> units_all, xsend, xrecv;
    int x_waves = 4;
    bool x_pipelined = false;
    hipStream_t k1s[2] = {nullptr, nullptr}, xs = nullptr;
    hipEvent_t ev_fork = nullptr, ev_k1[8] = {nullptr}, ev_k1_join[2] = {nullptr, nullptr}, ev_x = nullptr;
    struct ItemList { reo::DevBuf<uint32_t> buf; size_t n = 0; uint64_t key[5] = {0, 0, 0, 0, 0}; };
    ItemList k1_wave_items[8];
    reo::DevBuf<uint32_t> k1_park[2];
    reo::DevBuf<int32_t> k1_park_ge[2];
    int64_t eager_range_launches = 0;
    int eager_ranges = -1;
    reo::DevBuf<int32_t> check_flag;

    reo::DevBuf<uint32_t> refbits[2];
    reo::DevBuf<uint8_t> refbytes[2];
    int ref_slot = -1;
    const char *ref_gone = "reo_identify_degs has not run on this context";
    reo::DevBuf<int32_t> sc_slot2col;
    std::vector<int32_t> sc_slot2col_host;
    const int32_t *sc_slot2col_uploaded = nullptr;
    reo::DevBuf<double> st_lf;
    int64_t st_lf_G = -1;
    reo::DevBuf<uint8_t> vmask;
    bool vmask_set = false;
    int64_t vmask_G = 0, vmask_S = 0;
    reo::DevBuf<uint32_t> vwords;
    bool vwords_valid = false;
    reo::DevBuf<int32_t> mp_thr;
    std::vector<int32_t> mp_thr_host;
    int32_t mp_thr_n[2] = {-1, -1};
    double mp_thr_pval = -1.0;
    const int32_t *mp_thr_uploaded = nullptr;
    int built_masked = 0;
    int64_t perm_batch = 0;
    int64_t perm_kernel_us = 0;
    int64_t top_hist_us = 0;
    int64_t top_emit_us = 0;
    int64_t top_null_batch = 0;
    int64_t top_null_us = 0;
    int64_t top_loo_words_us = 0;
    int64_t top_loo_select_us = 0;
    int64_t top_partners_count_us = 0;
    int64_t top_partners_select_us = 0;
    reo::DevBuf<int32_t> raw;
    reo::DevBuf<uint32_t> delta_list;
    reo::DevBuf<int32_t> cont;
    reo::DevBuf<double> result;
    reo::DevBuf<double> sorted_d;
    reo::DevBuf<double> sorted_p;
    reo::DevBuf<uint32_t> rank_s, rank_a;
    reo::DevBuf<double> scal;
    reo::DevBuf<double> blockmin;
    reo::DevBuf<double> chunk_v;
    reo::DevBuf<uint16_t> chunk_i;
    reo::DevBuf<double> part;
    reo::DevBuf<reo::IterState> state;
    reo::DevBuf<int32_t> trace;
    reo::DevBuf<int32_t> modes;
    reo::DevBuf<double> cand;
    reo::DevBuf<unsigned> gridbar;
    reo::DevBuf<reo::LightState> lstate;
    reo::DevBuf<int32_t> clist;
    int light_band = 32;
    bool cycle_watch = true;
    reo::DevBuf<uint8_t> snap;
    int it_cycle_period = 0, it_cycle_at = 0, it_cycle_skipped = 0;
    int hist_below = 256;
    int xcc_local = 0;
    int light_window = 24, light_min_g = 4096;
    int light_mode = 1;
    reo::DevBuf<int32_t> olist;
    reo::DevBuf<int32_t> hist, mrank;
    double it_pval_deg = 1.0, it_padj_deg = 0.05;
    int it_n_iter = 0, it_n_conv = 0, it_a0 = 0, it_b0 = 0;
    int k2_idx = 0;
    int it_light_form = 1;
    bool it_no_light = false;
    reo::IterState *host_state = nullptr;
    bool state_mirror_wanted = true;
    bool debug_passes = false, debug_stamps = false, k1_stamps = false;
    bool state_mirror = false;
    uint8_t *host_ref = nullptr;
    size_t host_ref_cap = 0;

    bool profiling = false;
    double t_ms[REO_NTIMINGS] = {0};
    std::vector<std::pair<int, reo::StageTimer>> pending;
    std::vector<reo::StageTimer> pool;
    std::vector<size_t> open;
    std::vector<int32_t> k2_modes;
    size_t k2_seen = 0;
};

namespace reo {

int32_t run_transform(reo_ctx *c);
int32_t ensure_planes(reo_ctx *c);
enum { kLayoutColMajor = 0, kLayoutRowMajor = 1, kLayoutCsc = 2 };
int32_t eager_upload(reo_ctx *c, const void *hX, int64_t hld, bool with_k1, bool host_i32 = false, int layout = kLayoutColMajor);
int32_t upload_columns(reo_ctx *c, const void *hX, int64_t hld, int64_t G, int64_t ncols, void *dX, int dtype, int layout = kLayoutColMajor);
int32_t widen_device_i32(reo_ctx *c, const void *dX32, int64_t ld, int64_t G, int64_t S, void *dX64);
int32_t densify_device_csc(reo_ctx *c, int64_t G, int64_t S, const int64_t *colptr, const void *rows, int32_t index_bits, const void *vals,
                           int dtype, void *dX);
int32_t ensure_upload_streams(reo_ctx *c);
int32_t ensure_staging(reo_ctx *c, size_t slot_bytes);
void host_parallel(int nthreads, int ntasks, const std::function<void(int)> &fn);

struct K1Range { int b0, b1; bool first, last; };
int32_t launch_k1(reo_ctx *c, int k, int sides = 3, bool keep_table = false, const int32_t *gate = nullptr, const K1Range *range = nullptr,
                  bool prepare = false, int treat = -1);
int32_t k1_planes_fit(reo_ctx *c, bool *fit, size_t *need_bytes);
int64_t exchange_unit_words(const reo_ctx *c);
int32_t exchange_units_per_rank(const reo_ctx *c);
int32_t launch_pack_units(reo_ctx *c, int m0 = 0, int mcnt = -1, uint32_t *send = nullptr, hipStream_t st = nullptr);
int32_t launch_expand_units(reo_ctx *c, int m0 = 0, int mcnt = -1, const uint32_t *recv = nullptr, hipStream_t st = nullptr);
int32_t launch_slot_separated(reo_ctx *c, int64_t *half_tiles);
int32_t launch_counts(reo_ctx *c, int64_t i0, int64_t i1, int64_t j0, int64_t j1, uint16_t *d_gt, uint16_t *d_eq);
int32_t launch_check_table(reo_ctx *c, int *bad);
int32_t launch_decode(reo_ctx *c, int64_t i0, int64_t i1, int64_t j0, int64_t j1, uint8_t *d_code);
int32_t launch_pack_ref(reo_ctx *c, const uint8_t *d_bytes, uint32_t *d_bits);
int32_t launch_cycle_skip(reo_ctx *c, int skip, int period);
int32_t launch_iter_init(reo_ctx *c, const uint8_t *host_ref, const IterState *host_state);
int32_t launch_tally(reo_ctx *c, int nref);
int32_t launch_full_pass(reo_ctx *c, bool replay);
int32_t launch_light_persistent(reo_ctx *c);
int32_t launch_light_batch(reo_ctx *c, int nlight);
int32_t xcc_selftest(reo_ctx *c, int *ok);
int32_t light_min_genes();
int32_t light_window();
int32_t launch_mccullagh(reo_ctx *c, const int32_t *d_cont, int64_t n, double *d_out);

int plane_bits(int64_t G);
inline int32_t need_planes(reo_ctx *c, const char *what, int64_t max_genes)
{
    if (c->pos.p && c->lo.p && c->hi.p && c->goff_dev.p && !c->goff32.empty() && c->ngroups >= 1 && c->G <= max_genes) return ensure_planes(c);
    set_error("%s: no bit planes", what);
    return REO_EINVAL;
}
template <typename F>
void with_plane_bits(int64_t G, F &&f)
{
    switch (plane_bits(G)) {
    case 12: f(std::integral_constant<int, 12>{}); break;
    case 15: f(std::integral_constant<int, 15>{}); break;
    default: f(std::integral_constant<int, 16>{}); break;
    }
}
inline dim3 tile_grid(int64_t cols, int64_t rows, int tile_rows, int waves, int z = 1)
{
    const unsigned ctiles = static_cast<unsigned>((cols + 63) / 64);
    return dim3((ctiles + waves - 1) / waves, static_cast<unsigned>((rows + tile_rows - 1) / tile_rows), static_cast<unsigned>(z));
}

int32_t launch_pair_count(reo_ctx *c, const int32_t *d_genes, int64_t n_genes, const uint32_t *d_maskbits, uint32_t class_mask, int32_t *d_count);
int32_t launch_pair_fill(reo_ctx *c, const int32_t *d_genes, int64_t n_genes, const uint32_t *d_maskbits, uint32_t class_mask, const int64_t *d_rowptr,
                         int32_t *d_partner, uint8_t *d_code, int64_t capacity, int32_t *d_flag);

int32_t launch_sample_counts(reo_ctx *c, const int32_t *d_genes, int64_t n_queries, const uint32_t *d_maskbits, uint32_t class_mask,
                             const int32_t *d_slot2col, int32_t *d_sel, int32_t *d_gt, int32_t *d_eq);

int32_t launch_sample_fisher(reo_ctx *c, int64_t n_queries, const int32_t *d_sel_a, const int32_t *d_sel_b, const int32_t *d_gt_a,
                             const int32_t *d_eq_a, const int32_t *d_gt_b, const int32_t *d_eq_b, const double *d_lf, int64_t lf_entries,
                             int32_t *d_rev_up, int32_t *d_rev_down, int32_t *d_tied, double *d_p_up, double *d_p_down, int32_t *d_flag);

int32_t launch_call_rank(reo_ctx *c, int64_t n_genes, int64_t q0, int64_t nq, const double *d_p_up, const double *d_p_down, double pval_deg,
                         double padj_deg, uint32_t *d_words);
int32_t launch_call_cut(reo_ctx *c, int64_t n_genes, const uint32_t *d_words, int32_t *d_kstar, int32_t *d_cut, int32_t *d_n_up, int32_t *d_n_down);
int32_t launch_call_emit(reo_ctx *c, int64_t n_genes, const uint32_t *d_words, const int32_t *d_kstar, int8_t *d_calls);

struct PsItem;
int32_t launch_pair_support(reo_ctx *c, const PsItem *d_items, int64_t n_items, const int32_t *d_partner, const int32_t *d_slot2col,
                            int32_t *d_gt, int32_t *d_eq, uint8_t *d_outcome);

struct TpKey;
struct TpRec;
int32_t launch_rank_shift(reo_ctx *c, const int32_t *d_gside, int s_a, int s_b, int64_t *d_D, int64_t *d_sums = nullptr);
int32_t launch_top_hist(reo_ctx *c, const int32_t *d_gside, int s_a, int s_b, const int64_t *d_D, const uint32_t *d_maskbits, const TpKey &prefix,
                        int shift, unsigned long long *d_hist);
int32_t launch_top_emit(reo_ctx *c, const int32_t *d_gside, int s_a, int s_b, const int64_t *d_D, const uint32_t *d_maskbits, const TpKey &cut,
                        int shift, TpRec *d_cand, int64_t capacity, uint32_t *d_cand_n);

int32_t launch_top_null_words(reo_ctx *c, const uint8_t *d_side, int64_t n_perm, const int32_t *d_slot2col, uint32_t *d_aw, uint32_t *d_live);
int32_t launch_top_pairs_null(reo_ctx *c, const uint32_t *d_aw, const uint32_t *d_live, int np, int s_a, int s_b, const uint32_t *d_maskbits,
                              const int64_t *cuts, int n_cuts, unsigned long long *d_keys, unsigned long long *d_reach);

int32_t launch_loo_words(reo_ctx *c, const TpRec *d_cand, int64_t n_cand, uint2 *d_words);
int32_t launch_loo_select(reo_ctx *c, const TpRec *d_cand, int64_t n_cand, const uint2 *d_words, const int32_t *d_gside, const int32_t *d_slot2col,
                          const int64_t *d_sums, int s_a, int s_b, int kmax, int32_t *d_i, int32_t *d_j, int64_t *d_n, int64_t *d_g, int8_t *d_o);

int32_t launch_top_partners_count(reo_ctx *c, const int32_t *d_gside, int s_a, int s_b, const int32_t *d_genes, int64_t n_rows,
                                  unsigned long long *d_cells);
int32_t launch_top_partners_select(reo_ctx *c, const unsigned long long *d_cells, const int32_t *d_genes, int64_t n_rows, const int64_t *d_D,
                                   const uint32_t *d_maskbits, int s_a, int s_b, int m_want, int32_t *d_partner, int32_t *d_counts, int64_t *d_key,
                                   int32_t *d_found);

int32_t launch_valid_words(reo_ctx *c, const int32_t *d_slot2col);
int32_t launch_pairs_masked(reo_ctx *c, int k, const int32_t *d_m1, int n1, const int32_t *d_m2, int n2, int min_complete1, int min_complete2);
int32_t launch_counts_masked(reo_ctx *c, int64_t i0, int64_t i1, int64_t j0, int64_t j1, int32_t *d_gt, int32_t *d_eq, int32_t *d_avail);

int32_t launch_perm_words(reo_ctx *c, const uint8_t *d_side, int64_t n_perm, const int32_t *d_slot2col, uint32_t *d_aw, uint32_t *d_live);
int32_t launch_pairs_permuted(reo_ctx *c, const uint32_t *d_aw, const uint32_t *d_live, int np, int n1, int n2, int m1, int m2, uint32_t *d_tables);
int32_t launch_perm_accumulate(reo_ctx *c, const double *d_obs, double pval_deg, double padj_deg, int32_t *d_n_ge, int32_t *d_n_up, int32_t *d_n_down,
                               double *d_se);

int32_t pseudobulk_resident_dense(reo_ctx *c, const void *X, bool is_int, int64_t G, int64_t C, int64_t ld, const int32_t *order,
                                  int64_t n_order, const int32_t *chunk_ptr, int32_t n_out);
int32_t pseudobulk_resident_csc(reo_ctx *c, bool is_int, int64_t G, int64_t C, const int64_t *colptr, const int32_t *rowidx, const void *val,
                                const int32_t *order, int64_t n_order, const int32_t *chunk_ptr, int32_t n_out);
int32_t pseudobulk_device_dense(reo_ctx *c, int dtype, const void *dX, int64_t G, int64_t C, int64_t ld, const int32_t *order, int64_t n_order,
                                const int32_t *chunk_ptr, int32_t n_out);
int32_t pseudobulk_device_csc(reo_ctx *c, int dtype, int64_t G, int64_t C, int64_t nnz, const void *d_colptr, const void *d_rowidx,
                              int32_t index_bits, const void *d_val, const int32_t *order, int64_t n_order, const int32_t *chunk_ptr, int32_t n_out);
int32_t csc_device_check(reo_ctx *c, int64_t G, int64_t S, int64_t nnz, const void *d_colptr, const void *d_rowidx, int32_t index_bits,
                         const void *d_val, const int64_t **colptr64);
int32_t filter_matrix(reo_ctx *c, int64_t min_profiles, int64_t min_features, uint8_t *profile_kept, uint8_t *gene_kept,
                      int64_t *S_kept, int64_t *G_kept);

int32_t comm_allgather(reo_ctx *c, const void *send, void *recv, int64_t bytes_per_rank, hipStream_t st = nullptr);
void comm_release(reo_ctx *c);
void comm_abort(reo_ctx *c);
int32_t comm_wait(reo_ctx *c);
int32_t multi_build_pairs(reo_ctx *lead, int32_t k, int32_t (*build_local)(reo_ctx *, int32_t));

void tic(reo_ctx *c, int slot);
void toc(reo_ctx *c);
void collect_timings(reo_ctx *c);

int32_t use(reo_ctx *c);
int32_t no_multi(reo_ctx *c, const char *what);
int32_t need_complete_table(reo_ctx *c);
int32_t ensure_transform(reo_ctx *c);
int32_t wait_or_drop_table(reo_ctx *c);
bool mask_in_force(reo_ctx *c);
int32_t refuse_under_mask(reo_ctx *c, const char *what);
int32_t upload_slot2col(reo_ctx *c, const std::vector<int32_t> &map);
struct DrainOnExit {
    reo_ctx *c;
    bool armed = true;
    explicit DrainOnExit(reo_ctx *ctx) : c(ctx) {}
    DrainOnExit(const DrainOnExit &) = delete;
    DrainOnExit &operator=(const DrainOnExit &) = delete;
    void dismiss() { armed = false; }
    ~DrainOnExit()
    {
        if (!armed || !c || !c->stream) return;
        (void)hipStreamSynchronize(c->stream);
    }
};

}
```

Before: 52650 billion.

## Add row-list tally form for sparse reference sets in iterative pass

Adds a third k2 tally form that handles a sparse reference set (up to G/16 genes) by walking the list of reference genes in chunks, split across 16 slices. Each slice writes partial counts, and the pass kernel then sums them. This avoids scanning every bitplane word of the full table. The first pass now starts from a host-built list of reference genes, and the delta list may hold up to Gp entries instead of kDeltaMax. The cost is extra partial buffers, a larger k2 grid, and a reduction step inside the pass kernel.

```diff
diff --git a/rankcompv3.jl_amd/_ffi.py b/rankcompv3.jl_amd/_ffi.py
--- a/rankcompv3.jl_amd/_ffi.py
+++ b/rankcompv3.jl_amd/_ffi.py
@@ -1314,11 +1314,17 @@
         check(self._L.reo_get_timings(self._h, _ptr(ms), NTIMINGS))
         return {"transform_ms": ms[0], "k1_ms": ms[1], "k2_ms": ms[2], "iter_ms": ms[3], "k3_ms": max(ms[3] - ms[2], 0.0), "k2_launches": int(ms[4]),
                 "k1_launches": int(ms[5]), "exchange_ms": ms[6], "pseudobulk_ms": ms[7], "k2_full_ms": ms[8],
-                "k2_full_launches": int(ms[9]), "k2_delta_ms": ms[10], "set_matrix_host_wall_ms": ms[11]}
+                "k2_full_launches": int(ms[9]), "k2_delta_ms": ms[10], "set_matrix_host_wall_ms": ms[11],
+                "k2_rows_passes_last_call": self._k2_rows_passes()}
+
+    def _k2_rows_passes(self) -> int:
+        w = np.zeros(46, dtype=np.int64)
+        check(self._L.reo_get_info(self._h, _ptr(w), 46))
+        return int(w[44])
 
     def info(self) -> dict:
-        w = np.zeros(44, dtype=np.int64)
-        check(self._L.reo_get_info(self._h, _ptr(w), 44))
+        w = np.zeros(46, dtype=np.int64)
+        check(self._L.reo_get_info(self._h, _ptr(w), 46))
         v = np.zeros(28, dtype=np.int64)
         v[:] = w[:28]
         return {"G": int(v[0]), "S": int(v[1]), "Gp": int(v[2]), "table_bytes": int(v[3]), "has_ties": int(v[4]),
@@ -1335,4 +1341,5 @@
                 "top_pairs_hist_us": int(w[36]), "top_pairs_emit_us": int(w[37]),
                 "top_pairs_null_batch": int(w[38]), "top_pairs_null_us": int(w[39]),
                 "top_pairs_loo_words_us": int(w[40]), "top_pairs_loo_select_us": int(w[41]),
-                "top_partners_count_us": int(w[42]), "top_partners_select_us": int(w[43])}
+                "top_partners_count_us": int(w[42]), "top_partners_select_us": int(w[43]),
+                "k2_rows_mode": int(w[45])}
diff --git a/rankcompv3.jl_amd/csrc/api.hip b/rankcompv3.jl_amd/csrc/api.hip
--- a/rankcompv3.jl_amd/csrc/api.hip
+++ b/rankcompv3.jl_amd/csrc/api.hip
@@ -210,7 +210,7 @@
             c->t_ms[pr.first] += ms;
             if (pr.first == 2 && !c->k2_modes.empty()) {
                 if (c->k2_seen < c->k2_modes.size()) {
-                    if (c->k2_modes[c->k2_seen]) { c->t_ms[8] += ms; c->t_ms[9] += 1.0; }
+                    if (c->k2_modes[c->k2_seen] == 1) { c->t_ms[8] += ms; c->t_ms[9] += 1.0; }
                     else c->t_ms[10] += ms;
                 }
                 ++c->k2_seen;
@@ -442,7 +442,7 @@
         if ((rc = c->refbytes[t].ensure(c->Gp))) return rc;
     }
     if ((rc = c->raw.ensure(G * kRaw)) ||
-        (rc = c->delta_list.ensure(2 * static_cast<size_t>(c->Gp))) || (rc = c->cont.ensure(G * 9)) || (rc = c->result.ensure(G * 15)) ||
+        (rc = c->delta_list.ensure(2 * static_cast<size_t>(c->Gp))) || (rc = c->k2_part.ensure(static_cast<size_t>(kK2RowsSlices) * G * kRaw)) || (rc = c->cont.ensure(G * 9)) || (rc = c->result.ensure(G * 15)) ||
         (rc = c->sorted_d.ensure((G + 63) / 64 * 64 + (G + 63) / 64)) || (rc = c->sorted_p.ensure(G)) || (rc = c->rank_s.ensure(G)) ||
         (rc = c->rank_a.ensure(G)) || (rc = c->scal.ensure(8)) || (rc = c->blockmin.ensure(std::max<size_t>(64, (G + 1023) / 1024))) ||
         (rc = c->state.ensure(1)) ||
@@ -631,6 +631,7 @@
     if (const char *e = getenv("REO_LIGHT_BAND")) c->light_band = std::max(0, atoi(e));
     if (const char *e = getenv("REO_HIST_BELOW")) c->hist_below = std::max(0, atoi(e));
     if (const char *e = getenv("REO_CYCLE")) c->cycle_watch = atoi(e) != 0;
+    if (const char *e = getenv("REO_K2_ROWS")) c->k2_rows_mode = std::max(0, std::min(2, atoi(e)));
     if (const char *e = getenv("REO_LIGHT")) c->light_mode = e[0] == '0' ? 0 : (e[0] == '2' ? 2 : (e[0] == '3' ? 3 : 1));
     c->light_window = light_window(); c->light_min_g = light_min_genes();
     if (const char *e = getenv("REO_LIGHT_WINDOW")) c->light_window = std::max(1, std::min(31, atoi(e)));
@@ -698,7 +699,7 @@
     c->k1_slot_part.release(); c->k1_slot_maps.release(); c->pos_s.release(); c->lo_s.release(); c->k1_queue_ctr.release();
     c->t_pos32.release(); c->t_lo32.release(); c->t_hi32.release(); c->t_vin32.release(); c->t_vout32.release();
     for (int t = 0; t < 2; ++t) { c->refbits[t].release(); c->refbytes[t].release(); }
-    c->raw.release(); c->delta_list.release(); c->cont.release(); c->result.release(); c->sorted_d.release(); c->sorted_p.release();
+    c->raw.release(); c->delta_list.release(); c->k2_part.release(); c->cont.release(); c->result.release(); c->sorted_d.release(); c->sorted_p.release();
     c->rank_s.release(); c->rank_a.release(); c->scal.release(); c->blockmin.release();
     c->state.release(); c->trace.release(); c->modes.release(); c->cand.release(); c->hist.release(); c->mrank.release(); c->lstate.release(); c->clist.release(); c->olist.release(); c->units_all.release(); c->xsend.release(); c->xrecv.release(); c->check_flag.release(); c->gridbar.release(); c->chunk_v.release(); c->chunk_i.release(); c->part.release();
     if (c->host_state) pool_free(c->host_state, sizeof(IterState), true);
@@ -1287,20 +1288,28 @@
     if ((rc = c->modes.ensure(static_cast<size_t>(n_iter > 0 ? n_iter : 1) + 64))) return rc;
     for (const auto &pr : c->pending)
         if (pr.first == 2) { collect_timings(c); break; }
-    if (c->host_ref_cap < static_cast<size_t>(G)) {
+    const size_t ref_bytes = static_cast<size_t>(c->Gp) * (1 + sizeof(uint32_t));
+    if (c->host_ref_cap < ref_bytes) {
         if (c->host_ref) pool_free(c->host_ref, c->host_ref_cap, true);
         c->host_ref = nullptr; c->host_ref_cap = 0;
-        REO_HIP_CHECK(pool_alloc(reinterpret_cast<void **>(&c->host_ref), static_cast<size_t>(c->Gp), true));
-        c->host_ref_cap = static_cast<size_t>(c->Gp);
+        REO_HIP_CHECK(pool_alloc(reinterpret_cast<void **>(&c->host_ref), ref_bytes, true));
+        c->host_ref_cap = ref_bytes;
     }
     int32_t nref = 0;
-    for (int64_t i = 0; i < G; ++i) { c->host_ref[i] = ref0[i]; nref += ref0[i] != 0; }
+    uint32_t *host_list = reinterpret_cast<uint32_t *>(c->host_ref + c->Gp);
+    for (int64_t i = 0; i < G; ++i) {
+        c->host_ref[i] = ref0[i];
+        host_list[nref] = (static_cast<uint32_t>(i) << 1) | 1u;
+        nref += ref0[i] != 0;
+    }
+    const bool list0 = k2_rows_wanted(nref, static_cast<int>(G), c->k2_rows_mode);
     {
         IterState st;
         memset(&st, 0, sizeof st);
         st.nref = nref;
         st.nref_prev = nref;
-        st.delta_cnt[0] = st.delta_cnt[1] = 0x7FFFFFFF;
+        st.delta_cnt[0] = list0 ? nref : 0x7FFFFFFF;
+        st.delta_cnt[1] = 0x7FFFFFFF;
         st.need_full = 1;
         st.raw_pass = -1;
         st.kstar = -1;
@@ -1314,7 +1323,8 @@
     }
     c->it_cycle_period = 0; c->it_cycle_at = 0; c->it_cycle_skipped = 0;
     DrainOnExit drain(c);
-    if ((rc = launch_iter_init(c, c->host_ref, c->host_state))) return rc;
+    c->it_k2_rows = 0;
+    if ((rc = launch_iter_init(c, c->host_ref, c->host_state, host_list, list0 ? nref : 0))) return rc;
     c->it_pval_deg = pval_deg; c->it_padj_deg = padj_deg; c->it_n_iter = n_iter; c->it_n_conv = n_conv;
     c->it_a0 = static_cast<int>(a - 1); c->it_b0 = static_cast<int>(b - 1);
     c->k2_idx = 0;
@@ -1413,6 +1423,7 @@
         fprintf(stderr, "  (x 10 ns)\n");
     }
     if (iters_run) *iters_run = passes;
+    c->it_k2_rows = c->host_state->k2_rows_n;
     const double w_copy = c->debug_passes ? wall_us() : 0.0;
     REO_HIP_CHECK(hipMemcpyAsync(result, c->result.p, sizeof(double) * 15 * G, hipMemcpyDeviceToHost, c->stream));
     const double w_copied = c->debug_passes ? wall_us() : 0.0;
@@ -1670,7 +1681,7 @@
         int32_t rc = use(c);
         if (rc || (rc = launch_slot_separated(c, &separated))) return rc;
     }
-    const int64_t v[44] = {c->G, c->S, c->Gp, static_cast<int64_t>(c->table.n * sizeof(uint32_t)), c->has_ties,
+    const int64_t v[46] = {c->G, c->S, c->Gp, static_cast<int64_t>(c->table.n * sizeof(uint32_t)), c->has_ties,
                            c->tiles_owned, c->tiles_total, kTileI, c->k1_cj, c->k1_q, kUnitH,
                            c->goff32.empty() ? 0 : c->goff32.back(), c->last_k1_shared,
                            static_cast<int64_t>(c->gcounts.n * sizeof(uint16_t)), c->transform_in_lds, c->xcc_local,
@@ -1680,9 +1691,9 @@
                            c->last_k1_slots ? c->last_k1_slot_sides : 0, (c->built_k >= 0 && c->built_masked) ? 1 : 0,
                            c->last_k1_slots ? c->last_k1_slot_slice : 0, c->transformed ? c->planes_on_demand : 0, c->perm_batch, c->perm_kernel_us,
                            c->top_hist_us, c->top_emit_us, c->top_null_batch, c->top_null_us, c->top_loo_words_us, c->top_loo_select_us,
-                           c->top_partners_count_us, c->top_partners_select_us};
-    for (int i = 0; i < n && i < 44; ++i) info[i] = v[i];
-    return REO_OK;
-}
-
-}
+                           c->top_partners_count_us, c->top_partners_select_us, c->it_k2_rows, c->k2_rows_mode};
+    for (int i = 0; i < n && i < 46; ++i) info[i] = v[i];
+    return REO_OK;
+}
+
+}
diff --git a/rankcompv3.jl_amd/csrc/k2_rows.h b/rankcompv3.jl_amd/csrc/k2_rows.h
--- /dev/null
+++ b/rankcompv3.jl_amd/csrc/k2_rows.h
@@ -0,0 +1,54 @@
+#pragma once
+
+#include <cstdint>
+
+#if defined(__HIPCC__)
+#define REO_K2R_HD __host__ __device__
+#else
+#define REO_K2R_HD
+#endif
+
+namespace reo {
+
+constexpr int kK2DeltaMax = 128;
+constexpr int kK2RowsChunk = 128;
+constexpr int kK2RowsSlices = 16;
+constexpr int kK2RowsDen = 16;
+
+enum : int { kK2ModeScan = 0, kK2ModeRule = 1, kK2ModeRows = 2 };
+enum : int { kK2FormNone = 0, kK2FormScan = 1, kK2FormDelta = 2, kK2FormRows = 3 };
+
+REO_K2R_HD inline int k2_rows_chunks(int n) { return n <= 0 ? 0 : (n - 1) / kK2RowsChunk + 1; }
+REO_K2R_HD inline int k2_rows_chunk_len(int n, int c)
+{
+    const int left = n - c * kK2RowsChunk;
+    return c < 0 || left <= 0 ? 0 : (left < kK2RowsChunk ? left : kK2RowsChunk);
+}
+REO_K2R_HD inline int k2_rows_slices(int n)
+{
+    const int ch = k2_rows_chunks(n);
+    return ch < kK2RowsSlices ? ch : kK2RowsSlices;
+}
+
+REO_K2R_HD inline int k2_rows_cross(int G) { return G / kK2RowsDen; }
+
+REO_K2R_HD inline bool k2_rows_wanted(int n, int G, int mode)
+{
+    if (mode == kK2ModeScan || n < 0 || n > G) return false;
+    return mode == kK2ModeRows || n <= k2_rows_cross(G);
+}
+
+REO_K2R_HD inline int k2_form(int t, int n, int G, bool complete, int mode)
+{
+    if (t > 0 && n >= 0 && n <= kK2DeltaMax) return kK2FormDelta;
+    return complete && k2_rows_wanted(n, G, mode) ? kK2FormRows : kK2FormScan;
+}
+
+REO_K2R_HD inline int k2_rows_grid_x(int Gp) { return (Gp / 256 + 31) / 32 * 32; }
+REO_K2R_HD inline int k2_rows_grid(int Gp) { return k2_rows_grid_x(Gp) * kK2RowsSlices; }
+REO_K2R_HD inline int k2_rows_gene_block(int w_in_x)
+{
+    return (w_in_x & ~31) + (w_in_x & 7) * 4 + ((w_in_x >> 3) & 3);
+}
+
+}
diff --git a/rankcompv3.jl_amd/csrc/kernels.hip b/rankcompv3.jl_amd/csrc/kernels.hip
--- a/rankcompv3.jl_amd/csrc/kernels.hip
+++ b/rankcompv3.jl_amd/csrc/kernels.hip
@@ -1373,6 +1373,9 @@
     uint32_t *zero[3];
     size_t zero_n[3];
     int G, Gp, state_words;
+    const uint32_t *host_list;
+    uint32_t *list;
+    int list_n;
 };
 __global__ __launch_bounds__(256) void k_iter_init(IterInitArgs a)
 {
@@ -1385,6 +1388,7 @@
         a.refbits[(g >> 5) + 1] = static_cast<uint32_t>(m >> 32);
     }
     if (blockIdx.x == 0 && static_cast<int>(threadIdx.x) < a.state_words) a.state[threadIdx.x] = a.host_state[threadIdx.x];
+    if (g < a.list_n) a.list[g] = a.host_list[g];
     const size_t nthreads = static_cast<size_t>(gridDim.x) * 256;
 #pragma unroll
     for (int k = 0; k < 3; ++k)
@@ -1457,24 +1461,28 @@
     }
 }
 
-__device__ __forceinline__ void delta_counts_block(const uint32_t *__restrict__ table, int Wp, const uint32_t *list, int n, int (&d)[kRaw], uint4 *buf)
-{
-    static_assert(kDeltaMax <= 255 && kDeltaMax * 32 <= 256 * 16, "8-bit fields; at most 16 fetches per thread");
+template <int NF = 16>
+__device__ __forceinline__ void delta_counts_words(const uint32_t *__restrict__ table, int Wp, const uint32_t *list, int n, int (&d)[kRaw], uint4 *buf, int wbase)
+{
+    static_assert(kDeltaMax <= 255 && kDeltaMax * 32 <= 256 * 16 && 16 % NF == 0, "8-bit fields; at most 16 fetches per thread");
     const int items = n * 32;
-    uint32_t v[16];
-#pragma unroll
-    for (int k = 0; k < 16; ++k) {
-        const int id = threadIdx.x + 256 * k;
-        v[k] = 0;
-        if (id < items) {
-            const uint32_t ent = list[id >> 5];
-            v[k] = table[(static_cast<size_t>(ent >> 1) * kPlanes + ((id >> 3) & 3)) * Wp + blockIdx.x * 8 + (id & 7)];
-        }
-    }
-#pragma unroll
-    for (int k = 0; k < 16; ++k) {
-        const int id = threadIdx.x + 256 * k;
-        if (id < items) reinterpret_cast<uint32_t *>(buf)[((id >> 5) * 8 + (id & 7)) * 4 + ((id >> 3) & 3)] = v[k];
+#pragma unroll 1
+    for (int k0 = 0; k0 < 16; k0 += NF) {
+        uint32_t v[NF];
+#pragma unroll
+        for (int k = 0; k < NF; ++k) {
+            const int id = threadIdx.x + 256 * (k0 + k);
+            v[k] = 0;
+            if (id < items) {
+                const uint32_t ent = list[id >> 5];
+                v[k] = table[(static_cast<size_t>(ent >> 1) * kPlanes + ((id >> 3) & 3)) * Wp + wbase + (id & 7)];
+            }
+        }
+#pragma unroll
+        for (int k = 0; k < NF; ++k) {
+            const int id = threadIdx.x + 256 * (k0 + k);
+            if (id < items) reinterpret_cast<uint32_t *>(buf)[((id >> 5) * 8 + (id & 7)) * 4 + ((id >> 3) & 3)] = v[k];
+        }
     }
     lds_barrier();
     const int wi = threadIdx.x >> 5, sh = threadIdx.x & 31;
@@ -1492,6 +1500,11 @@
     d[2] = f(accB[1], 0) - f(accB[0], 0);  d[3] = f(accB[1], 8) - f(accB[0], 8);
     d[4] = f(accX[1], 0) - f(accX[0], 0);  d[5] = f(accX[1], 8) - f(accX[0], 8);
     d[6] = f(accX[1], 16) - f(accX[0], 16); d[7] = f(accX[1], 24) - f(accX[0], 24);
+}
+
+__device__ __forceinline__ void delta_counts_block(const uint32_t *__restrict__ table, int Wp, const uint32_t *list, int n, int (&d)[kRaw], uint4 *buf)
+{
+    delta_counts_words(table, Wp, list, n, d, buf, blockIdx.x * 8);
 }
 
 __device__ __forceinline__ void delta_gene(const uint32_t *__restrict__ table, int Wp, const uint32_t *__restrict__ list,
@@ -1524,6 +1537,8 @@
     uint8_t *refbytes[2];
     int32_t *raw;
     uint32_t *delta_list;
+    int32_t *k2_part;
+    int k2_rows_mode;
     double *result;
     double *chunk_v; uint16_t *chunk_i; double *chunk_spl;
     double *sorted_d; double *sorted_spl; double *sorted_p;
@@ -1570,16 +1585,50 @@
     return !st->done && st->passes < a.n_iter && st->need_full;
 }
 
-__global__ __launch_bounds__(256) void k2_tally(IterArgs a)
+__device__ __forceinline__ void k2_rows_block(const IterArgs &a, const uint32_t *__restrict__ list, int n)
+{
+    __shared__ uint32_t dl[kK2RowsChunk];
+    __shared__ uint4 dbuf[kK2RowsChunk * 8];
+    const int nx = k2_rows_grid_x(a.Gp), slices = k2_rows_slices(n), chunks = k2_rows_chunks(n);
+    const int slice = static_cast<int>(blockIdx.x) / nx;
+    const int gb = k2_rows_gene_block(static_cast<int>(blockIdx.x) % nx);
+    if (slice >= slices || gb >= a.Gp / 256) return;
+    int d[kRaw] = {0, 0, 0, 0, 0, 0, 0, 0};
+    for (int ch = slice; ch < chunks; ch += slices) {
+        const int len = k2_rows_chunk_len(n, ch);
+        if (static_cast<int>(threadIdx.x) < len) dl[threadIdx.x] = list[static_cast<size_t>(ch) * kK2RowsChunk + threadIdx.x];
+        lds_barrier();
+        int dd[kRaw];
+        delta_counts_words<4>(a.table, a.Wp, dl, len, dd, dbuf, gb * 8);
+#pragma unroll
+        for (int q = 0; q < kRaw; ++q) d[q] += dd[q];
+        lds_barrier();
+    }
+    const int i = gb * 256 + threadIdx.x;
+    if (i >= a.G) return;
+    int4 *o = reinterpret_cast<int4 *>(a.k2_part + (static_cast<size_t>(slice) * a.G + i) * kRaw);
+    o[0] = make_int4(d[0], d[1], d[2], d[3]);
+    o[1] = make_int4(d[4], d[5], d[6], d[7]);
+}
+
+__global__ __launch_bounds__(256, 8) void k2_tally(IterArgs a)
 {
     int t, nref;
-    if (!full_pass_active(a, t, nref) || a.st->raw_pass == t) return;
+    if (!full_pass_active(a, t, nref)) return;
+    const bool first = blockIdx.x == 0 && threadIdx.x == 0;
+    if (a.st->raw_pass == t) { if (first) a.st->k2_form = kK2FormNone; return; }
     const int cur = t & 1;
     const int n = a.st->delta_cnt[cur];
-    const bool full = n > kDeltaMax;
-    if (a.modes && blockIdx.x == 0 && threadIdx.x == 0) a.modes[a.k2_idx] = full ? 1 : 0;
-    if (full) tally_rows(reinterpret_cast<const uint4 *>(a.table), reinterpret_cast<const uint4 *>(a.refbits[cur]), a.G, a.Wp / 4, a.raw);
-    else if (static_cast<int>(blockIdx.x) * 256 < a.G) delta_genes(a.table, a.G, a.Wp, a.delta_list + static_cast<size_t>(cur) * a.Gp, n, a.raw);
+    const int form = k2_form(t, n, a.G, t == 0 || a.st->last_full != 0, a.k2_rows_mode);
+    if (first) {
+        a.st->k2_form = form | (form == kK2FormRows ? (k2_rows_slices(n) << 8) | ((t == 0 ? 1 : 0) << 16) : 0);
+        if (form == kK2FormRows) a.st->k2_rows_n += 1;
+        if (a.modes) a.modes[a.k2_idx] = form == kK2FormScan ? 1 : (form == kK2FormRows ? 2 : 0);
+    }
+    const uint32_t *list = a.delta_list + static_cast<size_t>(cur) * a.Gp;
+    if (form == kK2FormScan) tally_rows(reinterpret_cast<const uint4 *>(a.table), reinterpret_cast<const uint4 *>(a.refbits[cur]), a.G, a.Wp / 4, a.raw);
+    else if (form == kK2FormRows) k2_rows_block(a, list, n);
+    else if (static_cast<int>(blockIdx.x) * 256 < a.G) delta_genes(a.table, a.G, a.Wp, list, n, a.raw);
 }
 
 __global__ __launch_bounds__(256) void k2_scan(const uint32_t *__restrict__ table, const uint4 *__restrict__ refbits, int G, int Wp,
@@ -1688,8 +1737,22 @@
         a.st->raw_pass = t;
     }
     if (i >= a.G) return;
+    int4 r0 = make_int4(0, 0, 0, 0), r1 = r0;
+    const int form = a.replay ? kK2FormNone : a.st->k2_form;
+    const bool rows = (form & 0xFF) == kK2FormRows;
+    if (!rows || !(form >> 16)) { r0 = reinterpret_cast<const int4 *>(a.raw)[2 * i]; r1 = reinterpret_cast<const int4 *>(a.raw)[2 * i + 1]; }
+    if (rows) {
+        const int slices = (form >> 8) & 0xFF;
+        for (int s = 0; s < slices; ++s) {
+            const int4 *p = reinterpret_cast<const int4 *>(a.k2_part + (static_cast<size_t>(s) * a.G + i) * kRaw);
+            const int4 p0 = p[0], p1 = p[1];
+            r0.x += p0.x; r0.y += p0.y; r0.z += p0.z; r0.w += p0.w;
+            r1.x += p1.x; r1.y += p1.y; r1.z += p1.z; r1.w += p1.w;
+        }
+        reinterpret_cast<int4 *>(a.raw)[2 * i] = r0; reinterpret_cast<int4 *>(a.raw)[2 * i + 1] = r1;
+    }
     int32_t c[9];
-    const bool ok = tallies_of(a.raw, a.refbytes[cur][i] != 0, nref, i, c);
+    const bool ok = tallies_from(r0, r1, nref - (a.refbytes[cur][i] != 0 ? 1 : 0), c);
     double o[5] = {1.0, 0.0, 0.0, 0.0, 0.0};
     if (ok) mccullagh3<true>(c, o);
     if (!ok || !(fabs(o[1]) < INFINITY)) {
@@ -1966,7 +2029,7 @@
         if ((threadIdx.x & 63) == 0) basepos = atomicAdd(&st->delta_cnt[nxt], __popcll(cm));
         basepos = __shfl(basepos, 0, 64);
         const int at = basepos + __popcll(cm & ((1ULL << (threadIdx.x & 63)) - 1ULL));
-        if (changed && at < kDeltaMax) a.delta_list[static_cast<size_t>(nxt) * a.Gp + at] = (static_cast<uint32_t>(i) << 1) | (ind ? 1u : 0u);
+        if (changed && at < a.Gp) a.delta_list[static_cast<size_t>(nxt) * a.Gp + at] = (static_cast<uint32_t>(i) << 1) | (ind ? 1u : 0u);
     }
     const unsigned long long m = __ballot(ind), mc = __ballot(in_cut);
     __shared__ int wave_nn[4], wave_kc[4];
@@ -2056,6 +2119,7 @@
         IterState *h = a.host_st;
         h->passes = t + 1; h->done = a.st->done; h->need_full = (over || !ok) ? 1 : 0; h->last_full = 1;
         h->delta_cnt[(t + 1) & 1] = a.st->delta_cnt[(t + 1) & 1];
+        h->k2_rows_n = a.st->k2_rows_n;
     }
 }
 
@@ -4149,7 +4213,7 @@
     return REO_OK;
 }
 
-int32_t launch_iter_init(reo_ctx *c, const uint8_t *host_ref, const IterState *host_state)
+int32_t launch_iter_init(reo_ctx *c, const uint8_t *host_ref, const IterState *host_state, const uint32_t *host_list, int list_n)
 {
     IterInitArgs a;
     a.host_ref = host_ref; a.host_state = reinterpret_cast<const uint32_t *>(host_state);
@@ -4158,6 +4222,8 @@
     a.zero[1] = reinterpret_cast<uint32_t *>(c->modes.p); a.zero_n[1] = c->modes.n;
     a.zero[2] = reinterpret_cast<uint32_t *>(c->hist.p); a.zero_n[2] = c->hist.n;
     a.G = static_cast<int>(c->G); a.Gp = c->Gp; a.state_words = static_cast<int>(sizeof(IterState) / 4);
+    if (list_n < 0 || list_n > a.G) { set_error("launch_iter_init: a list of %d of %d genes", list_n, a.G); return REO_EINVAL; }
+    a.host_list = host_list; a.list = c->delta_list.p; a.list_n = list_n;
     k_iter_init<<<c->Gp / 256, 256, 0, c->stream>>>(a);
     REO_HIP_CHECK(hipGetLastError());
     return REO_OK;
@@ -4184,6 +4250,7 @@
     a.pval_deg = c->it_pval_deg; a.padj_deg = c->it_padj_deg;
     for (int t = 0; t < 2; ++t) { a.refbits[t] = c->refbits[t].p; a.refbytes[t] = c->refbytes[t].p; }
     a.raw = c->raw.p; a.delta_list = c->delta_list.p; a.result = c->result.p;
+    a.k2_part = c->k2_part.p; a.k2_rows_mode = c->k2_rows_mode;
     const int nchunk = (a.G + kSortChunk - 1) / kSortChunk;
     a.chunk_v = c->chunk_v.p; a.chunk_i = c->chunk_i.p;
     a.chunk_spl = c->chunk_v.p + static_cast<size_t>(nchunk) * kSortChunk;
@@ -4210,7 +4277,7 @@
         if (c->k2_idx < static_cast<int>(c->modes.n)) { a.modes = c->modes.p; a.k2_idx = c->k2_idx; }
         ++c->k2_idx;
         tic(c, 2);
-        k2_tally<<<(G + 3) / 4, 256, 0, c->stream>>>(a);
+        k2_tally<<<std::max((G + 3) / 4, k2_rows_grid(a.Gp)), 256, 0, c->stream>>>(a);
         toc(c);
         c->t_ms[4] += 1.0;
     }
diff --git a/rankcompv3.jl_amd/csrc/reo_internal.h b/rankcompv3.jl_amd/csrc/reo_internal.h
--- a/rankcompv3.jl_amd/csrc/reo_internal.h
+++ b/rankcompv3.jl_amd/csrc/reo_internal.h
@@ -9,6 +9,7 @@
 #include <vector>
 
 #include "reo_hip.h"
+#include "k2_rows.h"
 
 namespace reo {
 
@@ -44,8 +45,11 @@
     int32_t cyc_lam;
     int32_t cyc_sel;
     int32_t cyc_ndiff;
-    int32_t pad[4];
-};
+    int32_t k2_form;
+    int32_t k2_rows_n;
+    int32_t pad[2];
+};
+static_assert(kK2DeltaMax == kDeltaMax && kK2RowsChunk <= 255 && kK2RowsChunk <= kDeltaMax, "k2_rows.h: the row form fills the light path's LDS layout");
 constexpr int kFaultBarrier = 1;
 constexpr int kFaultTallies = 2;
 
@@ -299,6 +303,9 @@
     int64_t top_partners_select_us = 0;
     reo::DevBuf<int32_t> raw;
     reo::DevBuf<uint32_t> delta_list;
+    reo::DevBuf<int32_t> k2_part;
+    int k2_rows_mode = 1;
+    int it_k2_rows = 0;
     reo::DevBuf<int32_t> cont;
     reo::DevBuf<double> result;
     reo::DevBuf<double> sorted_d;
@@ -375,7 +382,7 @@
 int32_t launch_decode(reo_ctx *c, int64_t i0, int64_t i1, int64_t j0, int64_t j1, uint8_t *d_code);
 int32_t launch_pack_ref(reo_ctx *c, const uint8_t *d_bytes, uint32_t *d_bits);
 int32_t launch_cycle_skip(reo_ctx *c, int skip, int period);
-int32_t launch_iter_init(reo_ctx *c, const uint8_t *host_ref, const IterState *host_state);
+int32_t launch_iter_init(reo_ctx *c, const uint8_t *host_ref, const IterState *host_state, const uint32_t *host_list, int list_n);
 int32_t launch_tally(reo_ctx *c, int nref);
 int32_t launch_full_pass(reo_ctx *c, bool replay);
 int32_t launch_light_persistent(reo_ctx *c);
```

After: 52470 billion. About the same (-0.3%).
